# ConsenSys/gnark-crypto

Measured on AMD Instinct MI355X. Metric: G1 MSM/sec (BN254), higher is better.
Workload: dtype u32; 1 GPU; BN254 G1 MultiExp 2^20 points, bases+scalars resident in HBM; points=1048576, window_bits=16, windows=8, glv_half_scalars=True, resident_bases=False, parallelism=single GPU

## Files before the change

gnark-crypto_amd/_lib.py:

```python
import ctypes
import os
import subprocess

_HERE = os.path.dirname(os.path.abspath(__file__))
CSRC = os.path.join(_HERE, "csrc")
LIB_PATH = os.environ.get("GMSM_LIB") or os.path.join(CSRC, "libgmsm.so")

GMSM_OK, GMSM_ERR_LEN, GMSM_ERR_CONFIG, GMSM_ERR_DEVICE, GMSM_ERR_ARG, GMSM_ERR_POINT = 0, 1, 2, 3, 4, 5

GROUP_IDS = {
    ("bn254", "g1"): 0, ("bn254", "g2"): 1,
    ("bls12_381", "g1"): 2, ("bls12_381", "g2"): 3,
    ("bw6_761", "g1"): 4, ("bw6_761", "g2"): 5,
}

ABI_SYMBOLS = [
    "gmsm_bn254_g1_multiexp", "gmsm_bn254_g2_multiexp", "gmsm_bls12_381_g1_multiexp", "gmsm_bls12_381_g2_multiexp",
    "gmsm_bw6_761_g1_multiexp", "gmsm_bw6_761_g2_multiexp", "gmsm_multiexp", "gmsm_multiexp_affine", "gmsm_fold",
    "gmsm_multiexp_device", "gmsm_bases_register", "gmsm_bases_release", "gmsm_multiexp_bases",
    "gmsm_multiexp_bases_device", "gmsm_multiexp_bases_submit", "gmsm_multiexp_collect", "gmsm_multiexp_bases_batch", "gmsm_default_window_bits", "gmsm_default_plan", "gmsm_num_windows", "gmsm_window_sums_device",
    "gmsm_window_sums_enqueue", "gmsm_fold_window_sets", "gmsm_fold_windows", "gmsm_batch_scalar_mul", "gmsm_batch_scalar_mul_device",
    "gmsm_batch_jac_to_affine", "gmsm_jac_to_affine", "gmsm_affine_limbs", "gmsm_scalar_limbs", "gmsm_debug_decompose",
    "gmsm_debug_field_op", "gmsm_debug_group_op", "gmsm_debug_glv_split", "gmsm_generate_points", "gmsm_set_profiling", "gmsm_get_stage_times",
    "gmsm_get_stage_launches", "gmsm_points_from_raw", "gmsm_points_validate", "gmsm_bases_register_raw",
    "gmsm_points_from_compressed", "gmsm_points_compress", "gmsm_bases_register_compressed",
    "gmsm_bases_register_dump", "gmsm_fft_domain_new", "gmsm_fft_domain_release", "gmsm_fft_domain_info", "gmsm_fft",
    "gmsm_fft_bit_reverse", "gmsm_poly_eval", "gmsm_poly_div_x_minus_a", "gmsm_kzg_open", "gmsm_kzg_open_folded",
    "gmsm_to_lagrange_g1", "gmsm_bases_to_lagrange", "gmsm_batch_scale", "gmsm_update_monomials", "gmsm_linear_combinations", "gmsm_shplonk_open_w", "gmsm_shplonk_open_wprime",
    "gmsm_fr_batch_invert", "gmsm_iop_ratio_copy_constraint", "gmsm_iop_ratio_shuffled",
    "gmsm_fflonk_next_divisor", "gmsm_fflonk_fold", "gmsm_fflonk_fold_commit", "gmsm_fflonk_open_w", "gmsm_fflonk_open_wprime",
    "gmsm_bases_precompute", "gmsm_bases_table_bits", "gmsm_debug_table_runs", "gmsm_debug_small_runs", "gmsm_debug_reduce_shape", "gmsm_multiexp_sharded", "gmsm_bases_register_sharded", "gmsm_multiexp_bases_sharded", "gmsm_set_devices",
    "gmsm_get_devices", "gmsm_set_option", "gmsm_get_option", "gmsm_trim", "gmsm_shutdown",
    "gmsm_device_count", "gmsm_set_device", "gmsm_last_error",
    "gmsm_version",
]

_lib = None


def build(jobs=None):
    jobs = jobs or os.cpu_count() or 4
    subprocess.check_call(["make", "-C", CSRC, f"-j{jobs}", "libgmsm.so"])
    return LIB_PATH


def load():
    global _lib
    if _lib is not None:
        return _lib
    if not os.path.exists(LIB_PATH):
        raise RuntimeError(f"{LIB_PATH} is missing: run `make -C gnark-crypto_amd/csrc` (or __graft_entry__.build()); "
                           "there is no fallback implementation")
    if os.environ.get("GMSM_NO_TORCH", "0") != "1":
        try:
            import torch
        except ImportError:
            pass
    L = ctypes.CDLL(LIB_PATH)
    vp, sz, u64p = ctypes.c_void_p, ctypes.c_size_t, ctypes.c_void_p
    for name in ABI_SYMBOLS[:6]:
        f = getattr(L, name)
        f.restype = ctypes.c_int
        f.argtypes = [u64p, sz, u64p, sz, ctypes.c_int, u64p]
    L.gmsm_multiexp.restype = ctypes.c_int
    L.gmsm_multiexp.argtypes = [ctypes.c_int, u64p, sz, u64p, sz, ctypes.c_int, u64p]
    L.gmsm_multiexp_affine.restype = ctypes.c_int
    L.gmsm_multiexp_affine.argtypes = [ctypes.c_int, u64p, sz, u64p, sz, ctypes.c_int, u64p]
    L.gmsm_fold.restype = ctypes.c_int
    L.gmsm_fold.argtypes = [ctypes.c_int, u64p, sz, u64p, ctypes.c_int, u64p]
    L.gmsm_multiexp_device.restype = ctypes.c_int
    L.gmsm_multiexp_device.argtypes = [ctypes.c_int, vp, vp, sz, vp, u64p]
    L.gmsm_bases_register.restype = ctypes.c_int
    L.gmsm_bases_register.argtypes = [ctypes.c_int, u64p, vp, sz, vp]
    L.gmsm_bases_release.restype = ctypes.c_int
    L.gmsm_bases_release.argtypes = [ctypes.c_uint64]
    L.gmsm_bases_precompute.restype = ctypes.c_int
    L.gmsm_bases_precompute.argtypes = [ctypes.c_uint64, ctypes.c_uint]
    L.gmsm_bases_table_bits.restype = ctypes.c_uint
    L.gmsm_bases_table_bits.argtypes = [ctypes.c_uint64]
    L.gmsm_debug_table_runs.restype = ctypes.c_ulong
    L.gmsm_debug_table_runs.argtypes = []
    L.gmsm_debug_small_runs.restype = ctypes.c_ulong
    L.gmsm_debug_small_runs.argtypes = []
    L.gmsm_debug_reduce_shape.restype = ctypes.c_int
    L.gmsm_debug_reduce_shape.argtypes = [ctypes.c_int, ctypes.c_uint32, ctypes.c_uint32, ctypes.POINTER(ctypes.c_uint32)]
    L.gmsm_multiexp_bases.restype = ctypes.c_int
    L.gmsm_multiexp_bases.argtypes = [ctypes.c_uint64, u64p, sz, ctypes.c_int, u64p]
    L.gmsm_multiexp_bases_device.restype = ctypes.c_int
    L.gmsm_multiexp_bases_device.argtypes = [ctypes.c_uint64, vp, sz, vp, u64p]
    L.gmsm_multiexp_bases_submit.restype = ctypes.c_int
    L.gmsm_multiexp_bases_submit.argtypes = [ctypes.c_uint64, vp, sz, vp, ctypes.POINTER(ctypes.c_uint64)]
    L.gmsm_multiexp_bases_batch.restype = ctypes.c_int
    L.gmsm_multiexp_bases_batch.argtypes = [ctypes.c_uint64, u64p, vp, sz, sz, vp, u64p]
    L.gmsm_multiexp_collect.restype = ctypes.c_int
    L.gmsm_multiexp_collect.argtypes = [ctypes.c_uint64, u64p]
    L.gmsm_default_window_bits.restype = ctypes.c_uint
    L.gmsm_default_window_bits.argtypes = [ctypes.c_int, sz]
    L.gmsm_default_plan.restype = ctypes.c_int
    L.gmsm_default_plan.argtypes = [ctypes.c_int, sz] + [ctypes.POINTER(ctypes.c_uint)] * 4
    L.gmsm_num_windows.restype = ctypes.c_uint
    L.gmsm_num_windows.argtypes = [ctypes.c_int, ctypes.c_uint]
    L.gmsm_window_sums_device.restype = ctypes.c_int
    L.gmsm_window_sums_device.argtypes = [ctypes.c_int, vp, vp, sz, ctypes.c_uint, ctypes.c_uint, ctypes.c_uint, vp, u64p]
    L.gmsm_window_sums_enqueue.restype = ctypes.c_int
    L.gmsm_window_sums_enqueue.argtypes = [ctypes.c_int, vp, ctypes.c_uint64, vp, sz, ctypes.c_uint, ctypes.c_uint,
                                           ctypes.c_uint, vp, vp]
    L.gmsm_fold_window_sets.restype = ctypes.c_int
    L.gmsm_fold_window_sets.argtypes = [ctypes.c_int, ctypes.c_uint, u64p, ctypes.c_uint, u64p]
    L.gmsm_batch_scalar_mul.restype = ctypes.c_int
    L.gmsm_batch_scalar_mul.argtypes = [ctypes.c_int, u64p, u64p, sz, u64p]
    L.gmsm_batch_scalar_mul_device.restype = ctypes.c_int
    L.gmsm_batch_scalar_mul_device.argtypes = [ctypes.c_int, u64p, vp, sz, vp, vp]
    L.gmsm_batch_jac_to_affine.restype = ctypes.c_int
    L.gmsm_batch_jac_to_affine.argtypes = [ctypes.c_int, u64p, sz, u64p]
    L.gmsm_fold_windows.restype = ctypes.c_int
    L.gmsm_fold_windows.argtypes = [ctypes.c_int, ctypes.c_uint, u64p, u64p]
    L.gmsm_jac_to_affine.restype = ctypes.c_int
    L.gmsm_jac_to_affine.argtypes = [ctypes.c_int, u64p, u64p]
    L.gmsm_affine_limbs.restype = sz
    L.gmsm_affine_limbs.argtypes = [ctypes.c_int]
    L.gmsm_scalar_limbs.restype = sz
    L.gmsm_scalar_limbs.argtypes = [ctypes.c_int]
    L.gmsm_debug_decompose.restype = ctypes.c_int
    L.gmsm_debug_decompose.argtypes = [ctypes.c_int, u64p, sz, ctypes.c_uint, vp]
    L.gmsm_debug_field_op.restype = ctypes.c_int
    L.gmsm_debug_field_op.argtypes = [ctypes.c_int, ctypes.c_int, ctypes.c_int, u64p, u64p, sz, u64p]
    L.gmsm_debug_group_op.restype = ctypes.c_int
    L.gmsm_debug_group_op.argtypes = [ctypes.c_int, ctypes.c_int, u64p, u64p, sz, u64p]
    L.gmsm_generate_points.restype = ctypes.c_int
    L.gmsm_generate_points.argtypes = [ctypes.c_int, u64p, u64p, u64p, ctypes.c_int, sz, ctypes.c_int, u64p]
    L.gmsm_set_profiling.restype = None
    L.gmsm_set_profiling.argtypes = [ctypes.c_int]
    L.gmsm_get_stage_times.restype = ctypes.c_int
    L.gmsm_get_stage_times.argtypes = [vp, ctypes.c_int, vp]
    i64p = ctypes.POINTER(ctypes.c_int64)
    L.gmsm_points_from_raw.restype = ctypes.c_int
    L.gmsm_points_from_raw.argtypes = [ctypes.c_int, vp, sz, ctypes.c_int, u64p, vp, i64p]
    L.gmsm_points_validate.restype = ctypes.c_int
    L.gmsm_points_validate.argtypes = [ctypes.c_int, u64p, vp, sz, ctypes.c_int, i64p]
    L.gmsm_bases_register_raw.restype = ctypes.c_int
    L.gmsm_bases_register_raw.argtypes = [ctypes.c_int, vp, sz, ctypes.c_int, ctypes.POINTER(ctypes.c_uint64), i64p]
    L.gmsm_points_from_compressed.restype = ctypes.c_int
    L.gmsm_points_from_compressed.argtypes = [ctypes.c_int, vp, sz, ctypes.c_int, u64p, vp, i64p]
    L.gmsm_points_compress.restype = ctypes.c_int
    L.gmsm_points_compress.argtypes = [ctypes.c_int, u64p, vp, sz, vp]
    L.gmsm_bases_register_compressed.restype = ctypes.c_int
    L.gmsm_bases_register_compressed.argtypes = [ctypes.c_int, vp, sz, ctypes.c_int, ctypes.POINTER(ctypes.c_uint64), i64p]
    L.gmsm_bases_register_dump.restype = ctypes.c_int
    L.gmsm_bases_register_dump.argtypes = [ctypes.c_int, ctypes.c_char_p, ctypes.c_uint64, ctypes.c_int, sz, ctypes.c_int,
                                           ctypes.POINTER(ctypes.c_uint64), ctypes.POINTER(sz), i64p]
    L.gmsm_fft_domain_new.restype = ctypes.c_int
    L.gmsm_fft_domain_new.argtypes = [ctypes.c_int, ctypes.c_uint64, ctypes.POINTER(ctypes.c_uint64)]
    L.gmsm_fft_domain_release.restype = ctypes.c_int
    L.gmsm_fft_domain_release.argtypes = [ctypes.c_uint64]
    L.gmsm_fft_domain_info.restype = ctypes.c_int
    L.gmsm_fft_domain_info.argtypes = [ctypes.c_uint64, ctypes.POINTER(ctypes.c_uint64), u64p, u64p, u64p, u64p, u64p]
    L.gmsm_fft.restype = ctypes.c_int
    L.gmsm_fft.argtypes = [ctypes.c_uint64, u64p, vp, sz, ctypes.c_int, ctypes.c_int, ctypes.c_int, vp]
    L.gmsm_fft_bit_reverse.restype = ctypes.c_int
    L.gmsm_fft_bit_reverse.argtypes = [ctypes.c_int, u64p, vp, sz, vp]
    szp = ctypes.POINTER(sz)
    L.gmsm_poly_eval.restype = ctypes.c_int
    L.gmsm_poly_eval.argtypes = [ctypes.c_int, u64p, vp, szp, sz, u64p, vp, u64p]
    L.gmsm_poly_div_x_minus_a.restype = ctypes.c_int
    L.gmsm_poly_div_x_minus_a.argtypes = [ctypes.c_int, u64p, vp, sz, u64p, vp, u64p, vp, u64p]
    L.gmsm_kzg_open.restype = ctypes.c_int
    L.gmsm_kzg_open.argtypes = [ctypes.c_uint64, u64p, vp, sz, u64p, vp, u64p, u64p]
    L.gmsm_kzg_open_folded.restype = ctypes.c_int
    L.gmsm_kzg_open_folded.argtypes = [ctypes.c_uint64, u64p, vp, szp, sz, u64p, u64p, vp, u64p]
    L.gmsm_to_lagrange_g1.restype = ctypes.c_int
    L.gmsm_to_lagrange_g1.argtypes = [ctypes.c_int, u64p, vp, sz, vp, u64p, vp]
    L.gmsm_bases_to_lagrange.restype = ctypes.c_int
    L.gmsm_bases_to_lagrange.argtypes = [ctypes.c_uint64, sz, ctypes.POINTER(ctypes.c_uint64)]
    L.gmsm_batch_scale.restype = ctypes.c_int
    L.gmsm_batch_scale.argtypes = [ctypes.c_int, u64p, vp, sz, u64p, vp, sz, vp, u64p, vp]
    L.gmsm_update_monomials.restype = ctypes.c_int
    L.gmsm_update_monomials.argtypes = [ctypes.c_int, u64p, vp, sz, u64p, vp, u64p, vp]
    L.gmsm_linear_combinations.restype = ctypes.c_int
    L.gmsm_linear_combinations.argtypes = [ctypes.c_int, u64p, vp, sz, szp, sz, u64p, vp, u64p, u64p]
    L.gmsm_shplonk_open_w.restype = ctypes.c_int
    L.gmsm_shplonk_open_w.argtypes = [ctypes.c_uint64, u64p, vp, szp, sz, u64p, szp, u64p, vp, u64p, u64p, vp, u64p]
    L.gmsm_shplonk_open_wprime.restype = ctypes.c_int
    L.gmsm_shplonk_open_wprime.argtypes = [ctypes.c_uint64, u64p, vp, szp, sz, u64p, szp, u64p, u64p, u64p, vp, u64p, vp, u64p]
    L.gmsm_fflonk_next_divisor.restype = ctypes.c_int
    L.gmsm_fflonk_next_divisor.argtypes = [ctypes.c_int, sz, szp]
    L.gmsm_fflonk_fold.restype = ctypes.c_int
    L.gmsm_fflonk_fold.argtypes = [ctypes.c_int, u64p, vp, szp, sz, vp, u64p, vp]
    L.gmsm_fflonk_fold_commit.restype = ctypes.c_int
    L.gmsm_fflonk_fold_commit.argtypes = [ctypes.c_uint64, u64p, vp, szp, sz, vp, vp, u64p]
    L.gmsm_fflonk_open_w.restype = ctypes.c_int
    L.gmsm_fflonk_open_w.argtypes = [ctypes.c_uint64, u64p, vp, szp, szp, sz, u64p, szp, u64p, vp, u64p, u64p, u64p, vp, u64p]
    L.gmsm_fflonk_open_wprime.restype = ctypes.c_int
    L.gmsm_fflonk_open_wprime.argtypes = [ctypes.c_uint64, u64p, vp, szp, szp, sz, u64p, szp, u64p, u64p, u64p, vp, u64p, vp, u64p]
    u32p = ctypes.POINTER(ctypes.c_uint32)
    L.gmsm_fr_batch_invert.restype = ctypes.c_int
    L.gmsm_fr_batch_invert.argtypes = [ctypes.c_int, u64p, vp, sz, vp, u64p, vp]
    L.gmsm_iop_ratio_copy_constraint.restype = ctypes.c_int
    L.gmsm_iop_ratio_copy_constraint.argtypes = [ctypes.c_uint64, u64p, vp, sz, u32p, vp, vp, u64p, u64p, ctypes.c_int, ctypes.c_int, vp, u64p, vp]
    L.gmsm_iop_ratio_shuffled.restype = ctypes.c_int
    L.gmsm_iop_ratio_shuffled.argtypes = [ctypes.c_uint64, u64p, vp, u64p, vp, sz, u32p, u32p, u64p, ctypes.c_int, ctypes.c_int, vp, u64p, vp]
    L.gmsm_get_stage_launches.restype = ctypes.c_int
    L.gmsm_get_stage_launches.argtypes = [vp, ctypes.c_int]
    ip = ctypes.POINTER(ctypes.c_int)
    L.gmsm_multiexp_sharded.restype = ctypes.c_int
    L.gmsm_multiexp_sharded.argtypes = [ctypes.c_int, u64p, sz, u64p, sz, ctypes.c_int, ip, ctypes.c_int, ctypes.c_int, u64p]
    L.gmsm_bases_register_sharded.restype = ctypes.c_int
    L.gmsm_bases_register_sharded.argtypes = [ctypes.c_int, u64p, sz, ip, ctypes.c_int, ctypes.POINTER(ctypes.c_uint64)]
    L.gmsm_multiexp_bases_sharded.restype = ctypes.c_int
    L.gmsm_multiexp_bases_sharded.argtypes = [ctypes.c_uint64, u64p, sz, ctypes.c_int, ctypes.c_int, u64p]
    L.gmsm_set_devices.restype = ctypes.c_int
    L.gmsm_set_devices.argtypes = [ip, ctypes.c_int]
    L.gmsm_get_devices.restype = ctypes.c_int
    L.gmsm_get_devices.argtypes = [ip, ctypes.c_int]
    L.gmsm_debug_glv_split.restype = ctypes.c_int
    L.gmsm_debug_glv_split.argtypes = [ctypes.c_int, u64p, sz, vp]
    L.gmsm_set_option.restype = ctypes.c_int
    L.gmsm_set_option.argtypes = [ctypes.c_int, ctypes.c_uint]
    L.gmsm_get_option.restype = ctypes.c_uint
    L.gmsm_get_option.argtypes = [ctypes.c_int]
    L.gmsm_trim.restype = ctypes.c_int
    L.gmsm_trim.argtypes = [sz, ctypes.POINTER(sz)]
    L.gmsm_shutdown.restype = ctypes.c_int
    L.gmsm_shutdown.argtypes = []
    L.gmsm_device_count.restype = ctypes.c_int
    L.gmsm_set_device.restype = ctypes.c_int
    L.gmsm_set_device.argtypes = [ctypes.c_int]
    L.gmsm_last_error.restype = ctypes.c_char_p
    L.gmsm_version.restype = ctypes.c_char_p
    _lib = L
    return L


def effective_cpus():
    n = len(os.sched_getaffinity(0))
    try:
        quota, period = open("/sys/fs/cgroup/cpu.max").read().split()
        if quota != "max":
            n = min(n, max(1, int(int(quota) / int(period))))
    except (OSError, ValueError):
        pass
    return n


def last_error():
    return load().gmsm_last_error().decode()


OPTIONS = {"window_bits": 0, "tables": 1, "max_run": 2, "host_ranges": 3, "fixed_base_bits": 4, "spin_wait_us": 5, "small_bits": 6, "small_max": 7, "split": 8, "glv": 9, "small_quad": 10,
           "poly_lane_bits": 11, "reduce_shape": 12}


def set_option(name, value):
    rc = load().gmsm_set_option(OPTIONS[name], int(value))
    if rc:
        raise ValueError("gmsm: " + last_error())


def get_option(name):
    return int(load().gmsm_get_option(OPTIONS[name]))


class options:

    def __init__(self, **kw):
        self.kw, self.old = kw, {}

    def __enter__(self):
        for k, v in self.kw.items():
            self.old[k] = get_option(k)
            set_option(k, v)
        return self

    def __exit__(self, *exc):
        for k, v in self.old.items():
            set_option(k, v)
        return False


def trim(keep_bytes=0):
    freed = ctypes.c_size_t(0)
    rc = load().gmsm_trim(keep_bytes, ctypes.byref(freed))
    if rc:
        raise RuntimeError("gmsm: " + last_error())
    return int(freed.value)


def shutdown():
    rc = load().gmsm_shutdown()
    if rc:
        raise RuntimeError("gmsm: " + last_error())
```

gnark-crypto_amd/csrc/gmsm_context.h:

```cpp
#pragma once
#include <hip/hip_runtime.h>
#include <atomic>

#include <algorithm>
#include <cstdio>
#include <cstdlib>
#include <chrono>
#include <condition_variable>
#include <memory>
#include <mutex>
#include <string>
#include <thread>
#include <vector>

#include "../../include/gmsm.h"

namespace gmsm {

int fail(int code, const std::string &msg);
void clear_last_error();

#define HIP_TRY(expr)                                                                                        \
    do {                                                                                                     \
        hipError_t e_ = (expr);                                                                              \
        if (e_ != hipSuccess)                                                                                \
            return ::gmsm::fail(GMSM_ERR_DEVICE, std::string(#expr) + ": " + hipGetErrorString(e_) + " (" __FILE__ ":" + \
                                                     std::to_string(__LINE__) + ")");                        \
    } while (0)

struct DeviceBuffer {
    void *ptr = nullptr;
    size_t cap = 0;
    int ensure(size_t bytes) {
        if (bytes <= cap) return GMSM_OK;
        if (ptr) HIP_TRY(hipFree(ptr));
        ptr = nullptr;
        cap = 0;
        size_t want = bytes + bytes / 8;
        HIP_TRY(hipMalloc(&ptr, want));
        cap = want;
        return GMSM_OK;
    }
    size_t release() {
        const size_t had = cap;
        if (ptr) (void)hipFree(ptr);
        ptr = nullptr;
        cap = 0;
        return had;
    }
};

struct Options {
    std::atomic<unsigned> window_bits{0};
    std::atomic<unsigned> tables{1};
    std::atomic<unsigned> max_run{0};
    std::atomic<unsigned> host_ranges{0};
    std::atomic<unsigned> fixed_base_bits{0};
    std::atomic<unsigned> spin_wait_us{0};
    std::atomic<unsigned> small_bits{0};
    std::atomic<unsigned> split{0};
    std::atomic<unsigned> small_max{0};
    std::atomic<unsigned> glv{1};
    std::atomic<unsigned> small_quad{0};
    std::atomic<unsigned> poly_lane_bits{0};
    std::atomic<unsigned> reduce_shape{0};
};
Options &options();

extern std::atomic<unsigned long> g_small_runs;
extern std::atomic<unsigned long> g_table_runs;

struct ResidentBases {
    int group = -1;
    int device = -1;
    size_t n = 0;
    DeviceBuffer upoints, skip;
    std::atomic<unsigned> tab_c{0};
    unsigned tab_nw = 0;
    std::mutex tab_mu;
    DeviceBuffer tables;
    std::atomic<unsigned> small_c{0};
    unsigned small_nw = 0;
    size_t small_m = 0;
    DeviceBuffer small_tables;
    ResidentBases() = default;
    ResidentBases(const ResidentBases &) = delete;
    ResidentBases &operator=(const ResidentBases &) = delete;
    ~ResidentBases() {
        if (!upoints.ptr && !skip.ptr && !tables.ptr && !small_tables.ptr) return;
        int prev = 0;
        (void)hipGetDevice(&prev);
        if (device >= 0) (void)hipSetDevice(device);
        (void)hipDeviceSynchronize();
        if (upoints.ptr) (void)hipFree(upoints.ptr);
        if (skip.ptr) (void)hipFree(skip.ptr);
        if (tables.ptr) (void)hipFree(tables.ptr);
        if (small_tables.ptr) (void)hipFree(small_tables.ptr);
        (void)hipSetDevice(prev);
    }
};


struct FftDomain {
    int group = -1;
    int device = -1;
    unsigned log2n = 0;
    std::vector<uint64_t> generator, generator_inv, cardinality_inv, shift, shift_inv;
    DeviceBuffer twiddles_lz, twiddles_inv_lz;
    DeviceBuffer twiddles_rev_lz, twiddles_inv_rev_lz;
    bool rev_ready = false;
    DeviceBuffer coset, coset_inv_scaled;
    std::vector<uint64_t> cardinality_inv_lz;
    bool coset_ready = false;
    std::mutex mu;
    FftDomain() = default;
    FftDomain(const FftDomain &) = delete;
    FftDomain &operator=(const FftDomain &) = delete;
    ~FftDomain() {
        DeviceBuffer *bufs[] = {&twiddles_lz, &twiddles_inv_lz, &twiddles_rev_lz, &twiddles_inv_rev_lz, &coset, &coset_inv_scaled};
        bool any = false;
        for (auto *b : bufs) any = any || b->ptr;
        if (!any) return;
        int prev = 0;
        (void)hipGetDevice(&prev);
        if (device >= 0) (void)hipSetDevice(device);
        (void)hipDeviceSynchronize();
        for (auto *b : bufs)
            if (b->ptr) (void)hipFree(b->ptr);
        (void)hipSetDevice(prev);
    }
};

struct Workspace {
    hipStream_t stream = nullptr;
    DeviceBuffer upoints, skip;
    DeviceBuffer seg_lvl;
    DeviceBuffer seg_partials, seg_flags, seg_bucket;
    DeviceBuffer parted;
    DeviceBuffer heavy;
    DeviceBuffer long_pieces;
    DeviceBuffer small_sums, small_done;
    DeviceBuffer digits, sorted, blockhist, counts, starts, buckets, partials, totals;
    DeviceBuffer red_pre;
    DeviceBuffer carry;
    hipStream_t mstream = nullptr;
    hipEvent_t ev_buckets = nullptr, ev_merged = nullptr;
    hipStream_t cstream = nullptr;
    hipEvent_t ev_fork = nullptr, ev_conv = nullptr;
    bool conv_pending = false;
    hipEvent_t events[12] = {nullptr};
    bool timed = false;
    int timed_level = 0;
    void *pinned = nullptr;
    size_t pinned_cap = 0;
    DeviceBuffer h2d_points, h2d_scalars;
    DeviceBuffer raw_bytes, flagword;
    DeviceBuffer poly;
    DeviceBuffer lagrange;
    bool busy = false;
    bool ticket = false;
    bool pending = false;
    int pending_group = -1;
    unsigned pending_c = 0;
    uint32_t pending_nw = 0;
    uint32_t pending_gen = 0;
    std::shared_ptr<ResidentBases> bases_ref;
    hipEvent_t dep = nullptr;
    bool uncollected = false;
    hipEvent_t last_use = nullptr;
    hipStream_t last_stream = nullptr;
    bool pending_timed = false;
    size_t trim(size_t keep) {
        DeviceBuffer *all[] = {&upoints, &skip, &seg_lvl, &seg_partials, &seg_flags, &seg_bucket, &parted, &heavy, &long_pieces, &small_sums, &small_done, &digits, &sorted,
                               &blockhist, &counts, &starts, &buckets, &partials, &totals, &red_pre, &carry, &h2d_points,
                               &h2d_scalars, &raw_bytes, &flagword, &poly, &lagrange};
        size_t freed = 0;
        for (DeviceBuffer *b : all)
            if (b->cap > keep) freed += b->release();
        if (pinned && pinned_cap > keep) {
            (void)hipHostFree(pinned);
            pinned = nullptr;
            pinned_cap = 0;
        }
        return freed;
    }
    void destroy() {
        (void)trim(0);
        hipEvent_t *evs[] = {&ev_buckets, &ev_merged, &dep, &last_use, &ev_fork, &ev_conv};
        for (hipEvent_t *e : evs) {
            if (*e) (void)hipEventDestroy(*e);
            *e = nullptr;
        }
        for (auto &e : events) {
            if (e) (void)hipEventDestroy(e);
            e = nullptr;
        }
        if (stream) (void)hipStreamDestroy(stream);
        if (mstream) (void)hipStreamDestroy(mstream);
        if (cstream) (void)hipStreamDestroy(cstream);
        stream = mstream = cstream = nullptr;
        last_stream = nullptr;
        bases_ref.reset();
    }
    int ensure_base() {
        if (stream) return GMSM_OK;
        HIP_TRY(hipStreamCreateWithFlags(&stream, hipStreamNonBlocking));
        HIP_TRY(hipEventCreateWithFlags(&ev_buckets, hipEventDisableTiming));
        HIP_TRY(hipEventCreateWithFlags(&ev_merged, hipEventDisableTiming));
        HIP_TRY(hipEventCreateWithFlags(&ev_fork, hipEventDisableTiming));
        HIP_TRY(hipEventCreateWithFlags(&ev_conv, hipEventDisableTiming));
        return GMSM_OK;
    }
    int side_stream(hipStream_t &slot) {
        if (!slot) HIP_TRY(hipStreamCreateWithFlags(&slot, hipStreamNonBlocking));
        return GMSM_OK;
    }
    int ensure_pinned(size_t bytes) {
        if (bytes <= pinned_cap) return GMSM_OK;
        if (pinned) HIP_TRY(hipHostFree(pinned));
        pinned = nullptr;
        HIP_TRY(hipHostMalloc(&pinned, bytes, hipHostMallocDefault));
        pinned_cap = bytes;
        return GMSM_OK;
    }
};

struct Context {
    static constexpr int NUM_WS = 3, MAX_TICKETS = 2;
    std::mutex mu;
    std::condition_variable cv;
    int device = -1;
    Workspace ws[NUM_WS];
    int num_cus = 256;
    uint64_t epoch = 0;
    std::atomic<bool> live{false};
    int init(int dev) {
        device = dev;
// ... 281 lines not shown
    if (!v || !*v) return dflt;
    return (unsigned)strtoul(v, nullptr, 10);
}
#ifdef GMSM_EXPERIMENTS
static inline unsigned tune_uint(const char *name, unsigned dflt) { return env_uint(name, dflt); }
#else
static inline constexpr unsigned tune_uint(const char *, unsigned dflt) { return dflt; }
#endif

static inline unsigned preferred_c(unsigned fr_bits, size_t aff_bytes, size_t n) {
    unsigned lg = 0;
    while (lg < 63 && ((size_t)2 << lg) <= n) ++lg;
    if (fr_bits > 320) return lg < 13 ? 9u : lg <= 14 ? 10u : lg <= 16 ? 12u : lg <= 20 ? 14u : 16u;
    if (fr_bits == 255 && aff_bytes > 96) return lg < 13 ? 8u : lg <= 15 ? 10u : lg == 16 ? 12u : lg <= 18 ? 13u : 16u;
    if (fr_bits == 255) return lg < 13 ? 8u : lg <= 14 ? 12u : lg == 15 ? 13u : lg == 16 ? 12u : lg == 18 ? 13u : lg < 24 ? 16u : 17u;
    if (aff_bytes > 64) return lg < 13 ? 8u : lg <= 14 ? 12u : lg == 15 ? 13u : lg == 16 ? 12u : lg <= 18 ? 13u : lg < 22 ? 16u : 17u;
    return lg < 13 ? 8u : lg < 15 ? 12u : lg < 17 ? 15u : lg < 21 ? 16u : 17u;
}
static inline unsigned glv_preferred_c(unsigned fr_bits, size_t aff_bytes, size_t n) {
    unsigned lg = 0;
    while (lg < 63 && ((size_t)2 << lg) <= n) ++lg;
    if (lg < 11 || lg > 21) return 0u;
    if (fr_bits > 320) return lg <= 14 ? 10u : lg <= 16 ? 12u : lg == 17 ? 13u : lg == 18 ? 14u : 16u;
    if (fr_bits == 255 && aff_bytes > 96)
        return lg <= 14 ? 10u : lg <= 16 ? 12u : lg <= 18 ? 13u : lg == 19 ? 15u : 0u;
    if (lg < 13) return 0u;
    if (fr_bits == 255) return lg <= 14 ? 13u : lg == 16 ? 12u : lg == 19 ? 16u : 0u;
    if (aff_bytes > 64) return lg == 13 ? 12u : lg == 14 ? 13u : lg <= 16 ? 12u : lg == 17 ? 13u : 16u;
    return lg == 13 ? 12u : lg == 14 ? 13u : lg <= 20 ? 16u : 0u;
}
static inline unsigned choose_c(unsigned fr_bits, size_t aff_bytes, size_t n) {
    const unsigned forced = options().window_bits.load(std::memory_order_relaxed);
    if (forced >= 2 && forced <= 20) return forced;
    return preferred_c(fr_bits, aff_bytes, n ? n : 1);
}

struct GroupVTable {
    unsigned fr_bits;
    size_t aff_bytes, scalar_bytes, jac_bytes, xyzz_bytes;
    int (*multiexp_host)(const uint64_t *points, size_t n_points, const uint64_t *scalars, size_t n_scalars, int nb_tasks,
                         uint64_t *out_jac);
    int (*multiexp_device)(Context &ctx, const void *d_points, const void *d_scalars, size_t n, hipStream_t stream,
                           uint64_t *out_jac, const ResidentBases *resident);
    int (*window_sums)(Context &ctx, const void *d_points, const void *d_scalars, size_t n, unsigned c, unsigned win_first,
                       unsigned win_stride, hipStream_t stream, uint64_t *out_xyzz, const ResidentBases *resident);
    void (*fold)(const uint64_t *xyzz_windows, unsigned c, uint64_t *out_jac);
    void (*jac_to_affine)(const uint64_t *jac, uint64_t *out_affine);
    int (*debug_decompose)(const uint64_t *scalars, size_t n, unsigned c, uint32_t *out_digits);
    int (*debug_field_op)(int field, int op, const uint64_t *a, const uint64_t *b, size_t count, uint64_t *out);
    int (*debug_group_op)(int op, const uint64_t *acc, const uint64_t *other, size_t count, uint64_t *out);
    void (*generate_points)(const uint64_t *base, const uint64_t *k0, const uint64_t *k1, int klimbs, size_t n, int nthreads,
                            uint64_t *out);
    int (*register_bases)(Context &ctx, const void *d_points, size_t n, hipStream_t stream, ResidentBases *out);
    int (*submit)(Context &ctx, Workspace &ws, const void *d_scalars, size_t n, const ResidentBases *resident);
    int (*collect)(Workspace &ws, uint64_t *out_jac);
    int (*window_sums_enqueue)(Context &ctx, const void *d_points, const void *d_scalars, size_t n, unsigned c,
                               unsigned win_first, unsigned win_stride, hipStream_t stream, void *d_out_xyzz,
                               const std::shared_ptr<ResidentBases> &resident);
    void (*fold_sets)(const uint64_t *xyzz_sets, unsigned nsets, unsigned c, uint64_t *out_jac);
    void (*fold_powers)(const uint64_t *coeff, size_t n, uint64_t *out_scalars);
    int (*multiexp_bases_host)(Context &ctx, const uint64_t *scalars, size_t n, uint64_t *out_jac,
                               const ResidentBases *resident);
    int (*batch_scalar_mul)(Context &ctx, const uint64_t *base, const uint64_t *scalars, const void *d_scalars, size_t n,
                            hipStream_t caller_stream, uint64_t *out, void *d_out);
    int (*batch_jac_to_affine)(Context &ctx, const uint64_t *jac, size_t n, uint64_t *out);
    int (*decode_raw)(Workspace &ws, const void *d_raw, size_t n, int level, void *d_out, long long *bad_index,
                      uint32_t *status);
    int (*validate_points)(Workspace &ws, const void *d_points, size_t n, int level, long long *bad_index, uint32_t *status);
    int (*decode_compressed)(Workspace &ws, const void *d_comp, size_t n, int level, void *d_out, long long *bad_index,
                             uint32_t *status);
    int (*encode_compressed)(Workspace &ws, const void *d_points, size_t n, void *d_comp);
    int (*fft_domain_new)(Context &ctx, hipStream_t stream, unsigned log2n, FftDomain *out);
    int (*fft_run)(hipStream_t stream, FftDomain *d, void *d_a, bool inverse, bool dif, bool coset);
    int (*fft_bit_reverse)(hipStream_t stream, void *d_a, size_t n);
    int (*precompute_tables)(Context &ctx, Workspace &ws, ResidentBases *rb, unsigned c);
    bool (*tables_serve)(size_t n_registered, size_t n_call);
    int (*shard_piece)(Context &ctx, const uint64_t *points, const ResidentBases *resident, size_t resident_base,
                       const uint64_t *scalars, size_t n, unsigned c, unsigned win_first, unsigned win_stride,
                       uint64_t *out_xyzz);
    unsigned (*host_piece_ranges)(size_t n, bool with_points);
    int (*debug_glv_split)(const uint64_t *scalars, size_t n, uint32_t *out);
    void (*plan_info)(size_t n, unsigned *c, unsigned *nwin, unsigned *entries_per_point, unsigned *fused);
    void (*reduce_shape)(const Context &ctx, uint32_t nw, uint32_t nbuckets, uint32_t out[6]);
    int (*poly_eval)(Context &ctx, const uint64_t *polys, const void *d_polys, const size_t *lens, size_t k, const uint64_t *point,
                     hipStream_t stream, uint64_t *out_values);
    int (*poly_div)(Context &ctx, const uint64_t *poly, const void *d_poly, size_t n, const uint64_t *point, hipStream_t stream,
                    uint64_t *out_h, void *d_out_h, uint64_t *out_value);
    int (*kzg_open)(Context &ctx, const uint64_t *polys, const void *d_polys, const size_t *lens, size_t k, const uint64_t *point,
                    const uint64_t *gamma, hipStream_t stream, uint64_t *out_claimed, uint64_t *out_jac, const ResidentBases *resident);
    int (*to_lagrange)(Context &ctx, const uint64_t *coeffs, const void *d_coeffs, const ResidentBases *from, unsigned log2n,
                       hipStream_t stream, uint64_t *out_affine, void *d_out_affine, ResidentBases *out_bases);
    bool (*fflonk_next_divisor)(size_t n, size_t *t);
    int (*open_check)(const char *entry, const size_t *lens, const size_t *pack_sizes, size_t k, const uint64_t *points,
                      const size_t *npoints, bool check_size, size_t registered);
    int (*fflonk_fold)(Context &ctx, const uint64_t *polys, const void *d_polys, const size_t *lens, size_t npolys, hipStream_t stream,
                       uint64_t *out, void *d_out, const ResidentBases *resident, uint64_t *out_jac);
    int (*open_w)(Context &ctx, const uint64_t *polys, const void *d_polys, const size_t *lens, const size_t *pack_sizes, size_t k,
                  const uint64_t *points, const size_t *npoints, const uint64_t *gamma, hipStream_t stream, uint64_t *out_claimed,
                  uint64_t *out_folded_claimed, uint64_t *out_w, void *d_out_w, uint64_t *out_jac, const ResidentBases *resident);
    int (*open_wprime)(Context &ctx, const uint64_t *polys, const void *d_polys, const size_t *lens, const size_t *pack_sizes, size_t k,
                       const uint64_t *points, const size_t *npoints, const uint64_t *folded_claimed, const uint64_t *gamma,
                       const uint64_t *w, const void *d_w, const uint64_t *z, hipStream_t stream, uint64_t *out_jac,
                       const ResidentBases *resident);
    int (*batch_scale)(Context &ctx, const uint64_t *points, const void *d_points, size_t n, const uint64_t *scalars, const void *d_scalars,
                       size_t n_scalars, const uint64_t *r, hipStream_t stream, uint64_t *out_affine, void *d_out_affine);
    int (*linear_combinations)(Context &ctx, const uint64_t *points, const void *d_points, size_t n, const size_t *ends, size_t n_ends,
                               const uint64_t *r, hipStream_t stream, uint64_t *out_truncated_jac, uint64_t *out_shifted_jac);
    int (*fr_batch_invert)(Context &ctx, const uint64_t *a, const void *d_a, size_t n, hipStream_t stream, uint64_t *out, void *d_out);
    int (*ratio_copy)(Context &ctx, FftDomain *d, const uint64_t *entries, const void *d_entries, size_t m, const uint32_t *layouts,
                      const int64_t *perm, const void *d_perm, const uint64_t *beta, const uint64_t *gamma, int basis, int layout,
                      hipStream_t stream, uint64_t *out, void *d_out);
    int (*ratio_shuffled)(Context &ctx, FftDomain *d, const uint64_t *num, const void *d_num, const uint64_t *den, const void *d_den,
                          size_t m, const uint32_t *num_layouts, const uint32_t *den_layouts, const uint64_t *beta, int basis, int layout,
                          hipStream_t stream, uint64_t *out, void *d_out);
    unsigned fr_max_order;
};

}
```

gnark-crypto_amd/csrc/gmsm_engine.hip:

```cpp
#include <atomic>
#include <cstdio>
#include <cstring>
#include <deque>
#include <functional>
#include <map>
#include <sys/stat.h>

#include "gmsm_context.h"

namespace gmsm {

static thread_local std::string g_last_error;
static std::mutex g_any_error_mu;
static std::string g_any_error;
static thread_local int g_device = -1;
static std::atomic<int> g_default_device{0};
std::atomic<unsigned long> g_table_runs{0};
std::atomic<unsigned long> g_small_runs{0};
static std::atomic<uint32_t> g_ticket_gen{0};

std::string g_env_error;
Options &options() {
    static Options *o = [] {
        Options *x = new Options();
        const unsigned c = env_uint("GMSM_C", 0);
        x->window_bits.store(c >= 2 && c <= 20 ? c : 0);
        const unsigned t = env_uint("GMSM_TABLES", 1);
        x->tables.store(std::min(2u, t));
        if (c != 0 && (c < 2 || c > 20)) g_env_error = "GMSM_C=" + std::to_string(c) + ": the window width must be 2..20 (or unset)";
        else if (t > 2) g_env_error = "GMSM_TABLES=" + std::to_string(t) + ": 0 never, 1 the measured call sizes, 2 every call size";
        return x;
    }();
    return *o;
}

int fail(int code, const std::string &msg) {
    g_last_error = msg;
    {
        std::lock_guard<std::mutex> lk(g_any_error_mu);
        g_any_error = msg;
    }
    return code;
}

void clear_last_error() { g_last_error.clear(); }

static std::mutex g_prof_mu;
static std::atomic<int> g_profiling{0};
static double g_stage_ms[STAGE_COUNT] = {0};
static unsigned long g_stage_launches[STAGE_COUNT] = {0};
static unsigned long g_stage_calls = 0;

int profiling_level() { return g_profiling.load(std::memory_order_relaxed); }
void record_stage_times(const float *ms, const unsigned *launches) {
    std::lock_guard<std::mutex> lk(g_prof_mu);
    for (int i = 0; i < STAGE_COUNT; ++i) {
        g_stage_ms[i] += ms[i];
        g_stage_launches[i] += launches[i];
    }
    ++g_stage_calls;
}

static std::mutex g_ctx_mu;
static std::vector<Context *> g_ctx;

int get_context_for(int device, Context **out) {
    std::lock_guard<std::mutex> lk(g_ctx_mu);
    int ndev = 0;
    hipError_t e = hipGetDeviceCount(&ndev);
    if (e != hipSuccess || ndev <= 0)
        return fail(GMSM_ERR_DEVICE, std::string("no usable HIP device (hipGetDeviceCount: ") + hipGetErrorString(e) +
                                         "); libgmsm has no CPU fallback");
    if (device < 0 || device >= ndev) return fail(GMSM_ERR_DEVICE, "gmsm_set_device: device index out of range");
    if ((int)g_ctx.size() < ndev) g_ctx.resize(ndev, nullptr);
    if (!g_ctx[device]) g_ctx[device] = new Context();
    if (!g_ctx[device]->live) {
        int rc = g_ctx[device]->init(device);
        if (rc != GMSM_OK) return rc;
    }
    *out = g_ctx[device];
    return GMSM_OK;
}

int get_context(Context **out) { return get_context_for(g_device >= 0 ? g_device : g_default_device.load(), out); }

int get_context_of_pointer(const void *p, Context **out) {
    if (p) {
        hipPointerAttribute_t attr;
        if (hipPointerGetAttributes(&attr, p) == hipSuccess && attr.type == hipMemoryTypeDevice)
            return get_context_for(attr.device, out);
        (void)hipGetLastError();
    }
    return get_context(out);
}

static int select_device(int rc, Context *const *ctx) {
    if (rc) return rc;
    HIP_TRY(hipSetDevice((*ctx)->device));
    return GMSM_OK;
}
static int enter(Context **ctx) { return select_device(get_context(ctx), ctx); }
// ... 672 lines not shown
}

struct ShardedBases {
    int group = -1;
    size_t n = 0;
    std::vector<int> devices;
    std::map<int, std::shared_ptr<ResidentBases>> replicas;
};
constexpr uint64_t SHARDED_TAG = (uint64_t)1 << 62;
static HandleTable<ShardedBases> g_sharded;

static std::shared_ptr<ShardedBases> lookup_sharded(uint64_t handle) {
    return (handle & SHARDED_TAG) ? g_sharded.get(handle & ~SHARDED_TAG) : nullptr;
}

GMSM_EXPORT int gmsm_bases_register_sharded(int group, const uint64_t *points, size_t n, const int *devices, int n_devices,
                                            uint64_t *out_handle) {
    VT_OR_FAIL(group);
    if (!out_handle) return fail(GMSM_ERR_ARG, "gmsm_bases_register_sharded: out_handle is null");
    if (n && !points) return fail(GMSM_ERR_ARG, "gmsm_bases_register_sharded: points is null");
    auto sb = std::make_shared<ShardedBases>();
    sb->group = group;
    sb->n = n;
    if (devices && n_devices > 0) sb->devices.assign(devices, devices + n_devices);
    else if (int rc0 = shard_devices(sb->devices)) return rc0;
    const int ndev = gmsm_device_count();
    if (ndev <= 0) return fail(GMSM_ERR_DEVICE, "no usable HIP device; libgmsm has no CPU fallback");
    if (sb->devices.empty()) every_device(ndev, sb->devices);
    if (int rc = devices_exist("gmsm_bases_register_sharded", sb->devices.data(), sb->devices.size(), ndev)) return rc;
    std::vector<int> distinct;
    for (int d : sb->devices)
        if (std::find(distinct.begin(), distinct.end(), d) == distinct.end()) distinct.push_back(d);
    std::vector<uint64_t> handles(distinct.size(), 0);
    const Failure bad = on_threads(distinct.size(), [&](size_t i) {
        g_device = distinct[i];
        return gmsm_bases_register(group, points, nullptr, n, &handles[i]);
    });
    for (size_t i = 0; i < distinct.size(); ++i)
        if (handles[i]) {
            sb->replicas[distinct[i]] = g_bases.get(handles[i]);
            (void)gmsm_bases_release(handles[i]);
        }
    if (bad.rc) return fail(bad.rc, "device " + std::to_string(distinct[bad.index]) + ": " + bad.err);
    *out_handle = SHARDED_TAG | g_sharded.add(sb);
    return GMSM_OK;
}

static int precompute_on(const BasesRef &rb, unsigned c) {
    const GroupVTable *vt = vtable(rb->group);
    std::lock_guard<std::mutex> only_one(rb->tab_mu);
    if (rb->tab_c.load() != 0) {
        if (c == 0 || c == rb->tab_c.load()) return GMSM_OK;
        return fail(GMSM_ERR_ARG, "gmsm_bases_precompute: the handle already has tables of another width");
    }
    Context *ctx;
    int rc = get_context_for(rb->device, &ctx);
    if (rc) return rc;
    struct RestoreDevice {
        int prev = 0;
        RestoreDevice() { (void)hipGetDevice(&prev); }
        ~RestoreDevice() { (void)hipSetDevice(prev); }
    } restore;
    HIP_TRY(hipSetDevice(ctx->device));
    GMSM_LEASE_OR_FAIL(lease, *ctx);
    return vt->precompute_tables(*ctx, *lease.w, rb.get(), c);
}

GMSM_EXPORT int gmsm_bases_precompute(uint64_t handle, unsigned c) {
    if (handle & SHARDED_TAG) {
        std::shared_ptr<ShardedBases> sb = lookup_sharded(handle);
        if (!sb) return fail(GMSM_ERR_ARG, "unknown bases handle");
        std::vector<BasesRef> replicas;
        for (auto &kv : sb->replicas) replicas.push_back(kv.second);
        const Failure bad = on_threads(replicas.size(), [&](size_t i) { return precompute_on(replicas[i], c); });
        return bad.rc ? fail(bad.rc, bad.err) : GMSM_OK;
    }
    BasesRef rb = g_bases.get(handle);
    if (!rb) return fail(GMSM_ERR_ARG, "unknown bases handle");
    return precompute_on(rb, c);
}

GMSM_EXPORT unsigned long gmsm_debug_table_runs(void) { return g_table_runs.load(); }
GMSM_EXPORT unsigned long gmsm_debug_small_runs(void) { return g_small_runs.load(); }

GMSM_EXPORT unsigned gmsm_bases_table_bits(uint64_t handle) {
    if (handle & SHARDED_TAG) {
        std::shared_ptr<ShardedBases> sb = lookup_sharded(handle);
        if (!sb || sb->replicas.empty()) return 0;
        return sb->replicas.begin()->second->tab_c.load();
    }
    BasesRef rb = g_bases.get(handle);
    return rb ? rb->tab_c.load() : 0;
}

GMSM_EXPORT int gmsm_bases_release(uint64_t handle) {
    BasesRef rb;
    std::shared_ptr<ShardedBases> sb;
    if (handle & SHARDED_TAG) sb = g_sharded.take(handle & ~SHARDED_TAG);
    else rb = g_bases.take(handle);
    if (!rb && !sb) return fail(GMSM_ERR_ARG, "unknown bases handle");
    std::vector<Context *> ctxs;
    {
        std::lock_guard<std::mutex> lk(g_ctx_mu);
        ctxs = g_ctx;
    }
    for (Context *c : ctxs) {
        if (!c) continue;
        BasesRef parked[Context::NUM_WS];
        {
            std::lock_guard<std::mutex> lk(c->mu);
            for (int i = 0; i < Context::NUM_WS; ++i) {
                Workspace &w = c->ws[i];
                if (w.busy || !w.bases_ref) continue;
                const bool mine = w.bases_ref == rb || (sb && sb->replicas.count(c->device) && sb->replicas[c->device] == w.bases_ref);
                if (mine && (!w.last_use || hipEventQuery(w.last_use) == hipSuccess)) parked[i].swap(w.bases_ref);
            }
        }
    }
    return GMSM_OK;
}

static int multiexp_bases_impl(uint64_t handle, const uint64_t *scalars, const void *d_scalars, size_t n, int nb_tasks,
                               void *hip_stream, uint64_t *out_jac) {
    BasesRef rb = g_bases.get(handle);
    if (!rb) return fail(GMSM_ERR_ARG, "unknown bases handle");
    const GroupVTable *vt = vtable(rb->group);
    if (n > rb->n) return fail(GMSM_ERR_LEN, "len(points) != len(scalars)");
    if (nb_tasks > 1024) return fail(GMSM_ERR_CONFIG, "invalid config: config.NbTasks > 1024");
    Context *ctx;
    if (int rc = enter_on(rb->device, &ctx)) return rc;
    if (scalars && n) return vt->multiexp_bases_host(*ctx, scalars, n, out_jac, rb.get());
    return vt->multiexp_device(*ctx, nullptr, d_scalars, n, (hipStream_t)hip_stream, out_jac, rb.get());
}

static int multiexp_bases_sharded(uint64_t handle, const uint64_t *scalars, size_t n, int nb_tasks, int mode, uint64_t *out_jac) {
    std::shared_ptr<ShardedBases> sb = lookup_sharded(handle);
    if (!sb) return fail(GMSM_ERR_ARG, "unknown bases handle");
    const GroupVTable *vt = vtable(sb->group);
    if (n > sb->n) return fail(GMSM_ERR_LEN, "len(points) != len(scalars)");
    bool done;
    int rc = multiexp_precheck(vt, n, n, nb_tasks, out_jac, &done);
    if (rc || done) return rc;
    if (!scalars) return fail(GMSM_ERR_ARG, "scalars is null");
    return multiexp_sharded_run(sb->group, nullptr, &sb->replicas, scalars, n, sb->devices, mode, out_jac);
}

GMSM_EXPORT int gmsm_multiexp_bases(uint64_t handle, const uint64_t *scalars, size_t n_scalars, int nb_tasks,
                                    uint64_t *out_jac) {
    if (handle & SHARDED_TAG) return multiexp_bases_sharded(handle, scalars, n_scalars, nb_tasks, 0, out_jac);
    return multiexp_bases_impl(handle, scalars, nullptr, n_scalars, nb_tasks, nullptr, out_jac);
}

GMSM_EXPORT int gmsm_multiexp_bases_sharded(uint64_t handle, const uint64_t *scalars, size_t n_scalars, int nb_tasks, int mode,
                                            uint64_t *out_jac) {
    if (!(handle & SHARDED_TAG)) return fail(GMSM_ERR_ARG, "gmsm_multiexp_bases_sharded: not a handle of gmsm_bases_register_sharded");
    return multiexp_bases_sharded(handle, scalars, n_scalars, nb_tasks, mode, out_jac);
}

GMSM_EXPORT int gmsm_multiexp_bases_device(uint64_t handle, const void *d_scalars, size_t n_scalars, void *hip_stream,
                                           uint64_t *out_jac) {
    return multiexp_bases_impl(handle, nullptr, d_scalars, n_scalars, 0, hip_stream, out_jac);
}

GMSM_EXPORT int gmsm_multiexp_bases_submit(uint64_t handle, const void *d_scalars, size_t n_scalars, void *hip_stream,
                                           uint64_t *out_ticket) {
    BasesRef rb = g_bases.get(handle);
// ... 649 lines not shown
    Context *ctx;
    if ((rc = enter_on(d->device, &ctx))) return rc;
    if ((rc = check_device_vector(E, "d_entries", d_entries, ctx->device)) || (rc = check_device_vector(E, "d_perm", d_perm, ctx->device)) ||
        (rc = check_device_vector(E, "d_out", d_out, ctx->device)))
        return rc;
    return vt->ratio_copy(*ctx, d.get(), entries, d_entries, m, layouts, perm, d_perm, beta, gamma, basis, layout, (hipStream_t)hip_stream, out, d_out);
}

GMSM_EXPORT int gmsm_iop_ratio_shuffled(uint64_t domain, const uint64_t *num, const void *d_num, const uint64_t *den, const void *d_den, size_t m,
                                        const uint32_t *num_layouts, const uint32_t *den_layouts, const uint64_t *beta, int basis, int layout,
                                        void *hip_stream, uint64_t *out, void *d_out) {
    const char *E = "gmsm_iop_ratio_shuffled";
    int rc = ratio_form(E, m, basis, layout, out, d_out);
    if (rc || (rc = ratio_layouts(E, "num_layouts", num_layouts, m)) || (rc = ratio_layouts(E, "den_layouts", den_layouts, m))) return rc;
    if (!beta) return fail(GMSM_ERR_ARG, std::string(E) + ": beta must not be null");
    if ((rc = ratio_pair(E, "num", "d_num", num, d_num)) || (rc = ratio_pair(E, "den", "d_den", den, d_den))) return rc;
    FftRef d;
    const GroupVTable *vt;
    if ((rc = ratio_domain(E, domain, m, &d, &vt))) return rc;
    const size_t zbytes = vt->scalar_bytes << d->log2n;
    if (ratio_overlap(out, d_out, zbytes, num, d_num, m * zbytes) || ratio_overlap(out, d_out, zbytes, den, d_den, m * zbytes)) return ratio_aliases(E);
    Context *ctx;
    if ((rc = enter_on(d->device, &ctx))) return rc;
    if ((rc = check_device_vector(E, "d_num", d_num, ctx->device)) || (rc = check_device_vector(E, "d_den", d_den, ctx->device)) ||
        (rc = check_device_vector(E, "d_out", d_out, ctx->device)))
        return rc;
    return vt->ratio_shuffled(*ctx, d.get(), num, d_num, den, d_den, m, num_layouts, den_layouts, beta, basis, layout, (hipStream_t)hip_stream, out,
                              d_out);
}

GMSM_EXPORT int gmsm_batch_scalar_mul(int group, const uint64_t *base_affine, const uint64_t *scalars, size_t n,
                                      uint64_t *out_affine) {
    VT_OR_FAIL(group);
    if (!base_affine || (n && (!scalars || !out_affine))) return fail(GMSM_ERR_ARG, "gmsm_batch_scalar_mul: null argument");
    Context *ctx;
    int rc = enter(&ctx);
    if (rc) return rc;
    return vt->batch_scalar_mul(*ctx, base_affine, scalars, nullptr, n, nullptr, out_affine, nullptr);
}

GMSM_EXPORT int gmsm_batch_scalar_mul_device(int group, const uint64_t *base_affine, const void *d_scalars, size_t n,
                                             void *hip_stream, void *d_out_affine) {
    VT_OR_FAIL(group);
    if (!base_affine || (n && (!d_scalars || !d_out_affine)))
        return fail(GMSM_ERR_ARG, "gmsm_batch_scalar_mul_device: null argument");
    Context *ctx;
    int rc = enter_owner(d_scalars, &ctx);
    if (rc) return rc;
    return vt->batch_scalar_mul(*ctx, base_affine, nullptr, d_scalars, n, (hipStream_t)hip_stream, nullptr, d_out_affine);
}

GMSM_EXPORT int gmsm_batch_jac_to_affine(int group, const uint64_t *jac, size_t n, uint64_t *out_affine) {
    VT_OR_FAIL(group);
    if (n && (!jac || !out_affine)) return fail(GMSM_ERR_ARG, "gmsm_batch_jac_to_affine: null argument");
    Context *ctx;
    int rc = enter(&ctx);
    if (rc) return rc;
    return vt->batch_jac_to_affine(*ctx, jac, n, out_affine);
}

GMSM_EXPORT unsigned gmsm_default_window_bits(int group, size_t n) {
    const GroupVTable *vt = vtable(group);
    return vt ? choose_c(vt->fr_bits, vt->aff_bytes, n) : 0;
}

GMSM_EXPORT int gmsm_default_plan(int group, size_t n, unsigned *c, unsigned *nwin, unsigned *entries_per_point, unsigned *fused) {
    VT_OR_FAIL(group);
    unsigned a = 0, b = 0, e = 1, f = 0;
    vt->plan_info(n, &a, &b, &e, &f);
    if (c) *c = a;
    if (nwin) *nwin = b;
    if (entries_per_point) *entries_per_point = e;
    if (fused) *fused = f;
    return GMSM_OK;
}

GMSM_EXPORT int gmsm_debug_reduce_shape(int group, uint32_t nw, uint32_t nbuckets, uint32_t out[6]) {
    VT_OR_FAIL(group);
    if (nw == 0 || nbuckets == 0 || nbuckets > (1u << 19) || !out) return fail(GMSM_ERR_ARG, "gmsm_debug_reduce_shape: nw >= 1, 1 <= nbuckets <= 2^19");
    Context *ctx;
    int rc = get_context(&ctx);
    if (rc) return rc;
    vt->reduce_shape(*ctx, nw, nbuckets, out);
    return GMSM_OK;
}

GMSM_EXPORT unsigned gmsm_num_windows(int group, unsigned c) {
    const GroupVTable *vt = vtable(group);
    return (vt && c) ? num_windows(vt->fr_bits, c) : 0;
}

GMSM_EXPORT int gmsm_window_sums_device(int group, const void *d_points, const void *d_scalars, size_t n, unsigned c,
                                        unsigned win_first, unsigned win_stride, void *hip_stream, uint64_t *out_xyzz) {
    VT_OR_FAIL(group);
    if (c < 2 || c > 20) return fail(GMSM_ERR_ARG, "c out of range (2..20)");
    Context *ctx;
    int rc = enter_owner(d_scalars, &ctx);
    if (rc) return rc;
    return vt->window_sums(*ctx, d_points, d_scalars, n, c, win_first, win_stride, (hipStream_t)hip_stream, out_xyzz, nullptr);
}

GMSM_EXPORT int gmsm_window_sums_enqueue(int group, const void *d_points, uint64_t bases_handle, const void *d_scalars,
                                         size_t n, unsigned c, unsigned win_first, unsigned win_stride, void *hip_stream,
                                         void *d_out_xyzz) {
    VT_OR_FAIL(group);
    if (c < 2 || c > 20) return fail(GMSM_ERR_ARG, "c out of range (2..20)");
    if (!d_out_xyzz) return fail(GMSM_ERR_ARG, "d_out_xyzz is null");
    BasesRef rb;
    if (bases_handle) {
        rb = g_bases.get(bases_handle);
        if (!rb || rb->group != group) return fail(GMSM_ERR_ARG, "unknown bases handle");
        if (n > rb->n) return fail(GMSM_ERR_LEN, "len(points) != len(scalars)");
    }
    Context *ctx;
    int rc = rb ? enter_on(rb->device, &ctx) : enter_owner(d_out_xyzz, &ctx);
    if (rc) return rc;
    return vt->window_sums_enqueue(*ctx, d_points, d_scalars, n, c, win_first, win_stride, (hipStream_t)hip_stream,
                                   d_out_xyzz, rb);
}

GMSM_EXPORT int gmsm_fold_window_sets(int group, unsigned c, const uint64_t *xyzz_sets, unsigned nsets, uint64_t *out_jac) {
    VT_OR_FAIL(group);
    if (c < 2 || c > 24) return fail(GMSM_ERR_ARG, "c out of range");
    if (nsets == 0) return fail(GMSM_ERR_ARG, "nsets must be >= 1");
    vt->fold_sets(xyzz_sets, nsets, c, out_jac);
    return GMSM_OK;
}

GMSM_EXPORT int gmsm_fold_windows(int group, unsigned c, const uint64_t *xyzz_windows, uint64_t *out_jac) {
    VT_OR_FAIL(group);
    if (c < 2 || c > 24) return fail(GMSM_ERR_ARG, "c out of range");
    vt->fold(xyzz_windows, c, out_jac);
    return GMSM_OK;
}

GMSM_EXPORT int gmsm_jac_to_affine(int group, const uint64_t *jac, uint64_t *out_affine) {
    VT_OR_FAIL(group);
    vt->jac_to_affine(jac, out_affine);
    return GMSM_OK;
}

GMSM_EXPORT size_t gmsm_affine_limbs(int group) {
    const GroupVTable *vt = vtable(group);
    return vt ? vt->aff_bytes / 8 : 0;
}

GMSM_EXPORT size_t gmsm_scalar_limbs(int group) {
    const GroupVTable *vt = vtable(group);
    return vt ? vt->scalar_bytes / 8 : 0;
}

GMSM_EXPORT int gmsm_debug_decompose(int group, const uint64_t *scalars, size_t n, unsigned c, uint32_t *out_digits) {
    VT_OR_FAIL(group);
    return vt->debug_decompose(scalars, n, c, out_digits);
}

GMSM_EXPORT int gmsm_debug_glv_split(int group, const uint64_t *scalars, size_t n, uint32_t *out) {
    VT_OR_FAIL(group);
    return vt->debug_glv_split(scalars, n, out);
}

GMSM_EXPORT int gmsm_debug_field_op(int group, int field, int op, const uint64_t *a, const uint64_t *b, size_t count,
                                    uint64_t *out) {
    VT_OR_FAIL(group);
    if (count == 0) return GMSM_OK;
    return vt->debug_field_op(field, op, a, b, count, out);
// ... 27 lines not shown
GMSM_EXPORT int gmsm_get_stage_times(double *out_ms, int max_stages, unsigned long *out_calls) {
    std::lock_guard<std::mutex> lk(g_prof_mu);
    int n = max_stages < (int)STAGE_COUNT ? max_stages : (int)STAGE_COUNT;
    for (int i = 0; i < n; ++i) out_ms[i] = g_stage_ms[i];
    if (out_calls) *out_calls = g_stage_calls;
    return n;
}

GMSM_EXPORT int gmsm_get_stage_launches(unsigned long *out_launches, int max_stages) {
    std::lock_guard<std::mutex> lk(g_prof_mu);
    int n = max_stages < (int)STAGE_COUNT ? max_stages : (int)STAGE_COUNT;
    for (int i = 0; i < n; ++i) out_launches[i] = g_stage_launches[i];
    return n;
}

GMSM_EXPORT int gmsm_device_count(void) {
    int n = 0;
    if (hipGetDeviceCount(&n) != hipSuccess) return 0;
    return n;
}

GMSM_EXPORT int gmsm_set_device(int device) {
    int n = gmsm_device_count();
    if (device < 0 || device >= n) return fail(GMSM_ERR_DEVICE, "gmsm_set_device: no such device");
    g_device = device;
    g_default_device.store(device);
    g_pinned.store(true);
    return GMSM_OK;
}

GMSM_EXPORT int gmsm_set_devices(const int *devices, int count) {
    std::vector<int> list;
    if (count > 0) {
        if (!devices) return fail(GMSM_ERR_ARG, "gmsm_set_devices: devices is null");
        if (int rc = devices_exist("gmsm_set_devices", devices, (size_t)count, gmsm_device_count())) return rc;
        list.assign(devices, devices + count);
    }
    std::lock_guard<std::mutex> lk(g_devices_mu);
    g_devices = list;
    g_devices_explicit = count > 0;
    if (count > 0) g_default_device.store(list[0]);
    else g_pinned.store(false);
    return GMSM_OK;
}

GMSM_EXPORT int gmsm_get_devices(int *out_devices, int max_devices) {
    std::vector<int> list;
    if (shard_devices(list) != GMSM_OK) return -1;
    if (list.empty()) {
        if (out_devices && max_devices > 0) out_devices[0] = g_device >= 0 ? g_device : g_default_device.load();
        return 1;
    }
    if (out_devices)
        for (int i = 0; i < (int)list.size() && i < max_devices; ++i) out_devices[i] = list[i];
    return (int)list.size();
}

struct OptionRow {
    int key;
    std::atomic<unsigned> Options::*member;
    bool (*accepts)(unsigned value);
    const char *refusal;
    bool as_flag = false;
};
static const OptionRow OPTION_ROWS[] = {
    {GMSM_OPT_WINDOW_BITS, &Options::window_bits, [](unsigned v) { return v == 0 || (v >= 2 && v <= 20); },
     "GMSM_OPT_WINDOW_BITS: 0 (the measured table) or 2..20"},
    {GMSM_OPT_TABLES, &Options::tables, [](unsigned v) { return v <= 2; }, "GMSM_OPT_TABLES: 0 never, 1 the measured call sizes, 2 every call size"},
    {GMSM_OPT_MAX_RUN, &Options::max_run, nullptr, nullptr},
    {GMSM_OPT_HOST_RANGES, &Options::host_ranges, nullptr, nullptr},
    {GMSM_OPT_FIXED_BASE_BITS, &Options::fixed_base_bits, [](unsigned v) { return v == 0 || (v >= 2 && v <= 14); },
     "GMSM_OPT_FIXED_BASE_BITS: 0 (by batch size) or 2..14"},
    {GMSM_OPT_SMALL_BITS, &Options::small_bits, [](unsigned v) { return v <= 7; },
     "GMSM_OPT_SMALL_BITS: 0 (on, width by size), 1 (off) or 2..7 (on, forced width)"},
    {GMSM_OPT_SMALL_MAX, &Options::small_max, nullptr, nullptr},
    {GMSM_OPT_SPLIT, &Options::split, nullptr, nullptr, true},
    {GMSM_OPT_GLV, &Options::glv, [](unsigned v) { return v <= 2; }, "GMSM_OPT_GLV: 0 never, 1 where measured ahead, 2 every unregistered call"},
    {GMSM_OPT_SMALL_QUAD, &Options::small_quad, [](unsigned v) { return v <= 2; }, "GMSM_OPT_SMALL_QUAD: 0 by call size, 1 never, 2 always"},
    {GMSM_OPT_POLY_LANE_BITS, &Options::poly_lane_bits, [](unsigned v) { return v <= 6; },
     "GMSM_OPT_POLY_LANE_BITS: 0 (lane width by length) or 1..6 (lanes of 2^(k-1) coefficients)"},
    {GMSM_OPT_REDUCE_SHAPE, &Options::reduce_shape,
     [](unsigned v) { return !(v > 255 || (v & 15u) > 8 || ((v >> 4) & 3u) == 1 || ((v >> 6) & 3u) == 3); },
     "GMSM_OPT_REDUCE_SHAPE: 0 (the cost model) or log2L (0, 1..8) | levels (0, 2, 3) << 4 | combine kernel (0, 1, 2) << 6"},
    {GMSM_OPT_SPIN_WAIT_US, &Options::spin_wait_us, [](unsigned v) { return v <= 1000000; }, "GMSM_OPT_SPIN_WAIT_US: at most 1000000"},
};
static const OptionRow *option_row(int key) {
    for (const OptionRow &r : OPTION_ROWS)
        if (r.key == key) return &r;
    return nullptr;
}

GMSM_EXPORT int gmsm_set_option(int key, unsigned value) {
    Options &o = options();
    const OptionRow *r = option_row(key);
    if (!r) return fail(GMSM_ERR_ARG, "gmsm_set_option: unknown key");
    if (r->accepts && !r->accepts(value)) return fail(GMSM_ERR_ARG, r->refusal);
    (o.*r->member).store(r->as_flag ? (value ? 1 : 0) : value);
    return GMSM_OK;
}

GMSM_EXPORT unsigned gmsm_get_option(int key) {
    Options &o = options();
    const OptionRow *r = option_row(key);
    return r ? (o.*r->member).load() : 0;
}

GMSM_EXPORT int gmsm_trim(size_t keep_bytes, size_t *out_freed) {
    if (out_freed) *out_freed = 0;
    std::vector<Context *> ctxs;
    {
        std::lock_guard<std::mutex> lk(g_ctx_mu);
        ctxs = g_ctx;
    }
    int prev = 0;
    (void)hipGetDevice(&prev);
    size_t freed = 0;
    for (Context *c : ctxs) {
        if (!c || !c->live) continue;
        (void)hipSetDevice(c->device);
        for (int i = 0; i < Context::NUM_WS; ++i) {
            Workspace *w = c->acquire_this(i);
            if (!w) continue;
            if (w->last_use) (void)hipEventSynchronize(w->last_use);
            if (w->stream) (void)hipStreamSynchronize(w->stream);
            if (w->mstream) (void)hipStreamSynchronize(w->mstream);
            if (w->cstream) (void)hipStreamSynchronize(w->cstream);
            w->conv_pending = false;
            std::shared_ptr<ResidentBases> parked;
            parked.swap(w->bases_ref);
            freed += w->trim(keep_bytes);
            c->release(w);
        }
    }
    (void)hipSetDevice(prev);
    if (out_freed) *out_freed = freed;
    return GMSM_OK;
}

GMSM_EXPORT int gmsm_shutdown(void) {
    std::vector<Context *> ctxs;
    {
        std::lock_guard<std::mutex> lk(g_ctx_mu);
        ctxs = g_ctx;
    }
    std::vector<std::pair<Context *, Workspace *>> held;
    for (Context *c : ctxs) {
        if (!c || !c->live) continue;
        for (int i = 0; i < Context::NUM_WS; ++i) {
            Workspace *w = c->acquire_unless_ticket(i);
            if (!w) {
                for (auto &h : held) h.first->release(h.second);
                return fail(GMSM_ERR_ARG, "gmsm_shutdown: a submitted MultiExp has not been collected");
            }
            held.emplace_back(c, w);
        }
    }
    {
        const auto bases = g_bases.drain();
        const auto sharded = g_sharded.drain();
        const auto ffts = g_fft.drain();
    }
    int prev = 0;
    (void)hipGetDevice(&prev);
    for (Context *c : ctxs) {
        if (!c || !c->live) continue;
        (void)hipSetDevice(c->device);
// ... 19 lines not shown
```

gnark-crypto_amd/csrc/gmsm_group.h:

```cpp
#pragma once
#include <algorithm>
#include <cstdlib>
#include <cstring>
#include <thread>
#include <type_traits>
#include <vector>

#include "gmsm_context.h"
#include "gmsm_group_host.h"
#include "gmsm_kernels.h"
#include "gmsm_fixup_q.h"
#include "gmsm_small.h"
#include "gmsm_fixedbase.h"
#include "gmsm_ingest.h"
#include "gmsm_decompress.h"
#include "gmsm_fft.h"
#include "gmsm_poly.h"
#include "gmsm_shplonk.h"
#include "gmsm_fflonk.h"
#include "gmsm_group_fft.h"
#include "gmsm_scale.h"
#include "gmsm_ratio.h"

namespace gmsm {

#define GMSM_TUNE(NAME, DFLT) tune_uint("GMSM_" #NAME, (DFLT))

template <class T> struct LazyOf;
template <class P> struct LazyOf<Fp<P>> { using type = FpU<P>; };
template <class P> struct LazyOf<Fp2<P>> { using type = Fp2U<P>; };

template <class F_, class FrP_, class Consts_, bool NEEDS_TORSION_>
struct Group : GroupHost<F_, FrP_> {
    using Host = GroupHost<F_, FrP_>;
    using Host::batch_to_affine;
    using Host::build_fixed_base_table;
    using Host::fold;
    using Host::fold_powers;
    using Host::fold_sets;
    using Host::generate_points;
    using Host::scalar_mul;
    using F = F_;
    using FrP = FrP_;
    using Consts = Consts_;
    static constexpr bool NEEDS_TORSION = NEEDS_TORSION_;
    using Aff = Affine<F>;
    using Ext = XYZZ<F>;
    using J = Jac<F>;
    static constexpr unsigned FR_BITS = FrP::BITS;
    static constexpr size_t AFF_BYTES = sizeof(Aff);
    static constexpr size_t SCALAR_BYTES = sizeof(Fp<FrP>);
    using U = typename LazyOf<F>::type;
#ifndef GMSM_INLINE_OPS_BYTES
#define GMSM_INLINE_OPS_BYTES (28 * 4)
#endif
    static constexpr bool INLINE_OPS = sizeof(U) <= GMSM_INLINE_OPS_BYTES;
    using OpsSerial = UnsatOps<U>;
    using OpsElem = typename OpsSerial::Elem;
#ifndef GMSM_FORK_CONVERT_LOG2
#define GMSM_FORK_CONVERT_LOG2 18
#endif
    static constexpr size_t FORK_CONVERT_MIN = (size_t)1 << GMSM_FORK_CONVERT_LOG2;
    static constexpr int COMBINE_N = 64;
    static constexpr int RED2_TPB = 64;
#ifndef GMSM_SERIAL_QUAD_WORDS
#define GMSM_SERIAL_QUAD_WORDS 14
#endif
    static constexpr bool SERIAL_QUAD = sizeof(U) >= GMSM_SERIAL_QUAD_WORDS * 4;
#ifndef GMSM_SERIAL_Q_QUADS
#define GMSM_SERIAL_Q_QUADS 64
#endif
    static constexpr int SERIAL_Q_QUADS = GMSM_SERIAL_Q_QUADS;
#ifndef GMSM_COMBINE_WE_WORDS
#define GMSM_COMBINE_WE_WORDS 9
#endif
    static constexpr bool COMBINE_WE = sizeof(U) <= GMSM_COMBINE_WE_WORDS * 4;
    static bool use_combine_we(const Context &ctx, uint32_t workgroups) {
        const unsigned forced = (options().reduce_shape.load(std::memory_order_relaxed) >> 6) & 3u;
        if (forced) return COMBINE_WE && forced == 2;
        return COMBINE_WE && workgroups >= 2u * (uint32_t)ctx.num_cus;
    }
    static constexpr uint32_t FIX_MAXWALK = FIXUP_MAXWALK;
#ifndef GMSM_FIXUP_QUAD_WORDS
#define GMSM_FIXUP_QUAD_WORDS 15
#endif
    static constexpr bool FIXUP_QUAD = sizeof(U) >= GMSM_FIXUP_QUAD_WORDS * 4;
    static constexpr bool SKEWED_HOST_RANGES = AFF_BYTES <= 96;
    static constexpr size_t COMBINE_RESIDENT = sizeof(U) <= 36 ? 4 : sizeof(U) <= 56 ? 3 : sizeof(U) <= 72 ? 2 : 1;

    static WindowPlan make_plan(unsigned c, unsigned win_first, unsigned win_stride) {
        WindowPlan p;
        p.c = c;
        p.nwin_total = num_windows(FR_BITS, c);
        unsigned lc = last_c(FR_BITS, c);
        p.nbuckets = 1u << (std::max(c, lc) - 1);
        p.win_first = win_first;
        p.win_stride = win_stride ? win_stride : 1;
        p.nwin_local = win_first < p.nwin_total ? (p.nwin_total - win_first + p.win_stride - 1) / p.win_stride : 0;
        p.shared = 0;
        p.glv = 0;
        return p;
    }
    static constexpr unsigned GLV_BITS = (unsigned)FrP::GLV_BITS;
    static WindowPlan make_plan_glv(unsigned c, unsigned win_first, unsigned win_stride) {
        WindowPlan p = make_plan(c, win_first, win_stride);
        p.nwin_total = num_windows(GLV_BITS, c);
        p.nbuckets = 1u << (std::max(c, last_c(GLV_BITS, c)) - 1);
        p.nwin_local = win_first < p.nwin_total ? (p.nwin_total - win_first + p.win_stride - 1) / p.win_stride : 0;
        p.glv = 1;
        return p;
    }

    static int window_sums(Context &ctx, Workspace &ws, const void *d_points, const void *d_scalars, size_t n,
                           const WindowPlan &plan, hipStream_t caller_stream, Ext *host_xyzz,
                           const ResidentBases *resident = nullptr, size_t resident_offset = 0) {
        int rc = order_after(ws, caller_stream);
        if (rc) return rc;
        if ((rc = enqueue_window_sums(ctx, ws, d_points, d_scalars, n, plan, ws.stream, resident, nullptr, resident_offset)))
            return rc;
        return collect_window_sums(ws, ws.stream, plan.nwin_local, host_xyzz);
    }

    static int collect_window_sums(Workspace &ws, hipStream_t stream, uint32_t nw, Ext *host_xyzz) {
        if (nw == 0) return GMSM_OK;
        HIP_TRY(wait_stream(stream));
        if (ws.pending_timed) StageTimer::collect(ws);
        ws.pending_timed = false;
        memcpy(host_xyzz, ws.pinned, (size_t)nw * sizeof(Ext));
        return GMSM_OK;
    }

    static uint64_t fr_modulus_shifted(unsigned shift) {
        uint64_t v = 0;
        for (int b = 62; b >= 0; --b) {
            const unsigned bit = shift + (unsigned)b;
            if (bit < 32u * FrP::N && ((FrP::Q[bit >> 5] >> (bit & 31)) & 1u)) v |= (uint64_t)1 << b;
        }
        return v;
    }
    static uint64_t max_digit_code(const WindowPlan &plan) {
        if (plan.glv) {
            const uint64_t low = ((uint64_t)1 << plan.c) - 1;
            const unsigned top_bits = GLV_BITS - (plan.nwin_total - 1) * plan.c;
            return std::max(low, (uint64_t)2 << top_bits);
        }
        const uint64_t low = ((uint64_t)1 << plan.c) - 1;
        const unsigned top_shift = (plan.nwin_total - 1) * plan.c;
        const uint64_t top = top_shift >= 63 + 32u * FrP::N ? 0 : ((fr_modulus_shifted(top_shift) + 1) << 1);
        return plan.nwin_total > 1 ? std::max(low, top) : top;
    }

    struct Geometry {
        uint32_t seg, tpw;
        uint32_t log2L, nblocks1, log2span;
        uint32_t nblocks2;
    };

    static Geometry plan_geometry(const Context &ctx, uint32_t nw, size_t n, uint32_t NB, bool shared_set = false) {
        Geometry q;
        constexpr size_t SPAN1 = COMBINE_N;
        const auto blocks1 = [&](uint32_t l2) { return ((size_t)NB + (SPAN1 << l2) - 1) / (SPAN1 << l2); };
        const auto blocks2 = [&](uint32_t l2) { return (blocks1(l2) + SPAN1 - 1) / SPAN1; };
        const unsigned forced_shape = options().reduce_shape.load(std::memory_order_relaxed);
        uint32_t log2L = GMSM_TUNE(LOG2L, forced_shape & 15u);
        const uint32_t force_levels = GMSM_TUNE(REDUCE_LEVELS, (forced_shape >> 4) & 3u);
        bool three = force_levels == 3;
        if (log2L == 0) {
            const auto costs = [&](uint32_t l2, size_t resident, size_t *c3) {
                const size_t serial_threads = (size_t)nw * (((size_t)NB + ((size_t)1 << l2) - 1) >> l2);
                const size_t serial_lanes = SERIAL_QUAD ? 4 * serial_threads : serial_threads;
                const size_t serial_rounds = (serial_lanes + (size_t)ctx.num_cus * 256 - 1) / ((size_t)ctx.num_cus * 256);
                const size_t per_round = (size_t)ctx.num_cus * resident;
                const size_t rounds = ((size_t)nw * blocks1(l2) + per_round - 1) / per_round;
                const size_t cost_serial = (SERIAL_QUAD ? 1 : 3) * serial_rounds * ((size_t)2 << l2);
                const size_t c2 = cost_serial + rounds * (2 * 6 + l2 + 1);
                const size_t rounds_b = ((size_t)nw * blocks2(l2) + per_round - 1) / per_round;
                *c3 = c2 + rounds_b * (2 * 6 + 8) + 4;
                return c2;
            };
            size_t best2 = ~(size_t)0, best3 = ~(size_t)0, unused = 0;
            uint32_t l2_two = 0, l2_three = 0;
            for (uint32_t l2 = 1; l2 <= 8; ++l2) {
                const size_t c2 = costs(l2, 1, &unused);
                if (blocks1(l2) <= (size_t)RED2_TPB && c2 < best2) {
                    best2 = c2;
                    l2_two = l2;
                }
                size_t c3 = 0;
                (void)costs(l2, COMBINE_RESIDENT, &c3);
                if (blocks1(l2) > 1 && blocks2(l2) <= (size_t)RED2_TPB && c3 < best3) {
                    best3 = c3;
                    l2_three = l2;
                }
            }
            const size_t two_resident = l2_two ? costs(l2_two, COMBINE_RESIDENT, &unused) : ~(size_t)0;
            if (force_levels == 3 ? l2_three != 0 : (force_levels != 2 && l2_three != 0 && best3 < two_resident)) {
                log2L = l2_three;
                three = true;
            } else if (l2_two) {
                log2L = l2_two;
                three = false;
            } else {
                log2L = 8;
            }
        } else if (three && blocks1(log2L) <= 1) {
            three = false;
        }
        if (three) {
            while (blocks2(log2L) > (size_t)RED2_TPB) ++log2L;
        } else {
            while (blocks1(log2L) > (size_t)RED2_TPB) ++log2L;
// ... 2 lines not shown
        q.nblocks1 = (uint32_t)blocks1(log2L);
        q.nblocks2 = three ? (uint32_t)blocks2(log2L) : 0u;
        q.log2span = log2L;
        for (size_t t = SPAN1; t > 1; t >>= 1) ++q.log2span;
        uint32_t seg = GMSM_TUNE(SEG, 0);
        if (seg == 0) {
            const size_t cap_blocks = (size_t)ctx.num_cus * AccWaves<U>::value;
            const size_t SEG_MAX = GMSM_TUNE(SEGMAX, 512);
            size_t seg_floor = 32;
            if (sizeof(U) <= 72 && n / NB <= 8) {
                const size_t entries = (size_t)nw * n, cap_threads = cap_blocks * 256;
                seg_floor = entries / 8 <= cap_threads ? 8 : entries / 16 <= cap_threads ? 16 : 32;
            } else if (sizeof(U) <= 72 && shared_set) {
                const size_t entries = (size_t)nw * n;
                if (sizeof(U) <= 56) seg_floor = entries <= ((size_t)1 << 19) ? 8 : entries <= ((size_t)3 << 19) ? 16 : 32;
                else seg_floor = entries <= ((size_t)3 << 18) ? 16 : 32;
            }
            size_t best_seg = 0, first_r = 0;
            double best_fill = -1.0;
            for (size_t r = 1; r < 100000; ++r) {
                const size_t bpw = r * cap_blocks / nw;
                if (bpw == 0) continue;
                const size_t sg = std::max<size_t>((n + bpw * 256 - 1) / (bpw * 256), seg_floor);
                if (sg > SEG_MAX) continue;
                if (!first_r) first_r = r;
                const size_t blocks = (size_t)nw * (((n + sg - 1) / sg + 255) / 256);
                const double fill = (double)blocks / (double)(((blocks + cap_blocks - 1) / cap_blocks) * cap_blocks);
                if (fill > best_fill + 1e-9) {
                    best_fill = fill;
                    best_seg = sg;
                }
                if (fill > 0.985 || r >= first_r + 5 || sg == seg_floor) break;
            }
            seg = (uint32_t)(best_seg ? best_seg : seg_floor);
        }
        q.seg = seg;
        q.tpw = (uint32_t)((n + seg - 1) / seg);
        return q;
    }

    static void launch_decompose(const void *d_scalars, size_t n, const WindowPlan &plan, bool d16, void *digits,
                                 const uint8_t *skip, hipStream_t stream) {
        const dim3 grid((unsigned)((n + 255) / 256)), block(256);
        if (plan.glv) {
#define GMSM_DECOMPOSE_GLV(CC)                                                                                                  \
    case CC:                                                                                                                    \
        if (d16) hipLaunchKernelGGL((k_decompose_glv<FrP, uint16_t, CC>), grid, block, 0, stream, (const uint32_t *)d_scalars, n, \
                                    plan, (uint16_t *)digits, skip);                                                             \
        else hipLaunchKernelGGL((k_decompose_glv<FrP, uint32_t, CC>), grid, block, 0, stream, (const uint32_t *)d_scalars, n,     \
                                plan, (uint32_t *)digits, skip);                                                                 \
        return;
            switch (plan.c) {
                GMSM_DECOMPOSE_GLV(10) GMSM_DECOMPOSE_GLV(11) GMSM_DECOMPOSE_GLV(12) GMSM_DECOMPOSE_GLV(13) GMSM_DECOMPOSE_GLV(14)
                GMSM_DECOMPOSE_GLV(15) GMSM_DECOMPOSE_GLV(16) GMSM_DECOMPOSE_GLV(17) GMSM_DECOMPOSE_GLV(18) GMSM_DECOMPOSE_GLV(20)
                default: return;
            }
#undef GMSM_DECOMPOSE_GLV
        }
#define GMSM_DECOMPOSE_C(CC)                                                                                                \
    case CC:                                                                                                                \
        if (d16) hipLaunchKernelGGL((k_decompose_c<FrP, uint16_t, CC>), grid, block, 0, stream, (const uint32_t *)d_scalars, n,  \
                                    plan, (uint16_t *)digits, skip);                                                         \
        else hipLaunchKernelGGL((k_decompose_c<FrP, uint32_t, CC>), grid, block, 0, stream, (const uint32_t *)d_scalars, n,      \
                                plan, (uint32_t *)digits, skip);                                                             \
        return;
        switch (plan.c) {
            GMSM_DECOMPOSE_C(8) GMSM_DECOMPOSE_C(9) GMSM_DECOMPOSE_C(10) GMSM_DECOMPOSE_C(12) GMSM_DECOMPOSE_C(13)
            GMSM_DECOMPOSE_C(14) GMSM_DECOMPOSE_C(15) GMSM_DECOMPOSE_C(16) GMSM_DECOMPOSE_C(17) GMSM_DECOMPOSE_C(18)
            GMSM_DECOMPOSE_C(20)
            default: break;
        }
#undef GMSM_DECOMPOSE_C
        if (d16)
            hipLaunchKernelGGL((k_decompose<FrP, uint16_t>), grid, block, 0, stream, (const uint32_t *)d_scalars, n, plan,
                               (uint16_t *)digits, skip);
        else
            hipLaunchKernelGGL((k_decompose<FrP, uint32_t>), grid, block, 0, stream, (const uint32_t *)d_scalars, n, plan,
                               (uint32_t *)digits, skip);
    }

    static int enqueue_window_sums(Context &ctx, Workspace &ws, const void *d_points, const void *d_scalars, size_t n,
                                   const WindowPlan &plan, hipStream_t stream, const ResidentBases *resident,
                                   void *d_out = nullptr, size_t resident_offset = 0 ,
                                   bool buckets_only = false, bool time_range = false ) {
        const uint32_t nwd = plan.nwin_local;
        ws.pending_timed = false;
        if (nwd == 0) return GMSM_OK;
        const bool shared = plan.shared != 0;
        if (shared && !(resident && resident->tab_c.load() == plan.c && plan.win_first == 0 && plan.win_stride == 1))
            return fail(GMSM_ERR_ARG, "shared-bucket plan without matching window tables");
        if (shared && n) g_table_runs.fetch_add(1, std::memory_order_relaxed);
        if (ws.uncollected) {
            if (ws.timed && hipEventQuery(ws.events[ws.timed_level == 2 ? T_FIXUP : T_END]) == hipSuccess) StageTimer::collect(ws);
            ws.uncollected = false;
        }
        int rc;
        if ((rc = begin_use(ws, stream))) return rc;
        if (n == 0) {
            int rc0 = ws.ensure_pinned((size_t)nwd * sizeof(Ext));
            if (rc0) return rc0;
            if (d_out) HIP_TRY(hipStreamSynchronize(stream));
            for (uint32_t k = 0; k < nwd; ++k) ((Ext *)ws.pinned)[k] = Ext::infinity();
            if (d_out) {
                HIP_TRY(hipMemcpyAsync(d_out, ws.pinned, (size_t)nwd * sizeof(Ext), hipMemcpyHostToDevice, stream));
                HIP_TRY(hipStreamSynchronize(stream));
            }
            return GMSM_OK;
        }
        const size_t n_points = n;
        const uint32_t nw = shared ? 1u : nwd;
        if (shared) n *= nwd;
        const bool glv = plan.glv != 0;
        if (glv && (shared || resident)) return fail(GMSM_ERR_ARG, "GLV plan over registered bases");
        if (glv) n *= 2;
        if (n >= ((size_t)1 << 31)) return fail(GMSM_ERR_ARG, "n must be < 2^31");
        const uint32_t NB = plan.nbuckets;
        constexpr size_t REC = sizeof(typename OpsSerial::Mem);

        const Geometry q = plan_geometry(ctx, nw, n, NB, shared);
        const bool split = options().split.load(std::memory_order_relaxed) != 0 && !buckets_only && !shared && nw >= 4 && q.nblocks2 == 0;
        const Geometry qa = split ? plan_geometry(ctx, nw / 2, n, NB, shared) : q;
        const size_t tot_thr = (size_t)nw * qa.tpw;
        const size_t tot_blk = (size_t)nw * q.nblocks1;

        uint32_t log2NB = 0;
        while ((1u << log2NB) < NB) ++log2NB;
        uint32_t log2n = 0;
        while (((size_t)1 << log2n) < n) ++log2n;
        const uint32_t lidx = log2n + 1;
        const uint32_t part_log2 = GMSM_TUNE(PART_LOG2, log2n <= 21 ? 13 : log2n >= 24 ? 15 : 14);
        int fb = (int)part_log2 + (int)log2NB - (int)log2n;
        if (fb > (int)log2NB) fb = (int)log2NB;
        if (fb > 15) fb = 15;
        if (fb < 0) fb = 0;
        if (fb + lidx > 32) fb = 32 - lidx;
        const uint32_t fbits = (uint32_t)fb;
        const uint32_t nparts = NB >> fbits;
        const bool big_chunk = n > ((size_t)1 << 25) && (size_t)nparts * 8 + PART_CHUNK_BIG * 6 <= 152 * 1024;
        const size_t pchunk_len = big_chunk ? PART_CHUNK_BIG : PART_CHUNK;
        const uint32_t pchunks = (uint32_t)((n + pchunk_len - 1) / pchunk_len);
        const size_t scatter_lds = (size_t)nparts * 8 + pchunk_len * 6;
        if (scatter_lds > 152 * 1024)
            return fail(GMSM_ERR_ARG, plan.c > 17 ? "window width too large for this many points in one pipeline run (a run takes up to "
                                                    "2^(44-c) points for c > 17): use a smaller c or split by point range"
                                                  : "more than 2^27 points in one pipeline run: split the window sums by point range "
                                                    "and add the sets (gmsm_fold_window_sets); the MultiExp entries do this themselves");
        const size_t fine_cnt_bytes = (size_t)4 << fbits;
        const uint32_t stage_cap = fine_cnt_bytes >= 156 * 1024 ? 0u
                                   : (uint32_t)std::min<size_t>(GMSM_TUNE(STAGE_CAP, part_log2 >= 15 ? 39000 : 24576),
                                                              (156 * 1024 - fine_cnt_bytes) / 4);
        if (stage_cap > 40u * 1024u) return fail(GMSM_ERR_ARG, "window geometry: staging slots beyond the fine sort's registers");
        if (fine_cnt_bytes + (size_t)stage_cap * 4 > 160 * 1024)
            return fail(GMSM_ERR_ARG, "window geometry: fine-sort counters exceed the LDS");
        const bool d16 = max_digit_code(plan) < 65536;
        const size_t dsz = d16 ? 2 : 4;

        if ((rc = ws.digits.ensure((size_t)nw * n * dsz))) return rc;
        if ((rc = ws.sorted.ensure((size_t)nw * n * 4))) return rc;
        if ((rc = ws.parted.ensure((size_t)nw * n * 4))) return rc;
        if ((rc = ws.starts.ensure((size_t)nw * (NB + 1) * 4))) return rc;
        if ((rc = ws.buckets.ensure((size_t)nw * NB * REC))) return rc;
        if ((rc = ws.partials.ensure((tot_blk + (size_t)nw * q.nblocks2) * 2 * REC))) return rc;
        const uint32_t T = (uint32_t)(((size_t)NB + ((size_t)1 << q.log2L) - 1) >> q.log2L);
        if ((rc = ws.red_pre.ensure((size_t)nw * T * 2 * REC))) return rc;
        if ((rc = ws.totals.ensure((size_t)nwd * sizeof(Ext)))) return rc;
        if ((rc = ws.ensure_pinned((size_t)nwd * sizeof(Ext)))) return rc;
        if ((rc = ws.blockhist.ensure((size_t)nw * pchunks * nparts * 4))) return rc;
        if ((rc = ws.counts.ensure((size_t)nw * (2 * nparts + 1) * 4))) return rc;
        if ((rc = ws.seg_partials.ensure(tot_thr * 2 * REC))) return rc;
        if ((rc = ws.seg_flags.ensure(tot_thr * 4))) return rc;
        if ((rc = ws.seg_bucket.ensure(tot_thr * 4))) return rc;
        const size_t list_cap = 2 * (tot_thr / FIX_MAXWALK + tot_thr / LONG_PIECE + nw + 16);
        if ((rc = ws.seg_lvl.ensure((size_t)nw * 4 + 16 + list_cap * sizeof(LongChain)))) return rc;
        uint32_t *long_flag = (uint32_t *)ws.seg_lvl.ptr;
        LongChain *long_list = (LongChain *)((char *)ws.seg_lvl.ptr + (((size_t)nw * 4 + 15) / 16) * 16);
        const size_t piece_sums_off = ((list_cap * 4 + 15) / 16) * 16;
        if ((rc = ws.long_pieces.ensure(piece_sums_off + list_cap * REC))) return rc;
        uint32_t *piece_done = (uint32_t *)ws.long_pieces.ptr;
        void *piece_sums = (char *)ws.long_pieces.ptr + piece_sums_off;
        const uint32_t hcap = (uint32_t)std::min<size_t>(nparts, n / ((size_t)stage_cap + 1) + 1);
        const uint32_t scap = (uint32_t)(n / HEAVY_SUB) + hcap;
        const size_t hparts_bytes = (((size_t)nw * hcap * sizeof(HeavyPart) + 15) / 16) * 16, hcount_bytes = (((size_t)nw * 8 + 4 + 15) / 16) * 16;
        if ((rc = ws.heavy.ensure(hparts_bytes + hcount_bytes + ((size_t)nw * scap << fbits) * 4))) return rc;
        HeavyPart *hparts = (HeavyPart *)ws.heavy.ptr;
        uint32_t *hcount = (uint32_t *)((char *)ws.heavy.ptr + hparts_bytes);
        uint32_t *subhist = (uint32_t *)((char *)ws.heavy.ptr + hparts_bytes + hcount_bytes);
        if (nw > HEAVY_MAX_WINDOWS) return fail(GMSM_ERR_ARG, "more than 256 windows in one pipeline run");
        const uint32_t heavy_wg = (uint32_t)std::min<size_t>((size_t)2 * ctx.num_cus, std::max<size_t>((size_t)nw * scap, 1));
        uint32_t *bh = (uint32_t *)ws.blockhist.ptr, *part_base = (uint32_t *)ws.counts.ptr;
        uint32_t *part_pop = part_base + (size_t)nw * (nparts + 1);

        if ((rc = ctx.allow_lds((const void *)k_part_hist<uint16_t>, 160 * 1024))) return rc;
        if ((rc = ctx.allow_lds((const void *)k_part_hist<uint32_t>, 160 * 1024))) return rc;
        if ((rc = ctx.allow_lds((const void *)k_part_scatter<uint16_t, PART_CHUNK>, 152 * 1024))) return rc;
        if ((rc = ctx.allow_lds((const void *)k_part_scatter<uint32_t, PART_CHUNK>, 152 * 1024))) return rc;
        if ((rc = ctx.allow_lds((const void *)k_part_scatter<uint16_t, PART_CHUNK_BIG>, 152 * 1024))) return rc;
        if ((rc = ctx.allow_lds((const void *)k_part_scatter<uint32_t, PART_CHUNK_BIG>, 152 * 1024))) return rc;
        if ((rc = ctx.allow_lds((const void *)k_fine_sort<24>, 160 * 1024))) return rc;
        if ((rc = ctx.allow_lds((const void *)k_fine_sort<40>, 160 * 1024))) return rc;
        if ((rc = ctx.allow_lds((const void *)k_heavy_hist, 128 * 1024))) return rc;
        if ((rc = ctx.allow_lds((const void *)k_heavy_scan, 128 * 1024))) return rc;
        if ((rc = ctx.allow_lds((const void *)k_heavy_place, 128 * 1024))) return rc;
        if ((rc = ctx.allow_lds((const void *)k_fixup_long<U>, (int)(128 * sizeof(QRec<U>))))) return rc;
        if constexpr (FIXUP_QUAD)
            if ((rc = ctx.allow_lds((const void *)k_fixup_seg_q<U>, (int)(128 * sizeof(QRec<U>))))) return rc;
        if ((rc = ctx.allow_lds((const void *)k_combine_q<U, true, COMBINE_N>, (int)((2 * COMBINE_N + 1) * sizeof(QRec<U>))))) return rc;
        if constexpr (COMBINE_WE)
            if ((rc = ctx.allow_lds((const void *)k_combine_we<U, true>, (int)((2 * COMBINE_N + 1) * sizeof(QRec<U>))))) return rc;
        if constexpr (SERIAL_QUAD)
            if ((rc = ctx.allow_lds((const void *)k_reduce_serial_q<U, SERIAL_Q_QUADS>, (int)(3 * SERIAL_Q_QUADS * sizeof(QRec<U>))))) return rc;
        if ((rc = ctx.allow_lds((const void *)k_reduce2_q<U, true>, (int)(2 * RED2_TPB * sizeof(QRec<U>))))) return rc;

        StageTimer timer(ws, !buckets_only || time_range);
        ws.timed = timer.on;
        timer.mark(T_DECOMPOSE, stream);
        const uint8_t *skip = nullptr;
        const void *upoints = nullptr;
        bool forked = false;
        if (resident) {
            upoints = (const char *)(shared ? resident->tables.ptr : resident->upoints.ptr) + resident_offset * AFF_BYTES;
            skip = (const uint8_t *)resident->skip.ptr + resident_offset;
        } else {
            if ((rc = ws.upoints.ensure((glv ? 2 : 1) * n_points * AFF_BYTES))) return rc;
            forked = n_points >= FORK_CONVERT_MIN;
            if (forked && (rc = ws.side_stream(ws.cstream))) return rc;
            hipStream_t cs = forked ? ws.cstream : stream;
            if (forked) {
                HIP_TRY(hipEventRecord(ws.ev_fork, stream));
                HIP_TRY(hipStreamWaitEvent(cs, ws.ev_fork, 0));
            }
            if (glv)
                hipLaunchKernelGGL((k_convert_points_glv<U, Consts>), dim3((unsigned)((n_points + 255) / 256)), dim3(256), 0,
                                   cs, d_points, n_points, ws.upoints.ptr);
            else
                hipLaunchKernelGGL((k_convert_points<U>), dim3((unsigned)((n_points + 255) / 256)), dim3(256), 0,
                                   cs, d_points, n_points, ws.upoints.ptr, (uint8_t *)nullptr);
            if (forked) {
                ws.conv_pending = true;
                HIP_TRY(hipEventRecord(ws.ev_conv, cs));
            }
            upoints = ws.upoints.ptr;
            skip = nullptr;
        }
        launch_decompose(d_scalars, n_points, plan, d16, ws.digits.ptr, skip, stream);

        const void *digits = ws.digits.ptr;
        uint32_t *sorted = (uint32_t *)ws.sorted.ptr, *parted = (uint32_t *)ws.parted.ptr, *starts = (uint32_t *)ws.starts.ptr;
        char *buckets = (char *)ws.buckets.ptr, *seg_partials = (char *)ws.seg_partials.ptr;
        uint32_t *seg_flags = (uint32_t *)ws.seg_flags.ptr, *seg_bucket = (uint32_t *)ws.seg_bucket.ptr;

        timer.mark(T_HIST, stream);
        if (d16)
            hipLaunchKernelGGL(k_part_hist<uint16_t>, dim3(pchunks, nw), dim3(1024), (size_t)nparts * 4, stream,
                               (const uint16_t *)digits, n, nparts, fbits, pchunk_len, bh);
        else
            hipLaunchKernelGGL(k_part_hist<uint32_t>, dim3(pchunks, nw), dim3(1024), (size_t)nparts * 4, stream,
                               (const uint32_t *)digits, n, nparts, fbits, pchunk_len, bh);
        timer.mark(T_SCAN, stream);
        if ((size_t)((nparts + 31) / 32) * nw < (size_t)ctx.num_cus && pchunks >= 256)
            hipLaunchKernelGGL(k_part_colscan<32>, dim3((nparts + 31) / 32, nw), dim3(1024), 0, stream, bh, pchunks, nparts, part_pop, hcount + 2 * nw);
        else
            hipLaunchKernelGGL(k_part_colscan<8>, dim3((nparts + 31) / 32, nw), dim3(256), 0, stream, bh, pchunks, nparts, part_pop, hcount + 2 * nw);
        hipLaunchKernelGGL(k_part_rowscan, dim3(nw), dim3(1024), 0, stream, part_pop, nparts, part_base, long_flag, stage_cap, hparts,
                           hcount, hcap);
        timer.mark(T_SCATTER, stream);
        {
            const dim3 grid(pchunks, nw), block(1024);
#define GMSM_SCATTER(D, CH)                                                                                              \
    hipLaunchKernelGGL((k_part_scatter<D, CH>), grid, block, scatter_lds, stream, (const D *)digits, n, nparts, fbits, lidx, \
                       pchunk_len, bh, part_base, parted)
            if (d16 && !big_chunk) GMSM_SCATTER(uint16_t, PART_CHUNK);
            else if (d16) GMSM_SCATTER(uint16_t, PART_CHUNK_BIG);
            else if (!big_chunk) GMSM_SCATTER(uint32_t, PART_CHUNK);
            else GMSM_SCATTER(uint32_t, PART_CHUNK_BIG);
#undef GMSM_SCATTER
        }
        if (stage_cap <= 24u * 1024u)
            hipLaunchKernelGGL(k_fine_sort<24>, dim3(nparts, nw), dim3(1024), ((size_t)4 << fbits) + (size_t)stage_cap * 4, stream,
                               parted, n, NB, fbits, lidx, part_base, sorted, starts, stage_cap);
        else
            hipLaunchKernelGGL(k_fine_sort<40>, dim3(nparts, nw), dim3(1024), ((size_t)4 << fbits) + (size_t)stage_cap * 4, stream,
                               parted, n, NB, fbits, lidx, part_base, sorted, starts, stage_cap);
        if (n > stage_cap) {
            hipLaunchKernelGGL(k_heavy_hist, dim3(heavy_wg), dim3(1024), (size_t)4 << fbits, stream, parted, n, nw, nparts, fbits, lidx,
                               part_base, (const HeavyPart *)hparts, (const uint32_t *)hcount, hcap, scap, subhist);
            hipLaunchKernelGGL(k_heavy_scan, dim3(std::min<uint32_t>(hcap, 64u), nw), dim3(1024), (size_t)4 << fbits, stream, nparts, NB, fbits,
                               part_base, (const HeavyPart *)hparts, (const uint32_t *)hcount, hcap, scap, subhist, starts);
            hipLaunchKernelGGL(k_heavy_place, dim3(heavy_wg), dim3(1024), (size_t)4 << fbits, stream, parted, n, nw, nparts, fbits, lidx,
                               part_base, (const HeavyPart *)hparts, (const uint32_t *)hcount, hcap, scap, (const uint32_t *)subhist, sorted);
        }
        if (forked) {
            HIP_TRY(hipStreamWaitEvent(stream, ws.ev_conv, 0));
            ws.conv_pending = false;
        }
        const auto accumulate = [&](uint32_t k0, uint32_t nk, hipStream_t st) {
            const uint32_t *st_g = starts + (size_t)k0 * (NB + 1);
            const uint32_t *sorted_g = sorted + (size_t)k0 * n;
            char *buckets_g = buckets + (size_t)k0 * NB * REC, *part_g = seg_partials + (size_t)k0 * qa.tpw * 2 * REC;
            if (shared)
                hipLaunchKernelGGL((k_accumulate_seg<U, true>), dim3((qa.tpw + 255) / 256, nk), dim3(256), 0, st, upoints, n, NB,
                                   qa.seg, st_g, sorted_g, buckets_g, part_g, seg_flags + (size_t)k0 * qa.tpw, seg_bucket + (size_t)k0 * qa.tpw,
                                   qa.tpw, (uint32_t)n_points, (uint32_t)resident->n);
            else
                hipLaunchKernelGGL((k_accumulate_seg<U, false>), dim3((qa.tpw + 255) / 256, nk), dim3(256), 0, st, upoints, n, NB,
                                   qa.seg, st_g, sorted_g, buckets_g, part_g, seg_flags + (size_t)k0 * qa.tpw, seg_bucket + (size_t)k0 * qa.tpw,
                                   qa.tpw, 0u, 0u);
        };
        const auto fixup_and_reduce = [&](uint32_t k0, uint32_t nk, size_t list_off, hipStream_t st, bool mark) {
            const uint32_t *st_g = starts + (size_t)k0 * (NB + 1);
            char *buckets_g = buckets + (size_t)k0 * NB * REC, *part_g = seg_partials + (size_t)k0 * qa.tpw * 2 * REC;
            const uint32_t *flags_g = seg_flags + (size_t)k0 * qa.tpw, *pb_g = seg_bucket + (size_t)k0 * qa.tpw;
            uint32_t *cnt_g = long_flag + k0;
            LongChain *list_g = long_list + list_off;
            uint32_t *done_g = piece_done + list_off;
            void *sums_g = (char *)piece_sums + list_off * REC;
            if (shared && n / NB >= 2 * (size_t)qa.seg)
                hipLaunchKernelGGL((k_fixup_bucket<OpsSerial>), dim3((NB + 255) / 256, nk), dim3(256), 0, st, NB, st_g, qa.seg,
                                   (const void *)part_g, qa.tpw, (void *)buckets_g, cnt_g, list_g, done_g, FIX_MAXWALK);
            else if constexpr (FIXUP_QUAD)
                hipLaunchKernelGGL((k_fixup_seg_q<U>), dim3((qa.tpw + 63) / 64, nk), dim3(256), 128 * sizeof(QRec<U>), st, NB,
                                   (const void *)part_g, flags_g, pb_g, qa.tpw, (void *)buckets_g, cnt_g, list_g, done_g, FIX_MAXWALK, st_g, qa.seg);
            else
                hipLaunchKernelGGL((k_fixup_seg<OpsSerial>), dim3((qa.tpw + 255) / 256, nk), dim3(256), 0, st, NB, part_g, flags_g, pb_g,
                                   qa.tpw, buckets_g, cnt_g, list_g, done_g, FIX_MAXWALK, st_g, qa.seg);
            hipLaunchKernelGGL((k_fixup_long<U>), dim3(2 * ctx.num_cus), dim3(256), 128 * sizeof(QRec<U>), st, NB, part_g, pb_g, qa.tpw,
                               buckets_g, (const uint32_t *)cnt_g, (const LongChain *)list_g, done_g, sums_g, st_g, qa.seg);
            if (mark) timer.mark(T_REDUCE, st);
            if (!buckets_only) enqueue_reduce_kernels(ctx, ws, q, T, buckets_g, st_g, nk, NB, st, k0);
        };
        timer.mark(T_ACCUMULATE, stream);
        if (!split) {
            accumulate(0, nw, stream);
            timer.mark(T_FIXUP, stream);
            fixup_and_reduce(0, nw, 0, stream, true);
        } else {
            const uint32_t ha = nw / 2;
            if ((rc = ws.side_stream(ws.mstream))) return rc;
            accumulate(0, ha, stream);
            HIP_TRY(hipEventRecord(ws.ev_buckets, stream));
            HIP_TRY(hipStreamWaitEvent(ws.mstream, ws.ev_buckets, 0));
            fixup_and_reduce(0, ha, 0, ws.mstream, false);
            HIP_TRY(hipEventRecord(ws.ev_merged, ws.mstream));
            accumulate(ha, nw - ha, stream);
            timer.mark(T_FIXUP, stream);
            fixup_and_reduce(ha, nw - ha, list_cap / 2, stream, true);
            HIP_TRY(hipStreamWaitEvent(stream, ws.ev_merged, 0));
        }
        if (!buckets_only && nwd > nw)
            hipLaunchKernelGGL((k_fill_infinity<Ext>), dim3((nwd - nw + 63) / 64), dim3(64), 0, stream, ws.totals.ptr, nw, nwd - nw);
        timer.mark(T_END, stream);
        HIP_TRY(hipGetLastError());
        if (!buckets_only) {
            if (d_out)
                HIP_TRY(hipMemcpyAsync(d_out, ws.totals.ptr, (size_t)nwd * sizeof(Ext), hipMemcpyDeviceToDevice, stream));
            else
                HIP_TRY(hipMemcpyAsync(ws.pinned, ws.totals.ptr, (size_t)nwd * sizeof(Ext), hipMemcpyDeviceToHost, stream));
        }
        if ((rc = end_use(ws, stream))) return rc;
        ws.pending_timed = timer.on;
        return GMSM_OK;
    }

    static uint32_t reduce2_active(uint32_t nlast) {
        uint32_t active = 2;
        while (active < nlast) active <<= 1;
        return active;
    }
    static void reduce_shape(const Context &ctx, uint32_t nw, uint32_t NB, uint32_t out[6]) {
        const Geometry q = plan_geometry(ctx, nw, NB, NB);
        out[0] = q.log2L;
        out[1] = q.nblocks1;
        out[2] = q.nblocks2;
        out[3] = use_combine_we(ctx, q.nblocks1 * nw) ? 2u : 1u;
        out[4] = SERIAL_QUAD ? 1u : 0u;
        out[5] = reduce2_active(q.nblocks2 ? q.nblocks2 : q.nblocks1);
    }

    static void enqueue_reduce_kernels(Context &ctx, Workspace &ws, const Geometry &q, uint32_t T, const void *buckets,
                                       const uint32_t *starts, uint32_t nw, uint32_t NB, hipStream_t stream,
                                       uint32_t k0 = 0 ) {
        constexpr size_t RECB = sizeof(typename OpsSerial::Mem);
        void *red_pre = (char *)ws.red_pre.ptr + (size_t)k0 * T * 2 * RECB;
        void *partials = (char *)ws.partials.ptr + (size_t)k0 * q.nblocks1 * 2 * RECB;
        void *totals = (char *)ws.totals.ptr + (size_t)k0 * sizeof(Ext);
        const uint32_t prescale = q.log2span;
        if constexpr (SERIAL_QUAD)
            hipLaunchKernelGGL((k_reduce_serial_q<U, SERIAL_Q_QUADS>), dim3((T + SERIAL_Q_QUADS - 1) / SERIAL_Q_QUADS, nw), dim3(4 * SERIAL_Q_QUADS),
                               3 * SERIAL_Q_QUADS * sizeof(QRec<U>), stream, buckets, NB, q.log2L, T, starts, red_pre);
        else
            hipLaunchKernelGGL((k_reduce_serial<OpsSerial>), dim3((T + 255) / 256, nw), dim3(256), 0, stream, buckets, NB,
                               q.log2L, T, starts, red_pre);
        const auto combine = [&](const void *in, uint32_t pairs, void *out, uint32_t blocks, uint32_t l2, uint32_t pre) {
            if constexpr (COMBINE_WE) {
                if (use_combine_we(ctx, blocks * nw)) {
                    hipLaunchKernelGGL((k_combine_we<U, true>), dim3(blocks, nw), dim3(4 * COMBINE_N),
                                       (2 * COMBINE_N + 1) * sizeof(QRec<U>), stream, l2, out, pre, in, pairs);
                    return;
                }
            }
            hipLaunchKernelGGL((k_combine_q<U, true, COMBINE_N>), dim3(blocks, nw), dim3(4 * COMBINE_N),
                               (2 * COMBINE_N + 1) * sizeof(QRec<U>), stream, l2, out, pre, in, pairs);
        };
        combine(red_pre, T, partials, q.nblocks1, q.log2L, prescale);
        const void *last = partials;
        uint32_t nlast = q.nblocks1, rest = q.log2span - prescale;
        if (q.nblocks2) {
            constexpr size_t REC = sizeof(typename OpsSerial::Mem);
            void *out2 = (char *)partials + (size_t)nw * q.nblocks1 * 2 * REC;
            uint32_t lgN = 0;
            for (size_t t = COMBINE_N; t > 1; t >>= 1) ++lgN;
            combine(partials, q.nblocks1, out2, q.nblocks2, 0, lgN);
            last = out2;
            nlast = q.nblocks2;
            rest = 0;
        }
        const uint32_t active = reduce2_active(nlast);
        hipLaunchKernelGGL((k_reduce2_q<U, true>), dim3(nw), dim3(4 * active), 2 * active * sizeof(QRec<U>), stream, last, nlast,
                           rest, active, totals);
        (void)ctx;
    }

    static int enqueue_reduce(Context &ctx, Workspace &ws, const void *buckets, const WindowPlan &plan, size_t n_for_geometry,
                              hipStream_t stream) {
        const uint32_t nw = bucket_sets(plan), nwd = plan.nwin_local, NB = plan.nbuckets;
        constexpr size_t REC = sizeof(typename OpsSerial::Mem);
        const Geometry q = plan_geometry(ctx, nw, n_for_geometry, NB);
        const uint32_t T = (uint32_t)(((size_t)NB + ((size_t)1 << q.log2L) - 1) >> q.log2L);
        int rc;
        if ((rc = ws.partials.ensure((size_t)nw * (q.nblocks1 + q.nblocks2) * 2 * REC))) return rc;
        if ((rc = ws.red_pre.ensure((size_t)nw * T * 2 * REC))) return rc;
        if ((rc = ws.totals.ensure((size_t)nwd * sizeof(Ext)))) return rc;
        if ((rc = ws.ensure_pinned((size_t)nwd * sizeof(Ext)))) return rc;
        if ((rc = ctx.allow_lds((const void *)k_combine_q<U, true, COMBINE_N>, (int)((2 * COMBINE_N + 1) * sizeof(QRec<U>))))) return rc;
        if constexpr (COMBINE_WE)
            if ((rc = ctx.allow_lds((const void *)k_combine_we<U, true>, (int)((2 * COMBINE_N + 1) * sizeof(QRec<U>))))) return rc;
        if constexpr (SERIAL_QUAD)
            if ((rc = ctx.allow_lds((const void *)k_reduce_serial_q<U, SERIAL_Q_QUADS>, (int)(3 * SERIAL_Q_QUADS * sizeof(QRec<U>))))) return rc;
        if ((rc = ctx.allow_lds((const void *)k_reduce2_q<U, true>, (int)(2 * RED2_TPB * sizeof(QRec<U>))))) return rc;
        enqueue_reduce_kernels(ctx, ws, q, T, buckets, nullptr, nw, NB, stream);
        if (nwd > nw)
            hipLaunchKernelGGL((k_fill_infinity<Ext>), dim3((nwd - nw + 63) / 64), dim3(64), 0, stream, ws.totals.ptr, nw, nwd - nw);
        HIP_TRY(hipGetLastError());
        HIP_TRY(hipMemcpyAsync(ws.pinned, ws.totals.ptr, (size_t)nwd * sizeof(Ext), hipMemcpyDeviceToHost, stream));
        return GMSM_OK;
    }

    static int normalize_records(Workspace &ws, size_t n, void *d_out) {
        int rc;
        if ((rc = ws.partials.ensure(n * sizeof(U)))) return rc;
        constexpr int K = 32;
        const size_t threads = (n + K - 1) / K;
        hipLaunchKernelGGL((k_batch_normalize<U, INLINE_OPS, K>), dim3((unsigned)((threads + 63) / 64)), dim3(64), 0, ws.stream,
                           ws.buckets.ptr, n, (U *)ws.partials.ptr, d_out);
        HIP_TRY(hipGetLastError());
        return GMSM_OK;
    }

    static int batch_scalar_mul(Context &ctx, Workspace &ws, const uint64_t *base_limbs, const void *d_scalars, size_t n,
                                void *d_out) {
        if (n == 0) return GMSM_OK;
        Aff base;
        memcpy(&base, base_limbs, sizeof base);
        if (base.is_infinity()) {
            HIP_TRY(hipMemsetAsync(d_out, 0, n * AFF_BYTES, ws.stream));
            return GMSM_OK;
        }
        const unsigned forced_c = options().fixed_base_bits.load(std::memory_order_relaxed);
        const unsigned c = forced_c ? forced_c : n < ((size_t)1 << 21) ? 8 : 11;
        const WindowPlan plan = make_plan(c, 0, 1);
        std::vector<Aff> table;
        build_fixed_base_table(base, plan.c, plan.nwin_total, plan.nbuckets, (int)std::min<unsigned>(16, usable_cpus()), table);
        int rc;
        const size_t tn = table.size();
        if ((rc = ws.h2d_points.ensure(tn * AFF_BYTES))) return rc;
        if ((rc = ws.upoints.ensure(tn * AFF_BYTES))) return rc;
        if ((rc = ws.skip.ensure(tn))) return rc;
        if ((rc = ws.buckets.ensure(n * sizeof(XYZZL<U>)))) return rc;
        HIP_TRY(hipMemcpyAsync(ws.h2d_points.ptr, table.data(), tn * AFF_BYTES, hipMemcpyHostToDevice, ws.stream));
        hipLaunchKernelGGL((k_convert_points<U>), dim3((unsigned)((tn + 255) / 256)), dim3(256), 0, ws.stream,
                           ws.h2d_points.ptr, tn, ws.upoints.ptr, (uint8_t *)ws.skip.ptr);
        hipLaunchKernelGGL((k_fixed_base<U, FrP, INLINE_OPS>), dim3((unsigned)((n + 255) / 256)), dim3(256), 0, ws.stream,
                           (const uint32_t *)d_scalars, n, plan, ws.upoints.ptr, ws.buckets.ptr);
        HIP_TRY(hipGetLastError());
        if ((rc = normalize_records(ws, n, d_out))) return rc;
        HIP_TRY(hipStreamSynchronize(ws.stream));
        (void)ctx;
        return GMSM_OK;
    }

    static int batch_jac_to_affine(Workspace &ws, const void *d_jac, size_t n, void *d_out) {
        if (n == 0) return GMSM_OK;
        int rc;
        if ((rc = ws.buckets.ensure(n * sizeof(XYZZL<U>)))) return rc;
        hipLaunchKernelGGL((k_jac_to_recs<U, INLINE_OPS>), dim3((unsigned)((n + 255) / 256)), dim3(256), 0, ws.stream, d_jac, n,
                           ws.buckets.ptr);
        HIP_TRY(hipGetLastError());
        return normalize_records(ws, n, d_out);
    }

    static constexpr bool LAGRANGE_GLV = GMSM_LAGRANGE_GLV != 0;
    static int to_lagrange(Workspace &ws, const void *d_in, bool packed, unsigned log2n, void *d_out) {
        static_assert(std::is_same<U, FpU<typename LzTraits<U>::Params>>::value, "ToLagrangeG1: coordinates in Fp");
        using Tw = WalkScalar<FrP, LAGRANGE_GLV>;
        using Fld = FftField<FrP>;
        using Fr = Fp<FrP>;
        constexpr size_t REC = sizeof(XYZZL<U>);
        const size_t n = (size_t)1 << log2n, half = n / 2;
        const size_t tab_recs = LAGRANGE_GLV ? 3 * n : 0;
        const size_t tw_off = (n + tab_recs) * REC;
        int rc;
        if ((rc = ws.lagrange.ensure(tw_off + (n + 1) * sizeof(Tw)))) return rc;
// ... 273 lines not shown

    static unsigned device_ranges(size_t n, const WindowPlan &plan) {
        size_t run = max_run_points(plan);
        if (AFF_BYTES == 64 && !plan.shared && options().max_run.load(std::memory_order_relaxed) == 0) run = std::min<size_t>(run, (size_t)1 << 24);
        unsigned nr = (unsigned)((n + run - 1) / run);
        const unsigned forced = GMSM_TUNE(DEVICE_RANGES, 0);
        if (forced > nr) nr = (unsigned)std::min<size_t>(forced, n);
        return nr;
    }

    static constexpr uint32_t SMALL_SL = SmallSlice<U>::value;
    static constexpr bool SMALL_QUAD_ONLY = SmallQuadOnly<U>::value;
    static size_t small_max_points() {
        const size_t forced = options().small_max.load(std::memory_order_relaxed);
        return std::min<size_t>(forced ? forced : GMSM_TUNE(SMALL_MAX, sizeof(U) <= 36 ? 8192 : sizeof(U) <= 72 ? 4096 : 1024),
                                small_entry_cap() / 2);
    }
    static constexpr size_t small_entry_cap() {
        return SMALL_QUAD_ONLY ? (size_t)SMALL_QUAD_ENTRIES * SMALL_QUAD_MAX_CHUNKS * SMALL_MAX_SLICES : (size_t)SMALL_SL * SMALL_MAX_SLICES;
    }
    static bool small_glv() { return options().glv.load(std::memory_order_relaxed) >= 1; }
    static WindowPlan small_make_plan(unsigned c, bool glv) { return glv ? make_plan_glv(c, 0, 1) : make_plan(c, 0, 1); }
    static unsigned small_c(size_t n, bool glv) {
        const unsigned forced = options().small_bits.load(std::memory_order_relaxed);
        const size_t entries = glv ? 2 * n : n;
        unsigned c = (forced >= 2 && forced <= SMALL_MAX_C) ? forced
                     : FR_BITS > 300 ? (entries <= 512 ? 6 : 7)
                                     : entries <= 256 ? 5 : entries <= 4096 ? 6 : 7;
        while (c > 2 && small_make_plan(c, glv).nbuckets > SMALL_NB_MAX) --c;
        return c;
    }
    static bool small_serves(size_t n, const ResidentBases *rb) {
        if (options().small_bits.load(std::memory_order_relaxed) == 1) return false;
        if (options().window_bits.load(std::memory_order_relaxed) != 0) return false;
        if (small_shared(n, rb)) return true;
        return n >= 1 && n <= small_max_points() && !use_tables(rb, n);
    }
    static bool small_shared(size_t n, const ResidentBases *rb) {
        if (!rb || n < 1 || options().tables.load(std::memory_order_relaxed) == 0) return false;
        const unsigned c = rb->small_c.load(std::memory_order_acquire);
        if (c == 0 || n > rb->small_m) return false;
        const unsigned forced = options().small_bits.load(std::memory_order_relaxed);
        if (forced >= 2 && forced != c) return false;
        return n * rb->small_nw <= (size_t)SMALL_SL * SMALL_SHARED_MAX_SLICES;
    }
    struct SmallPlan {
        WindowPlan plan;
        bool shared, glv, quad;
        uint32_t chunks, nslices;
    };
    static SmallPlan small_plan(size_t n, const ResidentBases *rb) {
        SmallPlan sp;
        sp.shared = small_shared(n, rb);
        sp.glv = !sp.shared && small_glv();
        sp.plan = sp.shared ? make_plan(rb->small_c.load(), 0, 1) : small_make_plan(small_c(n, sp.glv), sp.glv);
        const size_t entries = sp.shared ? n * sp.plan.nwin_total : (sp.glv ? 2 * n : n);
        const unsigned fq = options().small_quad.load(std::memory_order_relaxed);
        const size_t wgs64 = (entries + SMALL_QUAD_ENTRIES - 1) / SMALL_QUAD_ENTRIES * (sp.shared ? 1 : sp.plan.nwin_total);
        sp.quad = SMALL_QUAD_ONLY || fq == 2 || (fq == 0 && wgs64 <= (size_t)GMSM_TUNE(SMALL_QUAD_WGS, 512));
        if (sp.quad) {
            const size_t max_slices = sp.shared ? SMALL_SHARED_MAX_SLICES : SMALL_MAX_SLICES;
            size_t chunks = 1;
            while ((entries + chunks * SMALL_QUAD_ENTRIES - 1) / (chunks * SMALL_QUAD_ENTRIES) > max_slices) chunks *= 2;
            const size_t nsets = sp.shared ? 1 : sp.plan.nwin_total, resident_wgs = SMALL_QUAD_ONLY ? 256 : 768;
            while (chunks < SMALL_QUAD_MAX_CHUNKS &&
                   (entries + chunks * SMALL_QUAD_ENTRIES - 1) / (chunks * SMALL_QUAD_ENTRIES) * nsets > resident_wgs &&
                   entries > chunks * SMALL_QUAD_ENTRIES)
                chunks *= 2;
            sp.chunks = (uint32_t)chunks;
            sp.nslices = (uint32_t)((entries + chunks * SMALL_QUAD_ENTRIES - 1) / (chunks * SMALL_QUAD_ENTRIES));
        } else {
            sp.chunks = 0;
            sp.nslices = (uint32_t)((entries + SMALL_SL - 1) / SMALL_SL);
        }
        return sp;
    }
    static int enqueue_small(Context &ctx, Workspace &ws, const void *d_points, const void *d_scalars, size_t n,
                             const SmallPlan &sp, const ResidentBases *resident) {
        const WindowPlan &plan = sp.plan;
        const uint32_t nw = sp.shared ? 1u : plan.nwin_total;
        constexpr size_t REC = sizeof(typename OpsSerial::Mem);
        int rc;
        ws.pending_timed = false;
        if ((rc = begin_use(ws, ws.stream))) return rc;
        if ((rc = ws.ensure_pinned((size_t)plan.nwin_total * sizeof(Ext)))) return rc;
        if ((rc = ws.small_sums.ensure((size_t)nw * sp.nslices * REC))) return rc;
        if ((rc = ws.small_done.ensure((size_t)HEAVY_MAX_WINDOWS * 4))) return rc;
        if (sp.nslices > 1) HIP_TRY(hipMemsetAsync(ws.small_done.ptr, 0, (size_t)nw * 4, ws.stream));
        SmallArgs a;
        a.points = d_points;
        a.upoints = nullptr;
        a.skip = nullptr;
        if (d_points == nullptr) {
            a.upoints = sp.shared ? resident->small_tables.ptr : resident->upoints.ptr;
            a.skip = (const uint8_t *)resident->skip.ptr;
        }
        a.scalars = (const uint32_t *)d_scalars;
        a.n = (uint32_t)n;
        a.glv = sp.glv ? 1u : 0u;
        a.tab_m = sp.shared ? (uint32_t)resident->small_m : 0u;
        a.chunks = sp.chunks;
        a.slice_sums = ws.small_sums.ptr;
        a.done = (uint32_t *)ws.small_done.ptr;
        a.totals = ws.pinned;
        g_small_runs.fetch_add(1, std::memory_order_relaxed);
        if (sp.shared) g_table_runs.fetch_add(1, std::memory_order_relaxed);
        StageTimer timer(ws, true);
        ws.timed = timer.on;
        if (timer.on) {
            ws.timed_level = 2;
            (void)hipEventRecord(ws.events[T_ACCUMULATE], ws.stream);
        }
        const dim3 grid(sp.nslices, nw);
        if (sp.quad) {
            const size_t lds = (size_t)192 * sizeof(QRec<U>);
            if (sp.shared) {
                if ((rc = ctx.allow_lds((const void *)k_msm_small_q<U, FrP, Consts, true>, (int)lds))) return rc;
                hipLaunchKernelGGL((k_msm_small_q<U, FrP, Consts, true>), grid, dim3(256), lds, ws.stream, a, plan);
            } else {
                if ((rc = ctx.allow_lds((const void *)k_msm_small_q<U, FrP, Consts, false>, (int)lds))) return rc;
                hipLaunchKernelGGL((k_msm_small_q<U, FrP, Consts, false>), grid, dim3(256), lds, ws.stream, a, plan);
            }
        } else {
            if constexpr (!SMALL_QUAD_ONLY) {
                const size_t lds = (size_t)SMALL_SL * REC;
                if (sp.shared) {
                    if ((rc = ctx.allow_lds((const void *)k_msm_small<U, FrP, Consts, SMALL_SL, true>, (int)lds))) return rc;
                    hipLaunchKernelGGL((k_msm_small<U, FrP, Consts, SMALL_SL, true>), grid, dim3(SMALL_SL), lds, ws.stream, a, plan);
                } else {
                    if ((rc = ctx.allow_lds((const void *)k_msm_small<U, FrP, Consts, SMALL_SL, false>, (int)lds))) return rc;
                    hipLaunchKernelGGL((k_msm_small<U, FrP, Consts, SMALL_SL, false>), grid, dim3(SMALL_SL), lds, ws.stream, a, plan);
                }
            }
        }
        HIP_TRY(hipGetLastError());
        if (timer.on) (void)hipEventRecord(ws.events[T_FIXUP], ws.stream);
        ws.pending_timed = timer.on;
        return end_use(ws, ws.stream);
    }
    static int collect_small(Workspace &ws, const SmallPlan &sp, J *out) {
        if (sp.shared) {
            Ext total;
            int rc = collect_window_sums(ws, ws.stream, 1, &total);
            if (rc) return rc;
            *out = total.zz.is_zero() ? J{F::one(), F::one(), F::zero()} : jac_from_xyzz(total);
            return GMSM_OK;
        }
        std::vector<Ext> totals(sp.plan.nwin_total);
        int rc = collect_window_sums(ws, ws.stream, sp.plan.nwin_total, totals.data());
        if (rc) return rc;
        *out = fold(totals.data(), sp.plan.c, sp.plan.nwin_total);
        return GMSM_OK;
    }
    static int multiexp_small(Context &ctx, Workspace &ws, const void *d_points, const void *d_scalars, size_t n,
                              hipStream_t caller_stream, J *out, const ResidentBases *resident) {
        const SmallPlan sp = small_plan(n, d_points ? nullptr : resident);
        if (sp.plan.nwin_total > HEAVY_MAX_WINDOWS) return fail(GMSM_ERR_ARG, "small path: too many windows");
        int rc = order_after(ws, caller_stream);
        if (rc) return rc;
        if ((rc = enqueue_small(ctx, ws, d_points, d_scalars, n, sp, resident))) return rc;
        return collect_small(ws, sp, out);
    }

    static int multiexp_device(Context &ctx, Workspace &ws, const void *d_points, const void *d_scalars, size_t n,
                               hipStream_t caller_stream, J *out, const ResidentBases *resident = nullptr) {
        if (small_serves(n, resident)) return multiexp_small(ctx, ws, d_points, d_scalars, n, caller_stream, out, resident);
        const WindowPlan plan = plan_for(resident, n);
        const unsigned c = plan.c;
        const unsigned nr = device_ranges(n, plan);
        std::vector<Ext> totals(plan.nwin_total);
        if (nr <= 1) {
            int rc = window_sums(ctx, ws, d_points, d_scalars, n, plan, caller_stream, totals.data(), resident);
            if (rc) return rc;
            *out = fold(totals.data(), c, plan.nwin_total);
            return GMSM_OK;
        }
        constexpr size_t REC = sizeof(typename OpsSerial::Mem);
        const size_t per = (n + nr - 1) / nr;
        int rc = order_after(ws, caller_stream);
        if (rc) return rc;
        if ((rc = ws.carry.ensure((size_t)bucket_sets(plan) * plan.nbuckets * REC))) return rc;
        const bool prof = profiling_level() != 0;
        float pms[STAGE_COUNT] = {0};
        unsigned plaunch[STAGE_COUNT] = {0};
        for (unsigned r = 0; r * per < n; ++r) {
            const size_t lo = (size_t)r * per, len = std::min(per, n - lo);
            const void *dp = d_points ? (const char *)d_points + lo * AFF_BYTES : nullptr;
            if ((rc = enqueue_window_sums(ctx, ws, dp, (const char *)d_scalars + lo * SCALAR_BYTES, len, plan, ws.stream, resident,
                                          nullptr, lo, true, prof)))
                return rc;
            if (prof && ws.pending_timed) {
                HIP_TRY(wait_stream(ws.stream));
                StageTimer::collect_add(ws, pms, plaunch);
                ws.pending_timed = false;
            }
            hipLaunchKernelGGL((k_merge_buckets<OpsSerial>), dim3((plan.nbuckets + 255) / 256, bucket_sets(plan)), dim3(256), 0, ws.stream,
                               ws.carry.ptr, (const void *)ws.buckets.ptr, (const uint32_t *)ws.starts.ptr, plan.nbuckets, r == 0 ? 1 : 0);
        }
        if ((rc = enqueue_reduce(ctx, ws, ws.carry.ptr, plan, per, ws.stream))) return rc;
        if ((rc = collect_window_sums(ws, ws.stream, plan.nwin_local, totals.data()))) return rc;
        if (prof) record_stage_times(pms, plaunch);
        *out = fold(totals.data(), c, plan.nwin_total);
        return GMSM_OK;
    }

    static int multiexp_submit(Context &ctx, Workspace &ws, const void *d_scalars, size_t n, const ResidentBases *resident) {
        if (n > max_run_points())
            return fail(GMSM_ERR_ARG, "submit/collect takes at most 2^27 points per ticket: use the blocking entry, which splits larger inputs");
        WindowPlan plan = plan_for(resident, n);
        if (n > max_run_points(plan)) plan = make_plan(choose_c(FR_BITS, AFF_BYTES, n), 0, 1);
        const unsigned c = plan.c;
        int rc = enqueue_window_sums(ctx, ws, nullptr, d_scalars, n, plan, ws.stream, resident);
        if (rc) return rc;
        ws.pending_c = c;
        ws.pending_nw = plan.nwin_total;
        return GMSM_OK;
    }
    static int multiexp_collect(Workspace &ws, J *out) {
        std::vector<Ext> totals(ws.pending_nw);
        int rc = collect_window_sums(ws, ws.stream, ws.pending_nw, totals.data());
        if (rc) return rc;
        *out = fold(totals.data(), ws.pending_c);
        return GMSM_OK;
    }


    static unsigned host_ranges(size_t n, bool with_points) {
        const unsigned forced = options().host_ranges.load(std::memory_order_relaxed);
        if (forced) return (unsigned)std::min<size_t>(forced, std::max<size_t>(1, n));
        if (with_points) {
            if (n < ((size_t)1 << 19)) return 1;
            if (n < ((size_t)1 << 23)) return (unsigned)std::min<size_t>(8, n >> 18);
            return 16;
        }
        if (n < ((size_t)1 << 20)) return 1;
        if (SKEWED_HOST_RANGES) return (unsigned)std::min<size_t>(8, std::max<size_t>(3, n >> 21));
        return (unsigned)std::min<size_t>(16, std::max<size_t>(2, n >> 20));
    }

    static int window_sums_from_host(Context &ctx, Workspace &first, const uint64_t *points, const ResidentBases *resident,
                                     size_t resident_base, const uint64_t *scalars, size_t n, const WindowPlan &plan,
                                     unsigned nr, Ext *out_totals) {
        const uint32_t nw = plan.nwin_local, nsets = bucket_sets(plan);
        if (nw == 0) return GMSM_OK;
        const size_t per = (n + nr - 1) / nr;
        std::vector<size_t> cut(nr + 1, 0);
        {
            const bool skew = SKEWED_HOST_RANGES && points == nullptr && nr >= 3 && options().host_ranges.load(std::memory_order_relaxed) == 0;
            std::vector<double> wgt(nr, 1.0);
            if (skew) {
                wgt[0] = 0.5;
                if (nr >= 4) wgt[nr - 1] = 0.5;
            }
            double tot = 0, run = 0;
            for (double v : wgt) tot += v;
            bool ok = true;
            for (unsigned r = 0; r < nr; ++r) {
                run += wgt[r];
                cut[r + 1] = r + 1 == nr ? n : (size_t)((double)n * run / tot);
                if (cut[r + 1] <= cut[r] || cut[r + 1] - cut[r] > max_run_points(plan)) ok = false;
            }
            if (!ok)
                for (unsigned r = 0; r <= nr; ++r) cut[r] = std::min(n, (size_t)r * per);
        }
        Workspace *w[2] = {&first, nr > 1 ? ctx.acquire(false) : nullptr};
        const unsigned nws = w[1] ? 2 : 1;
        constexpr size_t REC = sizeof(typename OpsSerial::Mem);
        int rc = GMSM_OK;
        if (nws == 2 && (rc = first.side_stream(first.mstream))) {
            ctx.release(w[1]);
            return rc;
        }
        hipStream_t ms = nws == 2 ? first.mstream : first.stream;
        if (nr > 1 && (rc = first.carry.ensure((size_t)nsets * plan.nbuckets * REC))) {
            if (w[1]) ctx.release(w[1]);
            return rc;
        }
        for (unsigned r = 0; r < nr && rc == GMSM_OK; ++r) {
            Workspace &ws = *w[r % nws];
            const size_t lo = cut[r], len = cut[r + 1] - lo;
            const void *dp = nullptr;
            if ((rc = ws.h2d_scalars.ensure(len * SCALAR_BYTES))) break;
            if (hipMemcpyAsync(ws.h2d_scalars.ptr, (const char *)scalars + lo * SCALAR_BYTES, len * SCALAR_BYTES,
                               hipMemcpyHostToDevice, ws.stream) != hipSuccess) {
                rc = fail(GMSM_ERR_DEVICE, "hipMemcpyAsync(scalars) failed");
                break;
            }
            if (points) {
                if ((rc = ws.h2d_points.ensure(len * AFF_BYTES))) break;
                if (hipMemcpyAsync(ws.h2d_points.ptr, (const char *)points + lo * AFF_BYTES, len * AFF_BYTES,
                                   hipMemcpyHostToDevice, ws.stream) != hipSuccess) {
                    rc = fail(GMSM_ERR_DEVICE, "hipMemcpyAsync(points) failed");
                    break;
                }
                dp = ws.h2d_points.ptr;
            }
            if (nr == 1) {
                rc = enqueue_window_sums(ctx, ws, dp, ws.h2d_scalars.ptr, len, plan, ws.stream, resident, nullptr, resident_base + lo);
                break;
            }
            hipError_t he = hipSuccess;
            if (nws == 2 && r >= 2) he = hipStreamWaitEvent(ws.stream, ws.ev_merged, 0);
            if (he != hipSuccess) {
                rc = fail(GMSM_ERR_DEVICE, std::string("hipStreamWaitEvent: ") + hipGetErrorString(he));
                break;
            }
// ... 99 lines not shown
```

gnark-crypto_amd/csrc/gmsm_group_host.h:

```cpp
#pragma once
#include <algorithm>
#include <cstring>
#include <thread>
#include <vector>

#include "gmsm_context.h"
#include "gmsm_curve.h"

namespace gmsm {

template <class F_, class FrP_>
struct GroupHost {
    using F = F_;
    using FrP = FrP_;
    using Aff = Affine<F>;
    using Ext = XYZZ<F>;
    using J = Jac<F>;
    static constexpr unsigned FR_BITS = FrP::BITS;

    static J fold_sets(const Ext *sets, unsigned nsets, unsigned c) {
        const unsigned nwin = num_windows(FR_BITS, c);
        std::vector<Ext> totals(sets, sets + nwin);
        for (unsigned s = 1; s < nsets; ++s)
            for (unsigned w = 0; w < nwin; ++w) xyzz_add(totals[w], sets[(size_t)s * nwin + w]);
        return fold(totals.data(), c);
    }

    static J fold(const Ext *totals, unsigned c, unsigned nwin = 0 ) {
        if (nwin == 0) nwin = num_windows(FR_BITS, c);
        J acc = jac_from_xyzz(totals[nwin - 1]);
        for (int j = (int)nwin - 2; j >= 0; --j) {
            if (!acc.z.is_zero())
                for (unsigned l = 0; l < c; ++l) acc = jac_double(acc);
            if (totals[j].zz.is_zero()) continue;
            Ext e = acc.z.is_zero() ? Ext::infinity() : xyzz_from_jac(acc);
            xyzz_add(e, totals[j]);
            acc = jac_from_xyzz(e);
        }
        if (acc.z.is_zero()) acc = J{F::one(), F::one(), F::zero()};
        return acc;
    }

    static Ext scalar_mul(const Aff &a, const uint64_t *k, int klimbs) {
        Ext acc = Ext::infinity();
        for (int i = klimbs * 64 - 1; i >= 0; --i) {
            acc = xyzz_double(acc);
            if ((k[i / 64] >> (i % 64)) & 1) xyzz_add_mixed(acc, a, false);
        }
        return acc;
    }
    static void batch_to_affine(Aff *out, const Ext *in, size_t count, F *scratch) {
        F acc = F::one();
        for (size_t i = 0; i < count; ++i) {
            scratch[i] = acc;
            if (!in[i].zzz.is_zero()) acc = fp_mul(acc, in[i].zzz);
        }
        F inv = fp_inv(acc);
        for (size_t i = count; i-- > 0;) {
            if (in[i].zzz.is_zero()) {
                out[i] = Aff{F::zero(), F::zero()};
                continue;
            }
            F zi = fp_mul(inv, scratch[i]);
            inv = fp_mul(inv, in[i].zzz);
            F izz = fp_mul(fp_mul(fp_sqr(zi), in[i].zz), in[i].zz);
            out[i].x = fp_mul(in[i].x, izz);
            out[i].y = fp_mul(in[i].y, zi);
        }
    }
    static void generate_points(const uint64_t *base_limbs, const uint64_t *k0, const uint64_t *k1, int klimbs, size_t n,
                                int nthreads, uint64_t *out_limbs) {
        Aff base;
        memcpy(&base, base_limbs, sizeof base);
        Aff *out = reinterpret_cast<Aff *>(out_limbs);
        Aff step;
        {
            Ext s = scalar_mul(base, k1, klimbs);
            F scratch;
            batch_to_affine(&step, &s, 1, &scratch);
        }
        if (nthreads < 1) nthreads = 1;
        const size_t per = (n + (size_t)nthreads - 1) / (size_t)nthreads;
        std::vector<std::thread> th;
        for (int t = 0; t < nthreads; ++t) {
            const size_t s = (size_t)t * per, e = std::min(n, s + per);
            if (s >= e) break;
            th.emplace_back([=, &base, &step]() {
                constexpr size_t BLK = 1024;
                std::vector<Ext> blk(BLK);
                std::vector<F> scr(BLK);
                Ext cur = scalar_mul(base, k0, klimbs);
                uint64_t s64 = (uint64_t)s;
                Ext off = scalar_mul(step, &s64, 1);
                xyzz_add(cur, off);
                for (size_t i = s; i < e;) {
                    const size_t cnt = std::min(BLK, e - i);
                    for (size_t k = 0; k < cnt; ++k) {
                        blk[k] = cur;
                        xyzz_add_mixed(cur, step, false);
                    }
                    batch_to_affine(out + i, blk.data(), cnt, scr.data());
                    i += cnt;
                }
            });
        }
        for (auto &t : th) t.join();
    }

    static void build_fixed_base_table(const Aff &base, uint32_t c, uint32_t nwin, uint32_t nb, int nthreads, std::vector<Aff> &table) {
        table.resize((size_t)nwin * nb);
        std::vector<Aff> win_base(nwin);
        {
            std::vector<Ext> wb(nwin);
            Ext cur = Ext::infinity();
            xyzz_add_mixed(cur, base, false);
            for (uint32_t j = 0; j < nwin; ++j) {
                wb[j] = cur;
                for (uint32_t l = 0; l < c; ++l) cur = xyzz_double(cur);
            }
            std::vector<F> scr(nwin);
            batch_to_affine(win_base.data(), wb.data(), nwin, scr.data());
        }
        if (nthreads < 1) nthreads = 1;
// ... 32 lines not shown
```

gnark-crypto_amd/csrc/gmsm_group_vtable.h:

```cpp
#pragma once
#include "gmsm_group.h"
#include "gmsm_group_debug.h"

namespace gmsm {


template <class G, bool IS_G1>
struct VTableOf {
    static int multiexp_host(const uint64_t *points, size_t n_points, const uint64_t *scalars, size_t n_scalars,
                             int nb_tasks, uint64_t *out_jac) {
        typename G::J j;
        int rc = G::multiexp_host(points, n_points, scalars, n_scalars, nb_tasks, &j);
        if (rc) return rc;
        memcpy(out_jac, &j, sizeof j);
        return GMSM_OK;
    }
    static int multiexp_device(Context &ctx, const void *d_points, const void *d_scalars, size_t n, hipStream_t stream,
                               uint64_t *out_jac, const ResidentBases *resident) {
        typename G::J j;
        if (n == 0) j = typename G::J{G::F::one(), G::F::one(), G::F::zero()};
        else {
            GMSM_LEASE_OR_FAIL(lease, ctx);
            int rc = G::multiexp_device(ctx, *lease.w, d_points, d_scalars, n, stream, &j, resident);
            if (rc) return rc;
// ... 58 lines not shown
        const void *dsc;
        if ((rc = stage_input(ws, ws.h2d_scalars, scalars, d_scalars, n * G::SCALAR_BYTES, {After::NOTHING}, &dsc))) return rc;
        void *dres = d_out;
        if (out && n) {
            if ((rc = ws.parted.ensure(n * G::AFF_BYTES))) return rc;
            dres = ws.parted.ptr;
        }
        if ((rc = G::batch_scalar_mul(ctx, ws, base, dsc, n, dres))) return rc;
        if (out && n) HIP_TRY(hipMemcpyAsync(out, dres, n * G::AFF_BYTES, hipMemcpyDeviceToHost, ws.stream));
        HIP_TRY(hipStreamSynchronize(ws.stream));
        return GMSM_OK;
    }
    static int batch_jac_to_affine(Context &ctx, const uint64_t *jac, size_t n, uint64_t *out) {
        if (n == 0) return GMSM_OK;
        GMSM_LEASE_OR_FAIL(lease, ctx);
        Workspace &ws = *lease.w;
        int rc;
        if ((rc = ws.h2d_points.ensure(n * sizeof(typename G::J)))) return rc;
        if ((rc = ws.parted.ensure(n * G::AFF_BYTES))) return rc;
        HIP_TRY(hipMemcpyAsync(ws.h2d_points.ptr, jac, n * sizeof(typename G::J), hipMemcpyHostToDevice, ws.stream));
        if ((rc = G::batch_jac_to_affine(ws, ws.h2d_points.ptr, n, ws.parted.ptr))) return rc;
        HIP_TRY(hipMemcpyAsync(out, ws.parted.ptr, n * G::AFF_BYTES, hipMemcpyDeviceToHost, ws.stream));
        HIP_TRY(hipStreamSynchronize(ws.stream));
        return GMSM_OK;
    }
    static int submit(Context &ctx, Workspace &ws, const void *d_scalars, size_t n, const ResidentBases *resident) {
        return G::multiexp_submit(ctx, ws, d_scalars, n, resident);
    }
    static int decode_raw(Workspace &ws, const void *d_raw, size_t n, int level, void *d_out, long long *bad_index,
                          uint32_t *status) {
        return G::decode_raw(ws, d_raw, n, level, d_out, bad_index, status);
    }
    static int decode_compressed(Workspace &ws, const void *d_comp, size_t n, int level, void *d_out, long long *bad_index,
                                 uint32_t *status) {
        return G::decode_compressed(ws, d_comp, n, level, d_out, bad_index, status);
    }
    static int encode_compressed(Workspace &ws, const void *d_points, size_t n, void *d_comp) {
        return G::encode_compressed(ws, d_points, n, d_comp);
    }
    static int fft_domain_new(Context &ctx, hipStream_t stream, unsigned log2n, FftDomain *out) {
        return FftField<typename G::FrP>::domain_new(ctx, stream, log2n, out);
    }
    static int fft_run(hipStream_t stream, FftDomain *d, void *d_a, bool inverse, bool dif, bool coset) {
        return FftField<typename G::FrP>::run(stream, d, d_a, inverse, dif, coset);
    }
    static int fft_bit_reverse(hipStream_t stream, void *d_a, size_t n) {
        return FftField<typename G::FrP>::bit_reverse(stream, d_a, n);
    }
    static int validate_points(Workspace &ws, const void *d_points, size_t n, int level, long long *bad_index,
                               uint32_t *status) {
        return G::validate_points(ws, d_points, n, level, bad_index, status);
    }
    static int collect(Workspace &ws, uint64_t *out_jac) {
        typename G::J j;
        int rc = G::multiexp_collect(ws, &j);
        if (rc) return rc;
        memcpy(out_jac, &j, sizeof j);
        return GMSM_OK;
    }
    static void fold(const uint64_t *xyzz_windows, unsigned c, uint64_t *out_jac) {
        typename G::J j = G::fold(reinterpret_cast<const typename G::Ext *>(xyzz_windows), c);
        memcpy(out_jac, &j, sizeof j);
    }
    static void jac_to_affine(const uint64_t *jac, uint64_t *out_affine) {
        typename G::J j;
        memcpy(&j, jac, sizeof j);
        typename G::Aff a = affine_from_jac(j);
        memcpy(out_affine, &a, sizeof a);
    }
    static int debug_decompose(const uint64_t *scalars, size_t n, unsigned c, uint32_t *out_digits) {
        return debug_decompose_impl<G>(scalars, n, c, out_digits);
    }
    static int debug_glv_split(const uint64_t *scalars, size_t n, uint32_t *out) { return debug_glv_split_impl<G>(scalars, n, out); }
    static void plan_info(size_t n, unsigned *c, unsigned *nwin, unsigned *entries_per_point, unsigned *fused) {
        if (G::small_serves(n, nullptr)) {
            const typename G::SmallPlan sp = G::small_plan(n, nullptr);
            *c = sp.plan.c, *nwin = sp.plan.nwin_total, *entries_per_point = sp.glv ? 2u : 1u, *fused = 1u;
            return;
        }
        const WindowPlan p = G::plan_for(nullptr, n);
        *c = p.c, *nwin = p.nwin_total, *entries_per_point = p.glv ? 2u : 1u, *fused = 0u;
    }
    static void reduce_shape(const Context &ctx, uint32_t nw, uint32_t nbuckets, uint32_t out[6]) { G::reduce_shape(ctx, nw, nbuckets, out); }
    static int debug_field_op(int field, int op, const uint64_t *a, const uint64_t *b, size_t count, uint64_t *out) {
        using BaseP = typename G::F::Params;
        if (field == 0) {
            if (op == 6) return debug_from_mont<BaseP>(a, count, out);
            return debug_field<Fp<BaseP>>(op, a, b, count, out);
        } else if (field == 1) {
            if (op == 6) return debug_from_mont<typename G::FrP>(a, count, out);
            return debug_field<Fp<typename G::FrP>>(op, a, b, count, out);
        }
        if (op == 6) return fail(GMSM_ERR_ARG, "from_mont is defined on prime fields only");
        if (field == 3) {
            using U = typename G::U;
            using S = typename LzTraits<U>::Sat;
            return run_elementwise<S>(count * sizeof(S), a, b ? count * sizeof(S) : 0, b, count * sizeof(S), out,
                                      [&](void *da, void *db, void *dout, hipStream_t s) {
                                          hipLaunchKernelGGL((k_lazy_field_op<U>), dim3((unsigned)((count + 63) / 64)), dim3(64),
                                                             0, s, op, (const S *)da, (const S *)db, count, (S *)dout);
                                      });
        }
        return debug_field<typename G::F>(op, a, b, count, out);
    }
    static int debug_group_op(int op, const uint64_t *acc, const uint64_t *other, size_t count, uint64_t *out) {
        if (op >= 4) {
            using U = typename G::U;
            using F = typename G::F;
            const int lop = op - 4;
            const size_t ob = (lop == 0 || lop == 1) ? sizeof(Affine<F>) : sizeof(XYZZ<F>);
            return run_elementwise<F>(count * sizeof(XYZZ<F>), acc, other ? count * ob : 0, other, count * sizeof(XYZZ<F>), out,
                                      [&](void *da, void *db, void *dout, hipStream_t s) {
                                          hipLaunchKernelGGL((k_lazy_group_op<U>), dim3((unsigned)((count + 63) / 64)), dim3(64),
                                                             0, s, lop, (const XYZZ<F> *)da, (const void *)db, count,
                                                             (XYZZ<F> *)dout);
                                      });
        }
        return debug_group<G>(op, acc, other, count, out);
    }
    static void generate_points(const uint64_t *base, const uint64_t *k0, const uint64_t *k1, int klimbs, size_t n,
                                int nthreads, uint64_t *out) {
        G::generate_points(base, k0, k1, klimbs, n, nthreads, out);
    }
    using PF = PolyField<typename G::FrP>;
    using Fr = Fp<typename G::FrP>;
    static_assert(sizeof(Fr) == G::SCALAR_BYTES, "fr.Element layout");
    static int poly_input(Workspace &ws, const uint64_t *polys, const void *d_polys, size_t total, hipStream_t caller, const Fr **out) {
        const void *in;
        int rc = stage_input(ws, ws.h2d_scalars, polys, d_polys, total * sizeof(Fr), {After::STREAM, caller}, &in);
        *out = (const Fr *)in;
        return rc;
    }
    static size_t word_slots(size_t words) { return (words * 8 + sizeof(Fr) - 1) / sizeof(Fr); }
    static size_t poly_scratch(const size_t *lens, size_t k, unsigned lanes) {
        size_t s = 0;
        for (size_t i = 0; i < k; ++i) s = std::max(s, PF::scratch_elems(lens[i], lanes));
        return s;
    }
    static int poly_eval(Context &ctx, const uint64_t *polys, const void *d_polys, const size_t *lens, size_t k, const uint64_t *point,
                         hipStream_t caller, uint64_t *out_values) {
        GMSM_LEASE_OR_FAIL(lease, ctx);
        Workspace &ws = *lease.w;
        size_t total = 0;
        for (size_t i = 0; i < k; ++i) total += lens[i];
        const Fr *in;
        int rc = poly_input(ws, polys, d_polys, total, caller, &in);
        if (rc) return rc;
        const unsigned lanes = PF::lane_option();
        if ((rc = ws.poly.ensure((k + poly_scratch(lens, k, lanes)) * sizeof(Fr)))) return rc;
        Fr *vals = (Fr *)ws.poly.ptr, *scratch = vals + k;
        const FftPowers<typename G::FrP> pw = PF::powers_of(point);
        for (size_t i = 0, off = 0; i < k; off += lens[i], ++i)
            if ((rc = PF::suffix(ws.stream, pw, in + off, lens[i], nullptr, vals + i, scratch, lanes))) return rc;
        HIP_TRY(hipMemcpyAsync(out_values, vals, k * sizeof(Fr), hipMemcpyDeviceToHost, ws.stream));
        HIP_TRY(hipStreamSynchronize(ws.stream));
        return GMSM_OK;
    }
    static int poly_div(Context &ctx, const uint64_t *poly, const void *d_poly, size_t n, const uint64_t *point, hipStream_t caller,
                        uint64_t *out_h, void *d_out_h, uint64_t *out_value) {
        GMSM_LEASE_OR_FAIL(lease, ctx);
        Workspace &ws = *lease.w;
        const Fr *in;
        int rc = poly_input(ws, poly, d_poly, n, caller, &in);
        if (rc) return rc;
        if (d_out_h && poly && (rc = order_after(ws, caller))) return rc;
        const size_t hbuf = out_h ? n - 1 : 0;
// ... 258 lines not shown
    static int ratio_copy(Context &ctx, FftDomain *d, const uint64_t *entries, const void *d_entries, size_t m, const uint32_t *layouts,
                          const int64_t *perm, const void *d_perm, const uint64_t *beta, const uint64_t *gamma, int basis, int layout,
                          hipStream_t caller, uint64_t *out, void *d_out) {
        GMSM_LEASE_OR_FAIL(lease, ctx);
        Workspace &ws = *lease.w;
        const size_t n = (size_t)1 << d->log2n;
        const Fr *in;
        const void *pm;
        int rc = poly_input(ws, entries, d_entries, m * n, caller, &in);
        if (rc || (rc = stage_input(ws, ws.h2d_points, perm, d_perm, m * n * 8, {After::STREAM, caller}, &pm))) return rc;
        if (d_out && entries && perm && (rc = order_after(ws, caller))) return rc;
        const size_t lay_slots = word_slots((m + 1) / 2);
        RatioBuffers b;
        if ((rc = ratio_buffers(ws, n, m + lay_slots + 1, &b))) return rc;
        Fr *bg = b.tail;
        uint32_t *lay = (uint32_t *)(bg + m);
        unsigned long long *bad = (unsigned long long *)(bg + m + lay_slots);
        Fr bt, gm;
        memcpy(&bt, beta, sizeof bt);
        memcpy(&gm, gamma, sizeof gm);
        std::vector<Fr> table(m);
        RF::coset_table(d, bt, m, table.data());
        const unsigned long long none = ~0ull;
        unsigned long long first_bad = none;
        DrainOnExit drain{ws.stream};
        HIP_TRY(hipMemcpyAsync(bg, table.data(), m * sizeof(Fr), hipMemcpyHostToDevice, ws.stream));
        HIP_TRY(hipMemcpyAsync(lay, layouts, m * sizeof(uint32_t), hipMemcpyHostToDevice, ws.stream));
        HIP_TRY(hipMemcpyAsync(bad, &none, sizeof none, hipMemcpyHostToDevice, ws.stream));
        ratio_settle_events(ws);
        StageTimer timer(ws, true);
        timer.mark(T_DECOMPOSE, ws.stream);
        hipLaunchKernelGGL((k_ratio_factors_copy<typename G::FrP>), dim3((unsigned)((n + 255) / 256)), dim3(256), 0, ws.stream, in,
                           (const uint32_t *)lay, m, n, d->log2n, (const long long *)pm, (const Fr *)d->twiddles_lz.ptr, (const Fr *)bg, gm, b.fnum,
                           b.fden, bad);
        HIP_TRY(hipGetLastError());
        if ((rc = ratio_finish(ws, timer, d, b, n, basis, layout, out, d_out, d_perm ? bad : nullptr, &first_bad))) return rc;
        if (first_bad != none) {
            long long v = 0;
            HIP_TRY(hipMemcpy(&v, (const long long *)d_perm + first_bad, sizeof v, hipMemcpyDeviceToHost));
            return fail(GMSM_ERR_ARG, ratio_perm_error((size_t)first_bad, v, m * n));
        }
        return GMSM_OK;
    }
    static int ratio_shuffled(Context &ctx, FftDomain *d, const uint64_t *num, const void *d_num, const uint64_t *den, const void *d_den,
                              size_t m, const uint32_t *num_layouts, const uint32_t *den_layouts, const uint64_t *beta, int basis, int layout,
                              hipStream_t caller, uint64_t *out, void *d_out) {
        GMSM_LEASE_OR_FAIL(lease, ctx);
        Workspace &ws = *lease.w;
        const size_t n = (size_t)1 << d->log2n;
        const Fr *pn;
        const void *pd;
        int rc = poly_input(ws, num, d_num, m * n, caller, &pn);
        if (rc || (rc = stage_input(ws, ws.h2d_points, den, d_den, m * n * sizeof(Fr), {After::STREAM, caller}, &pd))) return rc;
        if (d_out && num && den && (rc = order_after(ws, caller))) return rc;
        RatioBuffers b;
        if ((rc = ratio_buffers(ws, n, word_slots(m), &b))) return rc;
        uint32_t *lay = (uint32_t *)b.tail;
        Fr bt;
        memcpy(&bt, beta, sizeof bt);
        DrainOnExit drain{ws.stream};
        HIP_TRY(hipMemcpyAsync(lay, num_layouts, m * sizeof(uint32_t), hipMemcpyHostToDevice, ws.stream));
        HIP_TRY(hipMemcpyAsync(lay + m, den_layouts, m * sizeof(uint32_t), hipMemcpyHostToDevice, ws.stream));
        ratio_settle_events(ws);
        StageTimer timer(ws, true);
        timer.mark(T_DECOMPOSE, ws.stream);
        hipLaunchKernelGGL((k_ratio_factors_shuffled<typename G::FrP>), dim3((unsigned)((n + 255) / 256)), dim3(256), 0, ws.stream, pn,
                           (const Fr *)pd, (const uint32_t *)lay, m, n, d->log2n, bt, b.fnum, b.fden);
        HIP_TRY(hipGetLastError());
        return ratio_finish(ws, timer, d, b, n, basis, layout, out, d_out, nullptr, nullptr);
    }
    static const GroupVTable *get() {
        static const GroupVTable vt = [] {
            GroupVTable v{};
            v.fr_bits = G::FR_BITS, v.fr_max_order = (unsigned)G::FrP::MAX_ORDER;
            v.aff_bytes = G::AFF_BYTES, v.scalar_bytes = G::SCALAR_BYTES, v.jac_bytes = sizeof(typename G::J), v.xyzz_bytes = sizeof(typename G::Ext);
#define GMSM_VT(f) v.f = &f
            GMSM_VT(multiexp_host), GMSM_VT(multiexp_device), GMSM_VT(window_sums), GMSM_VT(fold), GMSM_VT(jac_to_affine);
            GMSM_VT(debug_decompose), GMSM_VT(debug_field_op), GMSM_VT(debug_group_op), GMSM_VT(generate_points);
            GMSM_VT(register_bases), GMSM_VT(submit), GMSM_VT(collect), GMSM_VT(window_sums_enqueue), GMSM_VT(fold_sets), GMSM_VT(fold_powers);
            GMSM_VT(multiexp_bases_host), GMSM_VT(batch_scalar_mul), GMSM_VT(batch_jac_to_affine);
            GMSM_VT(decode_raw), GMSM_VT(validate_points), GMSM_VT(decode_compressed), GMSM_VT(encode_compressed);
            GMSM_VT(fft_domain_new), GMSM_VT(fft_run), GMSM_VT(fft_bit_reverse);
            GMSM_VT(precompute_tables), GMSM_VT(tables_serve), GMSM_VT(shard_piece), GMSM_VT(host_piece_ranges);
            GMSM_VT(debug_glv_split), GMSM_VT(plan_info), GMSM_VT(reduce_shape);
            GMSM_VT(poly_eval), GMSM_VT(poly_div), GMSM_VT(kzg_open);
            if constexpr (IS_G1) GMSM_VT(to_lagrange);
            GMSM_VT(fflonk_next_divisor), GMSM_VT(open_check), GMSM_VT(fflonk_fold);
            if constexpr (IS_G1) GMSM_VT(open_w), GMSM_VT(open_wprime);
            GMSM_VT(batch_scale), GMSM_VT(linear_combinations);
            if constexpr (IS_G1) GMSM_VT(fr_batch_invert), GMSM_VT(ratio_copy), GMSM_VT(ratio_shuffled);
#undef GMSM_VT
            return v;
        }();
        return &vt;
    }
};

}
```

gnark-crypto_amd/csrc/gmsm_quad.h:

```cpp
#pragma once
#include "gmsm_curveu.h"

namespace gmsm {

#if defined(__HIPCC__)

__device__ __forceinline__ void quad_lds_fence() { __builtin_amdgcn_fence(__ATOMIC_ACQ_REL, "wavefront"); }

template <class U>
struct QRec {
    U c[4];
    uint32_t inf;
    uint32_t pad[3];
};

template <class U> struct QF;
template <class P>
struct QF<FpU<P>> {
    using F = FpU<P>;
    template <bool INL> __device__ static __forceinline__ F mul(const F &a, const F &b) { return fmul<INL>(a, b); }
    __device__ static __forceinline__ F sub4(const F &a, const F &b) { return fpu_sub<P, 4>(a, b); }
    __device__ static __forceinline__ F sub16(const F &a, const F &b) { return fpu_sub<P, 16>(a, b); }
    __device__ static __forceinline__ F dbl(const F &a) { return fpu_dbl(a); }
    __device__ static __forceinline__ F triple(const F &a) { return fpu_add(fpu_add(a, a), a); }
// ... 192 lines not shown
    if (t < 4) {
        using T = LzTraits<U>;
        using Mem = XYZZ<typename T::Sat>;
        typename T::Sat *dst = reinterpret_cast<typename T::Sat *>(reinterpret_cast<char *>(window_totals) + (size_t)k * sizeof(Mem));
        typename T::Sat v = T::template to_sat<INL>(W[0].c[t]);
        if (W[0].inf) {
            const Mem inf = Mem::infinity();
            v = t == 0 ? inf.x : t == 1 ? inf.y : t == 2 ? inf.zz : inf.zzz;
        }
        dst[t] = v;
    }
}

template <class U, bool INL, int N>
__global__ void __launch_bounds__(4 * N) k_combine_q(uint32_t log2L, void *__restrict__ out1, uint32_t prescale,
                                                     const void *__restrict__ pre, uint32_t T) {
    extern __shared__ __align__(16) unsigned char lds_raw[];
    QRec<U> *S = reinterpret_cast<QRec<U> *>(lds_raw), *W = S + N, *PARK = S + 2 * N;
    const uint32_t k = blockIdx.y, blk = blockIdx.x, t = threadIdx.x, j = t >> 2, lane = t & 63u;
    const uint32_t g = blk * N + j;
    quad_rec_load<U>(&S[j], pre, ((size_t)k * T + g) * 2 + 0, g < T, lane);
    quad_rec_load<U>(&W[j], pre, ((size_t)k * T + g) * 2 + 1, g < T, lane);
    __syncthreads();
    constexpr uint32_t LG = N == 64 ? 6 : N == 32 ? 5 : N == 16 ? 4 : N == 128 ? 7 : 0;
    static_assert(LG != 0, "N must be 16, 32, 64 or 128");
#pragma nounroll
    for (uint32_t s = 0; s < LG; ++s) {
        const uint32_t d = 1u << s;
        const bool act = j + d < (uint32_t)N;
        const QAddOps<U> o = quad_add_load<U>(&S[j], &S[act ? j + d : j], lane);
        __syncthreads();
        quad_add_store<U, INL>(&S[j], o, act, lane);
        __syncthreads();
    }
    if (j == 0) {
        PARK->c[t & 3u] = S[0].c[t & 3u];
        if ((t & 3u) == 0) {
            PARK->inf = S[0].inf;
            S[0].inf = 1u;
        }
    }
    __syncthreads();
    const bool upper = j >= (uint32_t)N / 2;
    const uint32_t jj = upper ? j - N / 2 : j;
    QRec<U> *arr = upper ? W : S;
    uint32_t dbl_left = prescale;
    const uint32_t n_tree = LG, n_fin = log2L + 1;
#pragma nounroll
    for (uint32_t s = 0; s < n_tree + n_fin; ++s) {
        bool act = false, fin_dbl = false;
        QRec<U> *X = &arr[jj], *Y = &arr[jj];
        if (s < n_tree) {
            const uint32_t d = (uint32_t)N >> (s + 1);
            if (d >= 1 && jj < d) {
                act = true;
                Y = &arr[jj + d];
            }
        } else if (s < n_tree + n_fin) {
            const uint32_t step = s - n_tree;
            if (j == 0) {
                if (step < log2L) fin_dbl = true;
                else {
                    act = true;
                    X = &W[0];
                    Y = &S[0];
                }
            }
        }
        const bool park_dbl = j == (uint32_t)N - 1 && s >= 1 && dbl_left > 0;
        const QAddOps<U> o = quad_add_load<U>(X, Y, lane);
        __syncthreads();
        quad_add_store<U, INL>(X, o, act, lane);
        if (fin_dbl && !S[0].inf) quad_dbl_inplace<U, INL>(&S[0], lane);
        if (park_dbl) {
            if (!PARK->inf) quad_dbl_inplace<U, INL>(PARK, lane);
        }
        if (s >= 1 && dbl_left > 0) --dbl_left;
        __syncthreads();
    }
    if (j == 0) quad_rec_store<U>(out1, ((size_t)k * gridDim.x + blk) * 2 + 1, &W[0], lane);
    if (j == 1) quad_rec_store<U>(out1, ((size_t)k * gridDim.x + blk) * 2 + 0, PARK, lane);
}

template <class U, bool INL>
__global__ void __launch_bounds__(256) k_combine_we(uint32_t log2L, void *__restrict__ out1, uint32_t prescale,
                                                    const void *__restrict__ pre, uint32_t T) {
    constexpr uint32_t N = 64;
    extern __shared__ __align__(16) unsigned char lds_raw[];
    QRec<U> *S = reinterpret_cast<QRec<U> *>(lds_raw), *W = S + N, *PARK = S + 2 * N;
    const uint32_t k = blockIdx.y, blk = blockIdx.x, t = threadIdx.x, j = t >> 2, lane = t & 63u;
    const uint32_t g0 = blk * N + j;
    quad_rec_load<U>(&S[j], pre, ((size_t)k * T + g0) * 2 + 0, g0 < T, lane);
    quad_rec_load<U>(&W[j], pre, ((size_t)k * T + g0) * 2 + 1, g0 < T, lane);
    __syncthreads();
#pragma nounroll
    for (uint32_t s = 1; s <= 6; ++s) {
        const uint32_t g = 32u >> (s - 1), G = j / g, i = j % g;
        const bool act = G <= s;
        QRec<U> *X = &S[0], *Y = &S[0];
        if (G == 0) {
            const uint32_t l = s - 1;
            X = &S[(2 * i) << l];
            Y = &S[(2 * i + 1) << l];
        } else if (G < s) {
            const uint32_t l = G - 1;
            X = &S[(2 * i + 1) << l];
            Y = &S[(2 * (i + g) + 1) << l];
        } else if (G == s) {
            X = &W[i];
            Y = &W[i + g];
        }
        const QAddOps<U> o = quad_add_load<U>(X, Y, lane);
        __syncthreads();
        quad_add_store<U, INL>(X, o, act, lane);
        __syncthreads();
    }
    if (j == 0) {
        PARK->c[t & 3u] = S[0].c[t & 3u];
        if ((t & 3u) == 0) PARK->inf = S[0].inf;
    }
    __syncthreads();
    uint32_t dbl_left = prescale;
    const uint32_t n_tail = 7 + log2L + 1;
#pragma nounroll
    for (uint32_t s = 0; s < n_tail; ++s) {
        int op = 0;
        QRec<U> *X = &S[0], *Y = &S[0];
        if (j < 3) {
            if (s == 0) { op = 1; X = &S[2u << (2 * j)]; }
            else if (s == 1) { op = 2; X = &S[1u << (2 * j)]; Y = &S[2u << (2 * j)]; }
            else if (s == 2 || s == 3) { if (j >= 1) { op = 1; X = &S[j == 1 ? 4 : 16]; } }
            else if (s == 4) { if (j == 0) { op = 2; X = &S[1]; Y = &S[4]; } else if (j == 2) { op = 1; X = &S[16]; } }
            else if (s == 5) { if (j == 2) { op = 1; X = &S[16]; } }
            else if (s == 6) { if (j == 0) { op = 2; X = &S[1]; Y = &S[16]; } }
            else if (s < 7 + log2L) { if (j == 0) { op = 1; X = &S[1]; } }
            else if (j == 0) { op = 2; X = &W[0]; Y = &S[1]; }
        }
        const bool park_dbl = j == 15 && dbl_left > 0;
        const QAddOps<U> o = quad_add_load<U>(X, Y, lane);
        __syncthreads();
        quad_add_store<U, INL>(X, o, op == 2, lane);
        if (op == 1 && !X->inf) quad_dbl_inplace<U, INL>(X, lane);
        if (park_dbl && !PARK->inf) quad_dbl_inplace<U, INL>(PARK, lane);
        if (dbl_left > 0) --dbl_left;
        __syncthreads();
    }
    if (j == 0) quad_rec_store<U>(out1, ((size_t)k * gridDim.x + blk) * 2 + 1, &W[0], lane);
    if (j == 1) quad_rec_store<U>(out1, ((size_t)k * gridDim.x + blk) * 2 + 0, PARK, lane);
}

#endif

}
```

gnark-crypto_amd/multiexp.py:

```python
from dataclasses import dataclass

import numpy as np

from . import _lib
from .curves import CURVES

ERR_LEN = "len(points) != len(scalars)"
ERR_NBTASKS = "invalid config: config.NbTasks > 1024"


@dataclass
class MultiExpConfig:
    NbTasks: int = 0


def _ptr(a):
    return a.ctypes.data_as(_lib.ctypes.c_void_p)


SHARD_MODES = {"auto": 0, "points": 1, "windows": 2}


def _dev_array(devices):
    if not devices:
# ... 248 lines not shown
            rc = L.gmsm_points_validate(self.gid, None, d_points, n, level, _lib.ctypes.byref(bad))
        return (True, None) if rc == 0 else (False, self._error(rc))

    def register_bases_raw(self, buf, subgroup_check=True):
        L = _lib.load()
        raw = np.frombuffer(bytes(buf), dtype=np.uint8) if not isinstance(buf, np.ndarray) else np.ascontiguousarray(buf, dtype=np.uint8)
        if raw.size % self.raw_point_bytes:
            return None, "short buffer"
        n = raw.size // self.raw_point_bytes
        handle = _lib.ctypes.c_uint64(0)
        bad = _lib.ctypes.c_int64(-1)
        rc = L.gmsm_bases_register_raw(self.gid, _ptr(raw), n, 2 if subgroup_check else 0, _lib.ctypes.byref(handle),
                                       _lib.ctypes.byref(bad))
        return (ResidentBases(self, handle.value, n), None) if rc == 0 else (None, self._error(rc))

    def register_bases_dump(self, path, offset=0, expect_marker=True, max_points=0, check=0):
        L = _lib.load()
        handle = _lib.ctypes.c_uint64(0)
        n = _lib.ctypes.c_size_t(0)
        bad = _lib.ctypes.c_int64(-1)
        rc = L.gmsm_bases_register_dump(self.gid, str(path).encode(), offset, 1 if expect_marker else 0, max_points, check,
                                        _lib.ctypes.byref(handle), _lib.ctypes.byref(n), _lib.ctypes.byref(bad))
        return (ResidentBases(self, handle.value, n.value), None) if rc == 0 else (None, self._error(rc))

    def default_window_bits(self, n):
        return int(_lib.load().gmsm_default_window_bits(self.gid, n))

    def default_plan(self, n):
        v = [_lib.ctypes.c_uint(0) for _ in range(4)]
        rc = _lib.load().gmsm_default_plan(self.gid, n, *[_lib.ctypes.byref(x) for x in v])
        if rc:
            raise RuntimeError(self._error(rc))
        return {"window_bits": v[0].value, "windows": v[1].value, "entries_per_point": v[2].value, "fused": bool(v[3].value)}

    def reduce_shape(self, nw, nbuckets):
        v = (_lib.ctypes.c_uint32 * 6)()
        rc = _lib.load().gmsm_debug_reduce_shape(self.gid, nw, nbuckets, v)
        if rc:
            raise RuntimeError(self._error(rc))
        return {"log2L": v[0], "nblocks1": v[1], "nblocks2": v[2], "combine": v[3], "serial_quad": v[4], "active": v[5]}

    def num_windows(self, c):
        return int(_lib.load().gmsm_num_windows(self.gid, c))

    def window_sums_device(self, d_points, d_scalars, n, c, win_first=0, win_stride=1, stream=0):
        L = _lib.load()
        nwin = self.num_windows(c)
        nloc = max(0, (nwin - win_first + win_stride - 1) // win_stride) if win_first < nwin else 0
        out = np.zeros((nloc, self.xyzz_limbs), dtype=np.uint64)
        rc = L.gmsm_window_sums_device(self.gid, d_points, d_scalars, n, c, win_first, win_stride, stream or None, _ptr(out))
        if rc:
            raise RuntimeError(self._error(rc))
        return out

    def window_sums_enqueue(self, d_points, d_scalars, n, c, win_first, win_stride, stream, d_out, bases=None):
        L = _lib.load()
        rc = L.gmsm_window_sums_enqueue(self.gid, d_points, bases.handle if bases is not None else 0, d_scalars, n, c,
                                        win_first, win_stride, stream or None, d_out)
        if rc:
            raise RuntimeError(self._error(rc))

    def fold_window_sets(self, xyzz_sets, c):
        L = _lib.load()
        xyzz_sets = np.ascontiguousarray(xyzz_sets, dtype=np.uint64)
        nwin = self.num_windows(c)
        nsets = xyzz_sets.size // (nwin * self.xyzz_limbs)
        assert nsets >= 1 and xyzz_sets.size == nsets * nwin * self.xyzz_limbs
        out = np.zeros(self.jac_limbs, dtype=np.uint64)
        rc = L.gmsm_fold_window_sets(self.gid, c, _ptr(xyzz_sets), nsets, _ptr(out))
        if rc:
            raise RuntimeError(self._error(rc))
        return out

    def fold_windows(self, xyzz_windows, c):
        L = _lib.load()
        xyzz_windows = np.ascontiguousarray(xyzz_windows, dtype=np.uint64)
        assert xyzz_windows.size == self.num_windows(c) * self.xyzz_limbs
        out = np.zeros(self.jac_limbs, dtype=np.uint64)
        rc = L.gmsm_fold_windows(self.gid, c, _ptr(xyzz_windows), _ptr(out))
        if rc:
            raise RuntimeError(self._error(rc))
        return out

    def jac_to_affine(self, jac):
        L = _lib.load()
        jac = np.ascontiguousarray(jac, dtype=np.uint64)
        out = np.zeros(self.aff_limbs, dtype=np.uint64)
        rc = L.gmsm_jac_to_affine(self.gid, _ptr(jac), _ptr(out))
        if rc:
            raise RuntimeError(self._error(rc))
        return out


class ResidentBases:

    def __init__(self, group, handle, n):
        self.group, self.handle, self.n = group, handle, n

    def precompute(self, c=0):
        L = _lib.load()
        rc = L.gmsm_bases_precompute(self.handle, int(c))
        if rc:
            raise RuntimeError(self.group._error(rc))
        return int(L.gmsm_bases_table_bits(self.handle))

    @property
    def table_bits(self):
        return int(_lib.load().gmsm_bases_table_bits(self.handle))

    def to_lagrange(self, n=None):
        L = _lib.load()
        n = self.n if n is None else int(n)
        handle = _lib.ctypes.c_uint64(0)
        if L.gmsm_bases_to_lagrange(self.handle, n, _lib.ctypes.byref(handle)):
            raise ValueError(_lib.last_error())
        return ResidentBases(self.group, handle.value, n)

    def MultiExp(self, scalars, config=MultiExpConfig()):
        L = _lib.load()
        g = self.group
        scalars = np.ascontiguousarray(scalars, dtype=np.uint64).reshape(-1, g.fr_limbs)
        out = np.zeros(g.jac_limbs, dtype=np.uint64)
        rc = L.gmsm_multiexp_bases(self.handle, _ptr(scalars), scalars.shape[0], int(config.NbTasks), _ptr(out))
        return (out, None) if rc == 0 else (None, g._error(rc))

    def MultiExpSharded(self, scalars, config=MultiExpConfig(), mode="auto"):
        L = _lib.load()
        g = self.group
        scalars = np.ascontiguousarray(scalars, dtype=np.uint64).reshape(-1, g.fr_limbs)
        out = np.zeros(g.jac_limbs, dtype=np.uint64)
        rc = L.gmsm_multiexp_bases_sharded(self.handle, _ptr(scalars), scalars.shape[0], int(config.NbTasks),
                                           SHARD_MODES[mode], _ptr(out))
        return (out, None) if rc == 0 else (None, g._error(rc))

    def multiexp_device(self, d_scalars, n, stream=0):
        L = _lib.load()
        out = np.zeros(self.group.jac_limbs, dtype=np.uint64)
        rc = L.gmsm_multiexp_bases_device(self.handle, d_scalars, n, stream or None, _ptr(out))
        if rc:
            raise RuntimeError(self.group._error(rc))
        return out

    def MultiExpBatch(self, scalars=None, d_scalars=None, n=None, k=None, stream=0):
        L = _lib.load()
        g = self.group
        if scalars is not None:
            scalars = np.ascontiguousarray(scalars, dtype=np.uint64)
            k, n = scalars.shape[0], scalars.shape[1]
            scalars = scalars.reshape(k, n, g.fr_limbs)
        out = np.zeros((k, g.jac_limbs), dtype=np.uint64)
        rc = L.gmsm_multiexp_bases_batch(self.handle, _ptr(scalars) if scalars is not None and scalars.size else None,
                                         d_scalars, n, k, stream or None, _ptr(out))
        return (out, None) if rc == 0 else (None, g._error(rc))

    def submit(self, d_scalars, n, stream=0):
        import ctypes
        L = _lib.load()
        ticket = ctypes.c_uint64(0)
        rc = L.gmsm_multiexp_bases_submit(self.handle, d_scalars, n, stream or None, ctypes.byref(ticket))
        if rc:
            raise RuntimeError(self.group._error(rc))
        return ticket.value

    def collect(self, ticket):
        L = _lib.load()
        out = np.zeros(self.group.jac_limbs, dtype=np.uint64)
# ... 38 lines not shown
```

include/gmsm.h:

```cpp
#ifndef GMSM_H
#define GMSM_H

#include <stddef.h>
#include <stdint.h>

#ifdef __cplusplus
extern "C" {
#endif

#define GMSM_OK 0
#define GMSM_ERR_LEN 1
#define GMSM_ERR_CONFIG 2
#define GMSM_ERR_DEVICE 3
#define GMSM_ERR_ARG 4
#define GMSM_ERR_POINT 5

enum gmsm_group {
    GMSM_BN254_G1 = 0,
    GMSM_BN254_G2 = 1,
    GMSM_BLS12_381_G1 = 2,
    GMSM_BLS12_381_G2 = 3,
    GMSM_BW6_761_G1 = 4,
    GMSM_BW6_761_G2 = 5,
    GMSM_NUM_GROUPS = 6
// ... 63 lines not shown
int gmsm_points_compress(int group, const uint64_t *points, const void *d_points, size_t n, uint8_t *out_comp);
int gmsm_bases_register_compressed(int group, const uint8_t *comp, size_t n, int check, uint64_t *out_handle, int64_t *bad_index);
int gmsm_bases_register_dump(int group, const char *path, uint64_t offset, int expect_marker, size_t max_points, int check,
                             uint64_t *out_handle, size_t *out_n, int64_t *bad_index);

int gmsm_fft_domain_new(int group, uint64_t m, uint64_t *out_handle);
int gmsm_fft_domain_release(uint64_t handle);
int gmsm_fft_domain_info(uint64_t handle, uint64_t *cardinality, uint64_t *generator, uint64_t *generator_inv,
                         uint64_t *cardinality_inv, uint64_t *fr_multiplicative_gen, uint64_t *fr_multiplicative_gen_inv);
int gmsm_fft(uint64_t handle, uint64_t *a, void *d_a, size_t n, int inverse, int decimation, int on_coset, void *hip_stream);
int gmsm_fft_bit_reverse(int group, uint64_t *a, void *d_a, size_t n, void *hip_stream);

int gmsm_poly_eval(int group, const uint64_t *polys, const void *d_polys, const size_t *lens, size_t k, const uint64_t *point,
                   void *hip_stream, uint64_t *out_values);
int gmsm_poly_div_x_minus_a(int group, const uint64_t *poly, const void *d_poly, size_t n, const uint64_t *point,
                            void *hip_stream, uint64_t *out_h, void *d_out_h, uint64_t *out_value);
int gmsm_kzg_open(uint64_t handle, const uint64_t *poly, const void *d_poly, size_t n, const uint64_t *point,
                  void *hip_stream, uint64_t *out_claimed, uint64_t *out_h_jac);
int gmsm_kzg_open_folded(uint64_t handle, const uint64_t *polys, const void *d_polys, const size_t *lens, size_t k,
                         const uint64_t *point, const uint64_t *gamma, void *hip_stream, uint64_t *out_h_jac);

int gmsm_shplonk_open_w(uint64_t handle, const uint64_t *polys, const void *d_polys, const size_t *lens, size_t k,
                        const uint64_t *points, const size_t *npoints, const uint64_t *gamma, void *hip_stream,
                        uint64_t *out_claimed, uint64_t *out_w, void *d_out_w, uint64_t *out_w_jac);
int gmsm_shplonk_open_wprime(uint64_t handle, const uint64_t *polys, const void *d_polys, const size_t *lens, size_t k,
                             const uint64_t *points, const size_t *npoints, const uint64_t *claimed, const uint64_t *gamma,
                             const uint64_t *w, const void *d_w, const uint64_t *z, void *hip_stream, uint64_t *out_wprime_jac);

int gmsm_fflonk_next_divisor(int group, size_t n, size_t *out_t);
int gmsm_fflonk_fold(int group, const uint64_t *polys, const void *d_polys, const size_t *lens, size_t npolys, void *hip_stream,
                     uint64_t *out, void *d_out);
int gmsm_fflonk_fold_commit(uint64_t handle, const uint64_t *polys, const void *d_polys, const size_t *lens, size_t npolys,
                            void *hip_stream, void *d_out_folded, uint64_t *out_jac);
int gmsm_fflonk_open_w(uint64_t handle, const uint64_t *polys, const void *d_polys, const size_t *lens, const size_t *pack_sizes,
                       size_t k, const uint64_t *points, const size_t *npoints, const uint64_t *gamma, void *hip_stream,
                       uint64_t *out_claimed, uint64_t *out_folded_claimed, uint64_t *out_w, void *d_out_w, uint64_t *out_w_jac);
int gmsm_fflonk_open_wprime(uint64_t handle, const uint64_t *polys, const void *d_polys, const size_t *lens, const size_t *pack_sizes,
                            size_t k, const uint64_t *points, const size_t *npoints, const uint64_t *folded_claimed,
                            const uint64_t *gamma, const uint64_t *w, const void *d_w, const uint64_t *z, void *hip_stream,
                            uint64_t *out_wprime_jac);

int gmsm_to_lagrange_g1(int group, const uint64_t *coeffs, const void *d_coeffs, size_t n, void *hip_stream,
                        uint64_t *out_affine, void *d_out_affine);
int gmsm_bases_to_lagrange(uint64_t handle, size_t n, uint64_t *out_handle);

int gmsm_batch_scale(int group, const uint64_t *points, const void *d_points, size_t n,
                     const uint64_t *scalars, const void *d_scalars, size_t n_scalars,
                     void *hip_stream, uint64_t *out_affine, void *d_out_affine);
int gmsm_update_monomials(int group, const uint64_t *points, const void *d_points, size_t n, const uint64_t *r,
                          void *hip_stream, uint64_t *out_affine, void *d_out_affine);
int gmsm_linear_combinations(int group, const uint64_t *points, const void *d_points, size_t n,
                             const size_t *ends, size_t n_ends, const uint64_t *r, void *hip_stream,
                             uint64_t *out_truncated_jac, uint64_t *out_shifted_jac);

int gmsm_fr_batch_invert(int group, const uint64_t *a, const void *d_a, size_t n, void *hip_stream,
                         uint64_t *out, void *d_out);
int gmsm_iop_ratio_copy_constraint(uint64_t domain, const uint64_t *entries, const void *d_entries, size_t m,
                                   const uint32_t *layouts, const int64_t *perm, const void *d_perm,
                                   const uint64_t *beta, const uint64_t *gamma, int basis, int layout,
                                   void *hip_stream, uint64_t *out, void *d_out);
int gmsm_iop_ratio_shuffled(uint64_t domain, const uint64_t *num, const void *d_num, const uint64_t *den,
                            const void *d_den, size_t m, const uint32_t *num_layouts, const uint32_t *den_layouts,
                            const uint64_t *beta, int basis, int layout, void *hip_stream, uint64_t *out, void *d_out);

unsigned gmsm_default_window_bits(int group, size_t n);
unsigned gmsm_num_windows(int group, unsigned c);
int gmsm_default_plan(int group, size_t n, unsigned *c, unsigned *nwin, unsigned *entries_per_point, unsigned *fused);
int gmsm_window_sums_device(int group, const void *d_points, const void *d_scalars, size_t n, unsigned c,
                            unsigned win_first, unsigned win_stride, void *hip_stream, uint64_t *out_xyzz);
int gmsm_window_sums_enqueue(int group, const void *d_points, uint64_t bases_handle, const void *d_scalars, size_t n,
                             unsigned c, unsigned win_first, unsigned win_stride, void *hip_stream, void *d_out_xyzz);
int gmsm_fold_window_sets(int group, unsigned c, const uint64_t *xyzz_sets, unsigned nsets, uint64_t *out_jac);
int gmsm_fold_windows(int group, unsigned c, const uint64_t *xyzz_windows, uint64_t *out_jac);
int gmsm_jac_to_affine(int group, const uint64_t *jac, uint64_t *out_affine);

size_t gmsm_affine_limbs(int group);
size_t gmsm_scalar_limbs(int group);
int gmsm_debug_decompose(int group, const uint64_t *scalars, size_t n, unsigned c, uint32_t *out_digits);
int gmsm_debug_glv_split(int group, const uint64_t *scalars, size_t n, uint32_t *out);
int gmsm_debug_field_op(int group, int field, int op, const uint64_t *a, const uint64_t *b, size_t count, uint64_t *out);
int gmsm_debug_group_op(int group, int op, const uint64_t *acc, const uint64_t *pts_or_acc2, size_t count, uint64_t *out);

int gmsm_debug_reduce_shape(int group, uint32_t nw, uint32_t nbuckets, uint32_t out[6]);

int gmsm_generate_points(int group, const uint64_t *base_affine, const uint64_t *k0, const uint64_t *k1, int klimbs,
                         size_t n, int nthreads, uint64_t *out_points);
void gmsm_set_profiling(int on);
int gmsm_get_stage_times(double *out_ms, int max_stages, unsigned long *out_calls);
int gmsm_get_stage_launches(unsigned long *out_launches, int max_stages);

enum gmsm_option {
    GMSM_OPT_WINDOW_BITS = 0,
    GMSM_OPT_TABLES = 1,
    GMSM_OPT_MAX_RUN = 2,
    GMSM_OPT_HOST_RANGES = 3,
    GMSM_OPT_FIXED_BASE_BITS = 4,
    GMSM_OPT_SPIN_WAIT_US = 5,
    GMSM_OPT_SMALL_BITS = 6,
    GMSM_OPT_SMALL_MAX = 7,
    GMSM_OPT_SPLIT = 8,
    GMSM_OPT_GLV = 9,
    GMSM_OPT_SMALL_QUAD = 10,
    GMSM_OPT_POLY_LANE_BITS = 11,
    GMSM_OPT_REDUCE_SHAPE = 12
};
int gmsm_set_option(int key, unsigned value);
unsigned gmsm_get_option(int key);

int gmsm_trim(size_t keep_bytes, size_t *out_freed);
int gmsm_shutdown(void);

int gmsm_device_count(void);
int gmsm_set_device(int device);
const char *gmsm_last_error(void);
const char *gmsm_version(void);

#ifdef __cplusplus
}
#endif
#endif
```

Before: 559.2 MSM/s.

## Replace device bucket-reduction ladder tail with per-plane sums folded on host

Adds a 'planes' reduction tail. Each block of the combine kernel writes its partial sums as separate bit planes, a new k_plane_sums kernel reduces those across blocks, and the host folds the planes together with the window shifts using a doubling chain. The aim is to drop the later device combine and ladder kernels, which are serial and have little parallelism. In exchange the host copies more data (7+log2 blocks points per window) and does more point additions and doublings. It is on by default for small field types such as BN254 when the multiexp goes through the folded path.

```diff
diff --git a/gnark-crypto_amd/_lib.py b/gnark-crypto_amd/_lib.py
--- a/gnark-crypto_amd/_lib.py
+++ b/gnark-crypto_amd/_lib.py
@@ -29,7 +29,7 @@
     "gmsm_to_lagrange_g1", "gmsm_bases_to_lagrange", "gmsm_batch_scale", "gmsm_update_monomials", "gmsm_linear_combinations", "gmsm_shplonk_open_w", "gmsm_shplonk_open_wprime",
     "gmsm_fr_batch_invert", "gmsm_iop_ratio_copy_constraint", "gmsm_iop_ratio_shuffled",
     "gmsm_fflonk_next_divisor", "gmsm_fflonk_fold", "gmsm_fflonk_fold_commit", "gmsm_fflonk_open_w", "gmsm_fflonk_open_wprime",
-    "gmsm_bases_precompute", "gmsm_bases_table_bits", "gmsm_debug_table_runs", "gmsm_debug_small_runs", "gmsm_debug_reduce_shape", "gmsm_multiexp_sharded", "gmsm_bases_register_sharded", "gmsm_multiexp_bases_sharded", "gmsm_set_devices",
+    "gmsm_bases_precompute", "gmsm_bases_table_bits", "gmsm_debug_table_runs", "gmsm_debug_small_runs", "gmsm_debug_reduce_shape", "gmsm_debug_fold_planes", "gmsm_debug_plane_runs", "gmsm_multiexp_sharded", "gmsm_bases_register_sharded", "gmsm_multiexp_bases_sharded", "gmsm_set_devices",
     "gmsm_get_devices", "gmsm_set_option", "gmsm_get_option", "gmsm_trim", "gmsm_shutdown",
     "gmsm_device_count", "gmsm_set_device", "gmsm_last_error",
     "gmsm_version",
@@ -82,6 +82,10 @@
     L.gmsm_debug_table_runs.argtypes = []
     L.gmsm_debug_small_runs.restype = ctypes.c_ulong
     L.gmsm_debug_small_runs.argtypes = []
+    L.gmsm_debug_plane_runs.restype = ctypes.c_ulong
+    L.gmsm_debug_plane_runs.argtypes = []
+    L.gmsm_debug_fold_planes.restype = ctypes.c_int
+    L.gmsm_debug_fold_planes.argtypes = [ctypes.c_int, ctypes.c_uint, ctypes.c_uint, ctypes.c_uint, ctypes.c_uint, u64p, u64p]
     L.gmsm_debug_reduce_shape.restype = ctypes.c_int
     L.gmsm_debug_reduce_shape.argtypes = [ctypes.c_int, ctypes.c_uint32, ctypes.c_uint32, ctypes.POINTER(ctypes.c_uint32)]
     L.gmsm_multiexp_bases.restype = ctypes.c_int
@@ -247,7 +251,7 @@
 
 
 OPTIONS = {"window_bits": 0, "tables": 1, "max_run": 2, "host_ranges": 3, "fixed_base_bits": 4, "spin_wait_us": 5, "small_bits": 6, "small_max": 7, "split": 8, "glv": 9, "small_quad": 10,
-           "poly_lane_bits": 11, "reduce_shape": 12}
+           "poly_lane_bits": 11, "reduce_shape": 12, "reduce_tail": 13}
 
 
 def set_option(name, value):
diff --git a/gnark-crypto_amd/csrc/gmsm_context.h b/gnark-crypto_amd/csrc/gmsm_context.h
--- a/gnark-crypto_amd/csrc/gmsm_context.h
+++ b/gnark-crypto_amd/csrc/gmsm_context.h
@@ -64,11 +64,13 @@
     std::atomic<unsigned> small_quad{0};
     std::atomic<unsigned> poly_lane_bits{0};
     std::atomic<unsigned> reduce_shape{0};
+    std::atomic<unsigned> reduce_tail{0};
 };
 Options &options();
 
 extern std::atomic<unsigned long> g_small_runs;
 extern std::atomic<unsigned long> g_table_runs;
+extern std::atomic<unsigned long> g_plane_runs;
 
 struct ResidentBases {
     int group = -1;
@@ -153,6 +155,7 @@
     int timed_level = 0;
     void *pinned = nullptr;
     size_t pinned_cap = 0;
+    uint32_t plane_np = 0, plane_log2L = 0;
     DeviceBuffer h2d_points, h2d_scalars;
     DeviceBuffer raw_bytes, flagword;
     DeviceBuffer poly;
@@ -600,6 +603,7 @@
     int (*debug_glv_split)(const uint64_t *scalars, size_t n, uint32_t *out);
     void (*plan_info)(size_t n, unsigned *c, unsigned *nwin, unsigned *entries_per_point, unsigned *fused);
     void (*reduce_shape)(const Context &ctx, uint32_t nw, uint32_t nbuckets, uint32_t out[6]);
+    void (*fold_planes)(const uint64_t *planes, unsigned c, unsigned nwin, unsigned log2L, unsigned nhigh, uint64_t *out_jac);
     int (*poly_eval)(Context &ctx, const uint64_t *polys, const void *d_polys, const size_t *lens, size_t k, const uint64_t *point,
                      hipStream_t stream, uint64_t *out_values);
     int (*poly_div)(Context &ctx, const uint64_t *poly, const void *d_poly, size_t n, const uint64_t *point, hipStream_t stream,
diff --git a/gnark-crypto_amd/csrc/gmsm_engine.hip b/gnark-crypto_amd/csrc/gmsm_engine.hip
--- a/gnark-crypto_amd/csrc/gmsm_engine.hip
+++ b/gnark-crypto_amd/csrc/gmsm_engine.hip
@@ -17,6 +17,7 @@
 static std::atomic<int> g_default_device{0};
 std::atomic<unsigned long> g_table_runs{0};
 std::atomic<unsigned long> g_small_runs{0};
+std::atomic<unsigned long> g_plane_runs{0};
 static std::atomic<uint32_t> g_ticket_gen{0};
 
 std::string g_env_error;
@@ -855,6 +856,7 @@
 
 GMSM_EXPORT unsigned long gmsm_debug_table_runs(void) { return g_table_runs.load(); }
 GMSM_EXPORT unsigned long gmsm_debug_small_runs(void) { return g_small_runs.load(); }
+GMSM_EXPORT unsigned long gmsm_debug_plane_runs(void) { return g_plane_runs.load(); }
 
 GMSM_EXPORT unsigned gmsm_bases_table_bits(uint64_t handle) {
     if (handle & SHARDED_TAG) {
@@ -1670,6 +1672,17 @@
     int rc = get_context(&ctx);
     if (rc) return rc;
     vt->reduce_shape(*ctx, nw, nbuckets, out);
+    return GMSM_OK;
+}
+
+GMSM_EXPORT int gmsm_debug_fold_planes(int group, unsigned c, unsigned nwin, unsigned log2L, unsigned nblocks1, const uint64_t *planes,
+                                       uint64_t *out_jac) {
+    VT_OR_FAIL(group);
+    if (c < 2 || c > 24 || nwin == 0 || nwin > 512 || log2L > 8 || nblocks1 == 0 || nblocks1 > 128 || !planes || !out_jac)
+        return fail(GMSM_ERR_ARG, "gmsm_debug_fold_planes: 2 <= c <= 24, 1 <= nwin <= 512, log2L <= 8, 1 <= nblocks1 <= 128");
+    unsigned nhigh = 0;
+    while ((1u << nhigh) < nblocks1) ++nhigh;
+    vt->fold_planes(planes, c, nwin, log2L, nhigh, out_jac);
     return GMSM_OK;
 }
 
@@ -1863,6 +1876,8 @@
     {GMSM_OPT_REDUCE_SHAPE, &Options::reduce_shape,
      [](unsigned v) { return !(v > 255 || (v & 15u) > 8 || ((v >> 4) & 3u) == 1 || ((v >> 6) & 3u) == 3); },
      "GMSM_OPT_REDUCE_SHAPE: 0 (the cost model) or log2L (0, 1..8) | levels (0, 2, 3) << 4 | combine kernel (0, 1, 2) << 6"},
+    {GMSM_OPT_REDUCE_TAIL, &Options::reduce_tail, [](unsigned v) { return v <= 2; },
+     "GMSM_OPT_REDUCE_TAIL: 0 by group and call, 1 the device ladder, 2 the host planes"},
     {GMSM_OPT_SPIN_WAIT_US, &Options::spin_wait_us, [](unsigned v) { return v <= 1000000; }, "GMSM_OPT_SPIN_WAIT_US: at most 1000000"},
 };
 static const OptionRow *option_row(int key) {
diff --git a/gnark-crypto_amd/csrc/gmsm_group.h b/gnark-crypto_amd/csrc/gmsm_group.h
--- a/gnark-crypto_amd/csrc/gmsm_group.h
+++ b/gnark-crypto_amd/csrc/gmsm_group.h
@@ -36,6 +36,7 @@
     using Host::batch_to_affine;
     using Host::build_fixed_base_table;
     using Host::fold;
+    using Host::fold_planes;
     using Host::fold_powers;
     using Host::fold_sets;
     using Host::generate_points;
@@ -116,17 +117,55 @@
                            const ResidentBases *resident = nullptr, size_t resident_offset = 0) {
         int rc = order_after(ws, caller_stream);
         if (rc) return rc;
-        if ((rc = enqueue_window_sums(ctx, ws, d_points, d_scalars, n, plan, ws.stream, resident, nullptr, resident_offset)))
+        if ((rc = enqueue_window_sums(ctx, ws, d_points, d_scalars, n, plan, ws.stream, resident, nullptr, resident_offset,
+                                      false, false, TAIL_IF_FORCED)))
             return rc;
         return collect_window_sums(ws, ws.stream, plan.nwin_local, host_xyzz);
     }
+    static int window_sums_folded(Context &ctx, Workspace &ws, const void *d_points, const void *d_scalars, size_t n,
+                                  const WindowPlan &plan, hipStream_t caller_stream, J *out, const ResidentBases *resident) {
+        int rc = order_after(ws, caller_stream);
+        if (rc) return rc;
+        if ((rc = enqueue_window_sums(ctx, ws, d_points, d_scalars, n, plan, ws.stream, resident, nullptr, 0, false, false, TAIL_AUTO)))
+            return rc;
+        return collect_folded(ws, ws.stream, plan.c, plan.nwin_total, out);
+    }
+
+    enum { TAIL_LADDER = 0, TAIL_IF_FORCED = 1, TAIL_AUTO = 2 };
+#ifndef GMSM_PLANES_AUTO_WORDS
+#define GMSM_PLANES_AUTO_WORDS 9
+#endif
+    static constexpr bool PLANES_AUTO = sizeof(U) <= GMSM_PLANES_AUTO_WORDS * 4;
+    static constexpr uint32_t PLANE_BLOCKS = 128;
 
     static int collect_window_sums(Workspace &ws, hipStream_t stream, uint32_t nw, Ext *host_xyzz) {
         if (nw == 0) return GMSM_OK;
         HIP_TRY(wait_stream(stream));
         if (ws.pending_timed) StageTimer::collect(ws);
         ws.pending_timed = false;
+        if (ws.plane_np) {
+            const Ext *planes = (const Ext *)ws.pinned;
+            for (uint32_t w = 0; w < nw; ++w) {
+                const J j = fold_planes(planes + (size_t)w * ws.plane_np, 0, 1, ws.plane_log2L, ws.plane_np - 7);
+                host_xyzz[w] = j.z.is_zero() ? Ext::infinity() : xyzz_from_jac(j);
+            }
+            return GMSM_OK;
+        }
         memcpy(host_xyzz, ws.pinned, (size_t)nw * sizeof(Ext));
+        return GMSM_OK;
+    }
+    static int collect_folded(Workspace &ws, hipStream_t stream, unsigned c, uint32_t nwin, J *out) {
+        if (ws.plane_np) {
+            HIP_TRY(wait_stream(stream));
+            if (ws.pending_timed) StageTimer::collect(ws);
+            ws.pending_timed = false;
+            *out = fold_planes((const Ext *)ws.pinned, c, nwin, ws.plane_log2L, ws.plane_np - 7);
+            return GMSM_OK;
+        }
+        std::vector<Ext> totals(nwin);
+        int rc = collect_window_sums(ws, stream, nwin, totals.data());
+        if (rc) return rc;
+        *out = fold(totals.data(), c, nwin);
         return GMSM_OK;
     }
 
@@ -295,9 +334,11 @@
     static int enqueue_window_sums(Context &ctx, Workspace &ws, const void *d_points, const void *d_scalars, size_t n,
                                    const WindowPlan &plan, hipStream_t stream, const ResidentBases *resident,
                                    void *d_out = nullptr, size_t resident_offset = 0 ,
-                                   bool buckets_only = false, bool time_range = false ) {
+                                   bool buckets_only = false, bool time_range = false ,
+                                   int tail_mode = TAIL_LADDER ) {
         const uint32_t nwd = plan.nwin_local;
         ws.pending_timed = false;
+        ws.plane_np = 0;
         if (nwd == 0) return GMSM_OK;
         const bool shared = plan.shared != 0;
         if (shared && !(resident && resident->tab_c.load() == plan.c && plan.win_first == 0 && plan.win_stride == 1))
@@ -335,6 +376,16 @@
         const Geometry qa = split ? plan_geometry(ctx, nw / 2, n, NB, shared) : q;
         const size_t tot_thr = (size_t)nw * qa.tpw;
         const size_t tot_blk = (size_t)nw * q.nblocks1;
+        bool planes = false;
+        if constexpr (COMBINE_WE) {
+            const unsigned tail = options().reduce_tail.load(std::memory_order_relaxed);
+            const bool can = tail_mode != TAIL_LADDER && !d_out && !buckets_only && !shared && !split && q.nblocks1 <= PLANE_BLOCKS;
+            planes = can && (tail == 2 || (tail == 0 && tail_mode == TAIL_AUTO && PLANES_AUTO &&
+                                           options().reduce_shape.load(std::memory_order_relaxed) == 0));
+        }
+        uint32_t plane_h = 0;
+        while ((1u << plane_h) < q.nblocks1) ++plane_h;
+        const uint32_t plane_np = 7 + plane_h;
 
         uint32_t log2NB = 0;
         while ((1u << log2NB) < NB) ++log2NB;
@@ -373,11 +424,11 @@
         if ((rc = ws.parted.ensure((size_t)nw * n * 4))) return rc;
         if ((rc = ws.starts.ensure((size_t)nw * (NB + 1) * 4))) return rc;
         if ((rc = ws.buckets.ensure((size_t)nw * NB * REC))) return rc;
-        if ((rc = ws.partials.ensure((tot_blk + (size_t)nw * q.nblocks2) * 2 * REC))) return rc;
+        if ((rc = ws.partials.ensure(planes ? tot_blk * 8 * REC : (tot_blk + (size_t)nw * q.nblocks2) * 2 * REC))) return rc;
         const uint32_t T = (uint32_t)(((size_t)NB + ((size_t)1 << q.log2L) - 1) >> q.log2L);
         if ((rc = ws.red_pre.ensure((size_t)nw * T * 2 * REC))) return rc;
         if ((rc = ws.totals.ensure((size_t)nwd * sizeof(Ext)))) return rc;
-        if ((rc = ws.ensure_pinned((size_t)nwd * sizeof(Ext)))) return rc;
+        if ((rc = ws.ensure_pinned((size_t)nwd * (planes ? plane_np : 1u) * sizeof(Ext)))) return rc;
         if ((rc = ws.blockhist.ensure((size_t)nw * pchunks * nparts * 4))) return rc;
         if ((rc = ws.counts.ensure((size_t)nw * (2 * nparts + 1) * 4))) return rc;
         if ((rc = ws.seg_partials.ensure(tot_thr * 2 * REC))) return rc;
@@ -423,6 +474,12 @@
         if constexpr (SERIAL_QUAD)
             if ((rc = ctx.allow_lds((const void *)k_reduce_serial_q<U, SERIAL_Q_QUADS>, (int)(3 * SERIAL_Q_QUADS * sizeof(QRec<U>))))) return rc;
         if ((rc = ctx.allow_lds((const void *)k_reduce2_q<U, true>, (int)(2 * RED2_TPB * sizeof(QRec<U>))))) return rc;
+        if constexpr (COMBINE_WE) {
+            if (planes) {
+                if ((rc = ctx.allow_lds((const void *)k_combine_we<U, true, true>, (int)((2 * COMBINE_N + 1) * sizeof(QRec<U>))))) return rc;
+                if ((rc = ctx.allow_lds((const void *)k_plane_sums<U, true>, (int)(PLANE_BLOCKS * sizeof(QRec<U>))))) return rc;
+            }
+        }
 
         StageTimer timer(ws, !buckets_only || time_range);
         ws.timed = timer.on;
@@ -539,7 +596,7 @@
             hipLaunchKernelGGL((k_fixup_long<U>), dim3(2 * ctx.num_cus), dim3(256), 128 * sizeof(QRec<U>), st, NB, part_g, pb_g, qa.tpw,
                                buckets_g, (const uint32_t *)cnt_g, (const LongChain *)list_g, done_g, sums_g, st_g, qa.seg);
             if (mark) timer.mark(T_REDUCE, st);
-            if (!buckets_only) enqueue_reduce_kernels(ctx, ws, q, T, buckets_g, st_g, nk, NB, st, k0);
+            if (!buckets_only) enqueue_reduce_kernels(ctx, ws, q, T, buckets_g, st_g, nk, NB, st, k0, planes);
         };
         timer.mark(T_ACCUMULATE, stream);
         if (!split) {
@@ -563,7 +620,11 @@
             hipLaunchKernelGGL((k_fill_infinity<Ext>), dim3((nwd - nw + 63) / 64), dim3(64), 0, stream, ws.totals.ptr, nw, nwd - nw);
         timer.mark(T_END, stream);
         HIP_TRY(hipGetLastError());
-        if (!buckets_only) {
+        if (planes) {
+            ws.plane_np = plane_np;
+            ws.plane_log2L = q.log2L;
+            g_plane_runs.fetch_add(1, std::memory_order_relaxed);
+        } else if (!buckets_only) {
             if (d_out)
                 HIP_TRY(hipMemcpyAsync(d_out, ws.totals.ptr, (size_t)nwd * sizeof(Ext), hipMemcpyDeviceToDevice, stream));
             else
@@ -591,7 +652,8 @@
 
     static void enqueue_reduce_kernels(Context &ctx, Workspace &ws, const Geometry &q, uint32_t T, const void *buckets,
                                        const uint32_t *starts, uint32_t nw, uint32_t NB, hipStream_t stream,
-                                       uint32_t k0 = 0 ) {
+                                       uint32_t k0 = 0 ,
+                                       bool planes = false ) {
         constexpr size_t RECB = sizeof(typename OpsSerial::Mem);
         void *red_pre = (char *)ws.red_pre.ptr + (size_t)k0 * T * 2 * RECB;
         void *partials = (char *)ws.partials.ptr + (size_t)k0 * q.nblocks1 * 2 * RECB;
@@ -603,6 +665,18 @@
         else
             hipLaunchKernelGGL((k_reduce_serial<OpsSerial>), dim3((T + 255) / 256, nw), dim3(256), 0, stream, buckets, NB,
                                q.log2L, T, starts, red_pre);
+        if constexpr (COMBINE_WE) {
+            if (planes) {
+                uint32_t h = 0;
+                while ((1u << h) < q.nblocks1) ++h;
+                const uint32_t quads = std::min(64u, std::max(16u, (1u << h) / 2));
+                hipLaunchKernelGGL((k_combine_we<U, true, true>), dim3(q.nblocks1, nw), dim3(4 * COMBINE_N),
+                                   (2 * COMBINE_N + 1) * sizeof(QRec<U>), stream, q.log2L, ws.partials.ptr, 0u, (const void *)red_pre, T);
+                hipLaunchKernelGGL((k_plane_sums<U, true>), dim3(nw, 8), dim3(4 * quads), ((size_t)1 << h) * sizeof(QRec<U>), stream,
+                                   (const void *)ws.partials.ptr, q.nblocks1, h, ws.pinned);
+                return;
+            }
+        }
         const auto combine = [&](const void *in, uint32_t pairs, void *out, uint32_t blocks, uint32_t l2, uint32_t pre) {
             if constexpr (COMBINE_WE) {
                 if (use_combine_we(ctx, blocks * nw)) {
@@ -640,6 +714,7 @@
         const Geometry q = plan_geometry(ctx, nw, n_for_geometry, NB);
         const uint32_t T = (uint32_t)(((size_t)NB + ((size_t)1 << q.log2L) - 1) >> q.log2L);
         int rc;
+        ws.plane_np = 0;
         if ((rc = ws.partials.ensure((size_t)nw * (q.nblocks1 + q.nblocks2) * 2 * REC))) return rc;
         if ((rc = ws.red_pre.ensure((size_t)nw * T * 2 * REC))) return rc;
         if ((rc = ws.totals.ensure((size_t)nwd * sizeof(Ext)))) return rc;
@@ -1079,6 +1154,7 @@
         constexpr size_t REC = sizeof(typename OpsSerial::Mem);
         int rc;
         ws.pending_timed = false;
+        ws.plane_np = 0;
         if ((rc = begin_use(ws, ws.stream))) return rc;
         if ((rc = ws.ensure_pinned((size_t)plan.nwin_total * sizeof(Ext)))) return rc;
         if ((rc = ws.small_sums.ensure((size_t)nw * sp.nslices * REC))) return rc;
@@ -1165,13 +1241,8 @@
         const WindowPlan plan = plan_for(resident, n);
         const unsigned c = plan.c;
         const unsigned nr = device_ranges(n, plan);
+        if (nr <= 1) return window_sums_folded(ctx, ws, d_points, d_scalars, n, plan, caller_stream, out, resident);
         std::vector<Ext> totals(plan.nwin_total);
-        if (nr <= 1) {
-            int rc = window_sums(ctx, ws, d_points, d_scalars, n, plan, caller_stream, totals.data(), resident);
-            if (rc) return rc;
-            *out = fold(totals.data(), c, plan.nwin_total);
-            return GMSM_OK;
-        }
         constexpr size_t REC = sizeof(typename OpsSerial::Mem);
         const size_t per = (n + nr - 1) / nr;
         int rc = order_after(ws, caller_stream);
@@ -1207,18 +1278,14 @@
         WindowPlan plan = plan_for(resident, n);
         if (n > max_run_points(plan)) plan = make_plan(choose_c(FR_BITS, AFF_BYTES, n), 0, 1);
         const unsigned c = plan.c;
-        int rc = enqueue_window_sums(ctx, ws, nullptr, d_scalars, n, plan, ws.stream, resident);
+        int rc = enqueue_window_sums(ctx, ws, nullptr, d_scalars, n, plan, ws.stream, resident, nullptr, 0, false, false, TAIL_AUTO);
         if (rc) return rc;
         ws.pending_c = c;
         ws.pending_nw = plan.nwin_total;
         return GMSM_OK;
     }
     static int multiexp_collect(Workspace &ws, J *out) {
-        std::vector<Ext> totals(ws.pending_nw);
-        int rc = collect_window_sums(ws, ws.stream, ws.pending_nw, totals.data());
-        if (rc) return rc;
-        *out = fold(totals.data(), ws.pending_c);
-        return GMSM_OK;
+        return collect_folded(ws, ws.stream, ws.pending_c, ws.pending_nw, out);
     }
 
 
diff --git a/gnark-crypto_amd/csrc/gmsm_group_host.h b/gnark-crypto_amd/csrc/gmsm_group_host.h
--- a/gnark-crypto_amd/csrc/gmsm_group_host.h
+++ b/gnark-crypto_amd/csrc/gmsm_group_host.h
@@ -39,6 +39,41 @@
         }
         if (acc.z.is_zero()) acc = J{F::one(), F::one(), F::zero()};
         return acc;
+    }
+
+    static J fold_planes(const Ext *planes, unsigned c, unsigned nwin, unsigned log2L, unsigned nhigh) {
+        const unsigned NP = 7 + nhigh;
+        const unsigned top = c * (nwin - 1) + log2L + NP - 2;
+        std::vector<int> head(top + 1, -1), next((size_t)nwin * NP, -1);
+        for (unsigned w = 0; w < nwin; ++w)
+            for (unsigned i = 0; i < NP; ++i) {
+                const int idx = (int)(w * NP + i);
+                if (planes[idx].zz.is_zero()) continue;
+                const unsigned b = c * w + (i == 0 ? 0 : log2L + i - 1);
+                next[idx] = head[b];
+                head[b] = idx;
+            }
+        int b = (int)top;
+        while (b >= 0 && head[b] < 0) --b;
+        Ext acc = Ext::infinity();
+        while (b >= 0) {
+            for (int i = head[b]; i >= 0; i = next[i]) xyzz_add(acc, planes[i]);
+            if (b == 0) break;
+            int nb = b - 1;
+            while (nb > 0 && head[nb] < 0) --nb;
+            const int gap = b - nb;
+            if (!acc.zz.is_zero()) {
+                if (gap >= 4) {
+                    J j = jac_from_xyzz(acc);
+                    for (int l = 0; l < gap; ++l) j = jac_double(j);
+                    acc = j.z.is_zero() ? Ext::infinity() : xyzz_from_jac(j);
+                } else {
+                    for (int l = 0; l < gap; ++l) acc = xyzz_double(acc);
+                }
+            }
+            b = nb;
+        }
+        return jac_from_xyzz(acc);
     }
 
     static Ext scalar_mul(const Aff &a, const uint64_t *k, int klimbs) {
diff --git a/gnark-crypto_amd/csrc/gmsm_group_vtable.h b/gnark-crypto_amd/csrc/gmsm_group_vtable.h
--- a/gnark-crypto_amd/csrc/gmsm_group_vtable.h
+++ b/gnark-crypto_amd/csrc/gmsm_group_vtable.h
@@ -164,6 +164,10 @@
         *c = p.c, *nwin = p.nwin_total, *entries_per_point = p.glv ? 2u : 1u, *fused = 0u;
     }
     static void reduce_shape(const Context &ctx, uint32_t nw, uint32_t nbuckets, uint32_t out[6]) { G::reduce_shape(ctx, nw, nbuckets, out); }
+    static void fold_planes(const uint64_t *planes, unsigned c, unsigned nwin, unsigned log2L, unsigned nhigh, uint64_t *out_jac) {
+        typename G::J j = G::fold_planes(reinterpret_cast<const typename G::Ext *>(planes), c, nwin, log2L, nhigh);
+        memcpy(out_jac, &j, sizeof j);
+    }
     static int debug_field_op(int field, int op, const uint64_t *a, const uint64_t *b, size_t count, uint64_t *out) {
         using BaseP = typename G::F::Params;
         if (field == 0) {
@@ -588,7 +592,7 @@
             GMSM_VT(decode_raw), GMSM_VT(validate_points), GMSM_VT(decode_compressed), GMSM_VT(encode_compressed);
             GMSM_VT(fft_domain_new), GMSM_VT(fft_run), GMSM_VT(fft_bit_reverse);
             GMSM_VT(precompute_tables), GMSM_VT(tables_serve), GMSM_VT(shard_piece), GMSM_VT(host_piece_ranges);
-            GMSM_VT(debug_glv_split), GMSM_VT(plan_info), GMSM_VT(reduce_shape);
+            GMSM_VT(debug_glv_split), GMSM_VT(plan_info), GMSM_VT(reduce_shape), GMSM_VT(fold_planes);
             GMSM_VT(poly_eval), GMSM_VT(poly_div), GMSM_VT(kzg_open);
             if constexpr (IS_G1) GMSM_VT(to_lagrange);
             GMSM_VT(fflonk_next_divisor), GMSM_VT(open_check), GMSM_VT(fflonk_fold);
diff --git a/gnark-crypto_amd/csrc/gmsm_quad.h b/gnark-crypto_amd/csrc/gmsm_quad.h
--- a/gnark-crypto_amd/csrc/gmsm_quad.h
+++ b/gnark-crypto_amd/csrc/gmsm_quad.h
@@ -298,7 +298,7 @@
     if (j == 1) quad_rec_store<U>(out1, ((size_t)k * gridDim.x + blk) * 2 + 0, PARK, lane);
 }
 
-template <class U, bool INL>
+template <class U, bool INL, bool PLANES = false>
 __global__ void __launch_bounds__(256) k_combine_we(uint32_t log2L, void *__restrict__ out1, uint32_t prescale,
                                                     const void *__restrict__ pre, uint32_t T) {
     constexpr uint32_t N = 64;
@@ -331,6 +331,13 @@
         quad_add_store<U, INL>(X, o, act, lane);
         __syncthreads();
     }
+    if constexpr (PLANES) {
+        if (j < 8) {
+            const QRec<U> *src = j == 0 ? &S[0] : j < 7 ? &S[1u << (j - 1)] : &W[0];
+            quad_rec_store<U>(out1, ((size_t)k * gridDim.x + blk) * 8 + j, src, lane);
+        }
+        return;
+    }
     if (j == 0) {
         PARK->c[t & 3u] = S[0].c[t & 3u];
         if ((t & 3u) == 0) PARK->inf = S[0].inf;
@@ -365,6 +372,59 @@
     if (j == 1) quad_rec_store<U>(out1, ((size_t)k * gridDim.x + blk) * 2 + 0, PARK, lane);
 }
 
+template <class U, bool INL>
+__global__ void __launch_bounds__(256) k_plane_sums(const void *__restrict__ in1, uint32_t nblocks1, uint32_t H,
+                                                    void *__restrict__ planes_out) {
+    extern __shared__ __align__(16) unsigned char lds_raw[];
+    QRec<U> *P = reinterpret_cast<QRec<U> *>(lds_raw);
+    const uint32_t NBP = 1u << H, k = blockIdx.x, p = blockIdx.y, t = threadIdx.x, j = t >> 2, lane = t & 63u, nq = blockDim.x >> 2;
+    for (uint32_t b = j; b < NBP; b += nq) quad_rec_load<U>(&P[b], in1, ((size_t)k * nblocks1 + b) * 8 + p, b < nblocks1, lane);
+    __syncthreads();
+#pragma nounroll
+    for (uint32_t s = 1; s <= H; ++s) {
+        const uint32_t g = NBP >> s, nops = p ? g : g * s;
+#pragma nounroll
+        for (uint32_t o0 = 0; o0 < nops; o0 += nq) {
+            const uint32_t op = o0 + j;
+            const bool act = op < nops;
+            QRec<U> *X = &P[0], *Y = &P[0];
+            if (act) {
+                const uint32_t G = op >> (H - s), i = op & (g - 1u);
+                if (p) {
+                    X = &P[i];
+                    Y = X + g;
+                } else if (G == 0u) {
+                    const uint32_t l = s - 1;
+                    X = &P[(2 * i) << l];
+                    Y = &P[(2 * i + 1) << l];
+                } else {
+                    const uint32_t l = G - 1u;
+                    X = &P[(2 * i + 1) << l];
+                    Y = &P[(2 * (i + g) + 1) << l];
+                }
+            }
+            const QAddOps<U> o = quad_add_load<U>(X, Y, lane);
+            __syncthreads();
+            quad_add_store<U, INL>(X, o, act, lane);
+            __syncthreads();
+        }
+    }
+    using T = LzTraits<U>;
+    using Mem = XYZZ<typename T::Sat>;
+    const uint32_t NP = 7u + H, r = t & 3u, nres = p ? 1u : H;
+    for (uint32_t q = j; q < nres; q += nq) {
+        const QRec<U> *src = p ? &P[0] : &P[1u << q];
+        const uint32_t slot = p == 7u ? 0u : p ? p : 7u + q;
+        typename T::Sat *dst = reinterpret_cast<typename T::Sat *>(reinterpret_cast<char *>(planes_out) + ((size_t)k * NP + slot) * sizeof(Mem));
+        typename T::Sat v = T::template to_sat<INL>(src->c[r]);
+        if (src->inf) {
+            const Mem inf = Mem::infinity();
+            v = r == 0 ? inf.x : r == 1 ? inf.y : r == 2 ? inf.zz : inf.zzz;
+        }
+        dst[r] = v;
+    }
+}
+
 #endif
 
 }
diff --git a/gnark-crypto_amd/multiexp.py b/gnark-crypto_amd/multiexp.py
--- a/gnark-crypto_amd/multiexp.py
+++ b/gnark-crypto_amd/multiexp.py
@@ -354,6 +354,15 @@
             raise RuntimeError(self._error(rc))
         return out
 
+    def fold_planes(self, planes, c, nwin, log2L, nblocks1):
+        planes = np.ascontiguousarray(planes, dtype=np.uint64)
+        assert planes.size == nwin * (7 + (nblocks1 - 1).bit_length()) * self.xyzz_limbs
+        out = np.zeros(self.jac_limbs, dtype=np.uint64)
+        rc = _lib.load().gmsm_debug_fold_planes(self.gid, c, nwin, log2L, nblocks1, _ptr(planes), _ptr(out))
+        if rc:
+            raise RuntimeError(self._error(rc))
+        return out
+
     def jac_to_affine(self, jac):
         L = _lib.load()
         jac = np.ascontiguousarray(jac, dtype=np.uint64)
diff --git a/include/gmsm.h b/include/gmsm.h
--- a/include/gmsm.h
+++ b/include/gmsm.h
@@ -169,6 +169,9 @@
 int gmsm_debug_group_op(int group, int op, const uint64_t *acc, const uint64_t *pts_or_acc2, size_t count, uint64_t *out);
 
 int gmsm_debug_reduce_shape(int group, uint32_t nw, uint32_t nbuckets, uint32_t out[6]);
+int gmsm_debug_fold_planes(int group, unsigned c, unsigned nwin, unsigned log2L, unsigned nblocks1, const uint64_t *planes,
+                           uint64_t *out_jac);
+unsigned long gmsm_debug_plane_runs(void);
 
 int gmsm_generate_points(int group, const uint64_t *base_affine, const uint64_t *k0, const uint64_t *k1, int klimbs,
                          size_t n, int nthreads, uint64_t *out_points);
@@ -189,6 +192,7 @@
     GMSM_OPT_GLV = 9,
     GMSM_OPT_SMALL_QUAD = 10,
     GMSM_OPT_POLY_LANE_BITS = 11,
+    GMSM_OPT_REDUCE_TAIL = 13,
     GMSM_OPT_REDUCE_SHAPE = 12
 };
 int gmsm_set_option(int key, unsigned value);
```

After: 604.5 MSM/s, median of 6. +8.1%, better.
